# s-esposito/MonoGS

Hardware: AMD Instinct MI355X
Metric: rasteriser fwd+bwd Mpix/s @1080p (higher is better)
Workload: dtype f32; 1 GPU; C5: 2000000 Gaussians, 1920x1080, fwd+bwd, seeded synthetic map (SURVEY.md 8d), one keyframe per GPU; gaussians=2000000, width=1920, height=1080, settle_steps=60, instance_count=device-side (capacity mode, overflow checked), parallelism=keyframe-per-gpu x1

## Files before the change

include/monogs_raster.h:

```cpp
#ifndef MONOGS_RASTER_H
#define MONOGS_RASTER_H

#include <stddef.h>
#include <stdint.h>

#ifdef __cplusplus
extern "C" {
#endif

#define MGS_ABI_VERSION 12
#define MGS_TILE 16

typedef struct mgs_camera {
    int32_t image_height;
    int32_t image_width;
    float tanfovx;
    float tanfovy;
    float scale_modifier;
    int32_t sh_degree;
    int32_t sh_coeffs;
    int32_t scale_dim;
    int32_t flags;
    const float* bg;
    const float* viewmatrix;
    const float* projmatrix;
    const float* projmatrix_raw;
    const float* campos;
} mgs_camera;

#define MGS_FLAG_EXCLUSIVE_DEVICE 1

typedef struct mgs_timing {
    float preprocess_ms;
    float depth_sort_ms;
    float scan_ms;
    float duplicate_ms;
    float sort_ms;
    float ranges_ms;
    float blend_fwd_ms;
    float blend_bwd_ms;
    float geom_bwd_ms;
} mgs_timing;

int mgs_abi_version(void);
const char* mgs_last_error(void);

#define MGS_MAX_GAUSSIANS ((1 << 26) - 1)

size_t mgs_geometry_bytes(int32_t P);
size_t mgs_image_bytes(int32_t width, int32_t height);
size_t mgs_binning_bytes(uint64_t num_rendered, int32_t width, int32_t height);
size_t mgs_backward_bytes(int32_t P);
float* mgs_backward_tau(void* backward_scratch, int32_t P);

int mgs_forward_preprocess(const mgs_camera* cam, int32_t P,
                           const float* means3D,
                           const float* shs,
                           const float* colors_precomp,
                           const float* opacities,
                           const float* scales,
                           const float* rotations,
                           const float* cov3D_precomp,
                           void* geometry, int32_t* radii ,
                           void* prepare_backward ,
                           uint64_t* num_rendered ,
                           const uint32_t* prev_status ,
                           uint32_t* prev_status_out ,
                           mgs_timing* timing , void* stream);

int mgs_forward_render(const mgs_camera* cam, int32_t P, uint64_t num_rendered,
                       void* geometry, void* binning, void* image,
                       float* out_color, float* out_depth, float* out_opacity, int32_t* n_touched,
                       uint32_t* status ,
                       mgs_timing* timing, void* stream);

#define MGS_STATUS_CAPACITY_OVERFLOW 1u
#define MGS_STATUS_DEPTH_SORT_TIMEOUT 2u
#define MGS_STATUS_TILE_SORT_TIMEOUT 4u

int mgs_debug_set_radix_spin_limit(uint32_t limit);
int mgs_debug_set_option(const char* name, int64_t value);

int mgs_binning_path(int32_t P, int32_t W, int32_t H);

size_t mgs_debug_sort_temp_bytes(uint64_t n, int32_t bits);
int mgs_debug_sort_pairs(uint32_t* keys, uint32_t* vals, uint32_t* keys_alt, uint32_t* vals_alt, uint64_t n, int32_t bits,
                         void* temp, void* stream);

int mgs_forward_render_capacity(const mgs_camera* cam, int32_t P, uint64_t capacity,
                                void* geometry, void* binning, void* image,
                                float* out_color, float* out_depth, float* out_opacity, int32_t* n_touched,
                                uint32_t* overflow, mgs_timing* timing, void* stream);
int mgs_forward_capacity(const mgs_camera* cam, int32_t P, const float* means3D, const float* shs,
                         const float* colors_precomp, const float* opacities, const float* scales, const float* rotations,
                         const float* cov3D_precomp, void* geometry, int32_t* radii, void* prepare_backward,
                         uint64_t capacity, void* binning, void* image, float* out_color, float* out_depth,
                         float* out_opacity, int32_t* n_touched, uint32_t* overflow, mgs_timing* timing, void* stream);

int mgs_backward(const mgs_camera* cam, int32_t P, uint64_t num_rendered,
                 const float* means3D, const float* shs, const float* colors_precomp,
                 const float* opacities, const float* scales, const float* rotations,
                 const float* cov3D_precomp, const int32_t* radii,
                 const void* geometry, const void* binning, const void* image,
                 const float* dL_dcolor, const float* dL_ddepth,
                 const float* out_color, const float* out_depth,
                 float* dL_dmeans2D,
                 float* dL_dcolors,
                 float* dL_dopacity,
                 float* dL_dmeans3D,
                 float* dL_dcov3D,
                 float* dL_dsh,
                 float* dL_dscales,
                 float* dL_drotations,
                 float* dL_dtau,
                 void* backward_scratch, int32_t scratch_prepared, mgs_timing* timing, void* stream);

#define MGS_VALU_CEILING_BLOCKS 2048
int mgs_debug_valu_ceiling(float* out, int32_t iters, void* stream);

int mgs_debug_set_blend_events(void* fwd_start, void* fwd_end, void* bwd_start, void* bwd_end);

int mgs_debug_last_backward_split(void);

#define MGS_BLEND_STATS_WORDS 24
int mgs_debug_blend_stats(const mgs_camera* cam, int32_t P, uint64_t num_rendered, const void* geometry,
                          const void* binning, const void* image, uint64_t* stats_dev, void* stream);

int mgs_mark_visible(int32_t P, const float* means3D, const float* viewmatrix, const float* projmatrix,
                     uint8_t* visible, void* stream);

size_t mgs_knn_scratch_bytes(int32_t P);
int mgs_dist2_knn(int32_t P, const float* points , float* out ,
                  void* scratch, void* stream);

#define MGS_LOSS_TRACKING 1
#define MGS_LOSS_INVERT_DEPTH 2
#define MGS_LOSS_SCRATCH_DAB 10
#define MGS_LOSS_SCRATCH_LOSS 12
size_t mgs_loss_scratch_bytes(void);
int mgs_loss_forward(int32_t width, int32_t height, int32_t mode, int32_t init, float lambda_rgb,
                     const float* render, const float* depth, const float* opacity, const float* gt_rgb,
                     const float* gt_depth, const uint8_t* mask, const uint8_t* grad_mask,
                     const float* exposure_a, const float* exposure_b, float* scratch, float* loss_out,
                     void* stream);
int mgs_loss_backward(int32_t width, int32_t height, int32_t mode, int32_t init, float lambda_rgb,
                      const float* render, const float* depth, const float* opacity, const float* gt_rgb,
                      const float* gt_depth, const uint8_t* mask, const uint8_t* grad_mask,
                      const float* exposure_a, const float* exposure_b, const float* scratch,
                      const float* grad_out, float* d_render, float* d_depth, float* d_exposure, void* stream);
int mgs_loss_grads(int32_t width, int32_t height, int32_t mode, int32_t init, float lambda_rgb,
                   const float* render, const float* depth, const float* opacity, const float* gt_rgb,
                   const float* gt_depth, const uint8_t* mask, const uint8_t* grad_mask,
                   const float* exposure_a, const float* exposure_b, float* scratch, float* d_render, float* d_depth,
                   void* stream);

#define MGS_SSIM_C1 0.0001f
#define MGS_SSIM_C2 0.0009f
#define MGS_SSIM_SCRATCH_LOSS 0
#define MGS_SSIM_SCRATCH_L1 1
#define MGS_SSIM_SCRATCH_SSIM 2
size_t mgs_ssim_scratch_bytes(int32_t planes, int32_t width, int32_t height, int32_t train);
int mgs_ssim_forward(int32_t planes, int32_t width, int32_t height, int32_t valid, int32_t train, float C1, float C2,
                     const float* img1, const float* img2, float* scratch, float* value_out, void* stream);
int mgs_ssim_backward(int32_t planes, int32_t width, int32_t height, int32_t valid, float C1, float C2,
                      const float* img1, const float* img2, const float* scratch, const float* grad_out,
                      float* d_img1, void* stream);
int mgs_refine_loss_forward(int32_t width, int32_t height, float lambda_ssim, const float* render, const float* gt_rgb,
                            float* scratch, float* loss_out, void* stream);
int mgs_refine_loss_backward(int32_t width, int32_t height, float lambda_ssim, const float* render, const float* gt_rgb,
                             const float* scratch, const float* grad_out, float* d_render, void* stream);
int mgs_refine_loss_grads(int32_t width, int32_t height, float lambda_ssim, const float* render, const float* gt_rgb,
                          float* scratch, float* d_render, void* stream);

#define MGS_POSE_STICKY 1
int mgs_pose_step(float* R, float* T, float* rot_delta, float* trans_delta, float* exposure_a, float* exposure_b,
                  const float* grad_rot, const float* grad_trans, const float* grad_a, const float* grad_b,
                  float* adam_m, float* adam_v, int32_t step, float lr_rot, float lr_trans, float lr_exposure,
                  float beta1, float beta2, float eps, float converged_threshold, int32_t* step_counter, float* out,
                  int32_t flags, float* host_flag ,
                  const float* projmatrix_raw, float* viewmatrix, float* projmatrix, float* campos ,
                  void* stream);
int mgs_pose_step_batch(int32_t n, void* const* ptrs, float lr_rot, float lr_trans, float lr_exposure, float beta1,
                        float beta2, float eps, float converged_threshold, int32_t flags, void* stream);

int mgs_backproject(int32_t N, int32_t W, int32_t H, const int64_t* selected, const float* rgb ,
                    const float* depth , const int32_t* segmentation ,
                    const float* exposure_a, const float* exposure_b, float fx, float fy, float cx, float cy,
                    const float* R, const float* T, float* points , float* features ,
                    int32_t* ids , void* stream);

int mgs_camera_setup(const float* R, const float* T, const float* projmatrix_raw, float* viewmatrix ,
                     float* projmatrix , float* campos , void* stream);

int mgs_adam_step(int32_t n_tensors, float* const* params, const float* const* grads, float* const* exp_avg,
                  float* const* exp_avg_sq, const uint64_t* numel, const float* lr, double beta1, double beta2,
                  double eps, int32_t step, int32_t* step_counter,
                  const float* lr_device ,
                  void* stream);
int mgs_densify_stats(int32_t P, const float* viewspace_grad , const int32_t* radii,
                      float* xyz_gradient_accum , float* denom , float* max_radii_2d ,
                      void* stream);
int mgs_window_stats(int32_t P, int32_t n_keyframes, const float* const* grad_means2D, const int32_t* const* radii,
                     const int32_t* const* n_touched, float* grad_norm , float* visible ,
                     float* max_radii , int32_t accumulate, uint64_t* visibility_bits, void* stream);
int mgs_window_apply(int32_t P, const float* grad_norm, const float* visible, const float* max_radii,
                     float* xyz_gradient_accum, float* denom, float* max_radii_2d, void* stream);
int mgs_lr_schedule_step(int32_t* iteration, float* lr_out, double lr_init, double lr_final, int32_t lr_delay_steps,
                         double lr_delay_mult, int32_t max_steps, void* stream);

int mgs_activate_forward(int32_t P, int32_t scale_dim , const float* rot_raw ,
                         const float* scale_raw , const float* opacity_raw ,
                         float* rotations , float* scales3 , float* opacities ,
                         void* stream);
int mgs_activate_backward(int32_t P, int32_t scale_dim, const float* rot_raw, const float* scales3,
                          const float* opacities, const float* grad_rotations, const float* grad_scales3,
                          const float* grad_opacities, float* d_rot_raw, float* d_scale_raw, float* d_opacity_raw,
                          void* stream);

int mgs_sum_buffers(int32_t n_src, const float* const* src, float* dst, uint64_t count, void* stream);

#ifdef __cplusplus
}
#endif
#endif
```

monogs_amd/_lib.py:

```python
from __future__ import annotations

import ctypes as C
import os

_HERE = os.path.dirname(os.path.abspath(__file__))
LIB_PATH = os.environ.get("MGS_LIB_PATH") or os.path.join(_HERE, "lib", "libmonogs_raster.so")
ABI_VERSION = 12

c_float_p = C.c_void_p


class MgsCamera(C.Structure):
    _fields_ = [
        ("image_height", C.c_int32), ("image_width", C.c_int32),
        ("tanfovx", C.c_float), ("tanfovy", C.c_float), ("scale_modifier", C.c_float),
        ("sh_degree", C.c_int32), ("sh_coeffs", C.c_int32), ("scale_dim", C.c_int32), ("flags", C.c_int32),
        ("bg", C.c_void_p), ("viewmatrix", C.c_void_p), ("projmatrix", C.c_void_p),
        ("projmatrix_raw", C.c_void_p), ("campos", C.c_void_p),
    ]


class MgsTiming(C.Structure):
    _fields_ = [(n, C.c_float) for n in (
        "preprocess_ms", "depth_sort_ms", "scan_ms", "duplicate_ms", "sort_ms", "ranges_ms", "blend_fwd_ms",
        "blend_bwd_ms", "geom_bwd_ms")]

    def as_dict(self):
        return {n: float(getattr(self, n)) for n, _ in self._fields_}


SIGNATURES = {
    "mgs_abi_version": (C.c_int, []),
    "mgs_last_error": (C.c_char_p, []),
    "mgs_geometry_bytes": (C.c_size_t, [C.c_int32]),
    "mgs_image_bytes": (C.c_size_t, [C.c_int32, C.c_int32]),
    "mgs_binning_bytes": (C.c_size_t, [C.c_uint64, C.c_int32, C.c_int32]),
    "mgs_backward_bytes": (C.c_size_t, [C.c_int32]),
    "mgs_forward_preprocess": (C.c_int, [C.POINTER(MgsCamera), C.c_int32] + [C.c_void_p] * 7
                               + [C.c_void_p, C.c_void_p, C.c_void_p, C.POINTER(C.c_uint64), C.c_void_p, C.POINTER(C.c_uint32),
                                  C.POINTER(MgsTiming), C.c_void_p]),
    "mgs_forward_capacity": (C.c_int, [C.POINTER(MgsCamera), C.c_int32] + [C.c_void_p] * 7 + [C.c_void_p] * 3 + [C.c_uint64]
                             + [C.c_void_p] * 7 + [C.POINTER(MgsTiming), C.c_void_p]),
    "mgs_forward_render": (C.c_int, [C.POINTER(MgsCamera), C.c_int32, C.c_uint64] + [C.c_void_p] * 8
                           + [C.POINTER(MgsTiming), C.c_void_p]),
    "mgs_debug_set_radix_spin_limit": (C.c_int, [C.c_uint32]),
    "mgs_debug_set_option": (C.c_int, [C.c_char_p, C.c_int64]),
    "mgs_binning_path": (C.c_int, [C.c_int32, C.c_int32, C.c_int32]),
    "mgs_debug_sort_temp_bytes": (C.c_size_t, [C.c_uint64, C.c_int32]),
    "mgs_debug_sort_pairs": (C.c_int, [C.c_void_p] * 4 + [C.c_uint64, C.c_int32, C.c_void_p, C.c_void_p]),
    "mgs_forward_render_capacity": (C.c_int, [C.POINTER(MgsCamera), C.c_int32, C.c_uint64] + [C.c_void_p] * 8
                                    + [C.POINTER(MgsTiming), C.c_void_p]),
    "mgs_backward": (C.c_int, [C.POINTER(MgsCamera), C.c_int32, C.c_uint64] + [C.c_void_p] * 7
                     + [C.c_void_p] * 4 + [C.c_void_p] * 4 + [C.c_void_p] * 9
                     + [C.c_void_p, C.c_int32, C.POINTER(MgsTiming), C.c_void_p]),
    "mgs_backward_tau": (C.c_void_p, [C.c_void_p, C.c_int32]),
    "mgs_debug_blend_stats": (C.c_int, [C.POINTER(MgsCamera), C.c_int32, C.c_uint64] + [C.c_void_p] * 5),
    "mgs_debug_valu_ceiling": (C.c_int, [C.c_void_p, C.c_int32, C.c_void_p]),
    "mgs_debug_set_blend_events": (C.c_int, [C.c_void_p] * 4),
    "mgs_debug_last_backward_split": (C.c_int, []),
    "mgs_mark_visible": (C.c_int, [C.c_int32, C.c_void_p, C.c_void_p, C.c_void_p, C.c_void_p, C.c_void_p]),
    "mgs_loss_scratch_bytes": (C.c_size_t, []),
    "mgs_loss_forward": (C.c_int, [C.c_int32] * 4 + [C.c_float] + [C.c_void_p] * 9 + [C.c_void_p, C.c_void_p, C.c_void_p]),
    "mgs_loss_backward": (C.c_int, [C.c_int32] * 4 + [C.c_float] + [C.c_void_p] * 9
                          + [C.c_void_p, C.c_void_p, C.c_void_p, C.c_void_p, C.c_void_p, C.c_void_p]),
    "mgs_loss_grads": (C.c_int, [C.c_int32] * 4 + [C.c_float] + [C.c_void_p] * 9 + [C.c_void_p] * 4),
    "mgs_ssim_scratch_bytes": (C.c_size_t, [C.c_int32] * 4),
    "mgs_ssim_forward": (C.c_int, [C.c_int32] * 5 + [C.c_float] * 2 + [C.c_void_p] * 5),
    "mgs_ssim_backward": (C.c_int, [C.c_int32] * 4 + [C.c_float] * 2 + [C.c_void_p] * 6),
    "mgs_refine_loss_forward": (C.c_int, [C.c_int32] * 2 + [C.c_float] + [C.c_void_p] * 5),
    "mgs_refine_loss_backward": (C.c_int, [C.c_int32] * 2 + [C.c_float] + [C.c_void_p] * 6),
    "mgs_refine_loss_grads": (C.c_int, [C.c_int32] * 2 + [C.c_float] + [C.c_void_p] * 5),
    "mgs_backproject": (C.c_int, [C.c_int32] * 3 + [C.c_void_p] * 6 + [C.c_float] * 4 + [C.c_void_p] * 6),
    "mgs_camera_setup": (C.c_int, [C.c_void_p] * 7),
    "mgs_pose_step": (C.c_int, [C.c_void_p] * 12 + [C.c_int32] + [C.c_float] * 7
                      + [C.c_void_p, C.c_void_p, C.c_int32, C.c_void_p] + [C.c_void_p] * 4 + [C.c_void_p]),
    "mgs_pose_step_batch": (C.c_int, [C.c_int32, C.POINTER(C.c_void_p)] + [C.c_float] * 7 + [C.c_int32, C.c_void_p]),
    "mgs_adam_step": (C.c_int, [C.c_int32] + [C.c_void_p] * 6 + [C.c_double] * 3 + [C.c_int32, C.c_void_p, C.c_void_p, C.c_void_p]),
    "mgs_window_stats": (C.c_int, [C.c_int32, C.c_int32] + [C.c_void_p] * 6 + [C.c_int32, C.c_void_p, C.c_void_p]),
    "mgs_window_apply": (C.c_int, [C.c_int32] + [C.c_void_p] * 7),
    "mgs_lr_schedule_step": (C.c_int, [C.c_void_p, C.c_void_p, C.c_double, C.c_double, C.c_int32, C.c_double, C.c_int32, C.c_void_p]),
    "mgs_densify_stats": (C.c_int, [C.c_int32] + [C.c_void_p] * 6),
    "mgs_sum_buffers": (C.c_int, [C.c_int32, C.POINTER(C.c_void_p), C.c_void_p, C.c_uint64, C.c_void_p]),
    "mgs_activate_forward": (C.c_int, [C.c_int32, C.c_int32] + [C.c_void_p] * 7),
    "mgs_activate_backward": (C.c_int, [C.c_int32, C.c_int32] + [C.c_void_p] * 10),
    "mgs_knn_scratch_bytes": (C.c_size_t, [C.c_int32]),
    "mgs_dist2_knn": (C.c_int, [C.c_int32, C.c_void_p, C.c_void_p, C.c_void_p, C.c_void_p]),
}

_lib = None


class MonoGSNativeError(RuntimeError):
    pass


def load():
    global _lib
    if _lib is not None:
        return _lib
    if not os.path.exists(LIB_PATH):
        raise MonoGSNativeError(
            f"{LIB_PATH} not found: build it with `python -c 'import __graft_entry__ as g; g.build()'` "
            "or `make -C monogs_amd/csrc`.  There is no CPU fallback.")
    lib = C.CDLL(LIB_PATH)
    for name, (res, args) in SIGNATURES.items():
        fn = getattr(lib, name)
        fn.restype = res
        fn.argtypes = args
    if lib.mgs_abi_version() != ABI_VERSION:
        raise MonoGSNativeError(f"ABI mismatch: library {lib.mgs_abi_version()} vs binding {ABI_VERSION}; rebuild")
    for kv in filter(None, os.environ.get("MGS_DEBUG_OPTIONS", "").split(",")):
        k, _, v = kv.partition("=")
        if lib.mgs_debug_set_option(k.strip().encode(), int(v)) != 0:
            raise MonoGSNativeError(f"MGS_DEBUG_OPTIONS: {lib.mgs_last_error().decode()}")
    _lib = lib
    return lib


def check(rc: int, what: str):
    if rc != 0:
        msg = load().mgs_last_error().decode("utf-8", "replace")
        raise Exception(msg) if rc == 1 else MonoGSNativeError(f"{what}: {msg}")
```

monogs_amd/csrc/api.hip:

```cpp
#include "common.h"

#include <stdarg.h>
#include <stdio.h>
#include <string.h>

namespace mgs {

static thread_local char g_err[512] = "";

void set_error(const char* fmt, ...) {
    va_list ap;
    va_start(ap, fmt);
    vsnprintf(g_err, sizeof(g_err), fmt, ap);
    va_end(ap);
}

static inline char* take(char*& p, size_t bytes) {
    char* r = p;
    p += align_up(bytes, 256);
    return r;
}

GeometryState GeometryState::carve(void* base, int P) {
    char* p = (char*)align_up((size_t)base, 256);
    GeometryState g;
    g.rec = (float*)take(p, (size_t)P * REC_FLOATS * sizeof(float));
    g.depth_key = (uint32_t*)take(p, (size_t)P * sizeof(uint32_t));
    g.depth_alt = (uint32_t*)take(p, (size_t)P * sizeof(uint32_t));
    g.iota = (uint32_t*)take(p, (size_t)P * sizeof(uint32_t));
    g.iota_alt = (uint32_t*)take(p, (size_t)P * sizeof(uint32_t));
    g.perm = (uint32_t*)take(p, (size_t)P * sizeof(uint32_t));
    g.point_offsets = (uint32_t*)take(p, (size_t)P * sizeof(uint32_t));
    g.scan_blocks = (uint32_t*)take(p, ((size_t)scan_nblocks(P) + 64) * sizeof(uint32_t));
    g.clamped = (uint8_t*)take(p, (size_t)P * 4);
    g.rect = (uint2*)take(p, (size_t)P * sizeof(uint2));
    g.rect_sorted = (uint2*)take(p, (size_t)P * sizeof(uint2));
    g.scan_status = (uint64_t*)take(p, (SCAN_SMALL_MAX_BLOCKS + 1) * sizeof(uint64_t));
    g.tile_hist = (uint32_t*)take(p, 4 * 256 * sizeof(uint32_t));
    g.sort_temp_bytes = radix_depth_temp_bytes((uint64_t)P);
    g.sort_temp = take(p, g.sort_temp_bytes);
    g.end = p;
    return g;
}
size_t GeometryState::bytes(int P) {
    const GeometryState g = carve(nullptr, P);
    return (size_t)g.end + 256;
}

size_t ImageState::bytes(int W, int H) {
    const size_t HW = (size_t)W * H, nt = (size_t)tiles_x(W) * tiles_y(H);
    return align_up(HW * 4, 256) * 2 + align_up(nt * sizeof(uint2), 256) + 256;
}
ImageState ImageState::carve(void* base, int W, int H) {
    const size_t HW = (size_t)W * H, nt = (size_t)tiles_x(W) * tiles_y(H);
    char* p = (char*)align_up((size_t)base, 256);
    ImageState s;
    s.final_T = (float*)take(p, HW * 4);
    s.n_contrib = (uint32_t*)take(p, HW * 4);
    s.ranges = (uint2*)take(p, nt * sizeof(uint2));
    return s;
}

size_t BinningState::bytes(uint64_t R, int W, int H) {
    const size_t r = (size_t)(R ? R : 1);
    return align_up(r * 4, 256) * 4 + align_up(mgs::sort_temp_bytes(R, tile_bits(W, H)), 256) + 256 + 256;
}
BinningState BinningState::carve(void* base, uint64_t R, int W, int H) {
    const size_t r = (size_t)(R ? R : 1);
    char* p = (char*)align_up((size_t)base, 256);
    BinningState b;
    b.keys_a = (uint32_t*)take(p, r * 4);
    b.keys_b = (uint32_t*)take(p, r * 4);
    b.vals_a = (uint32_t*)take(p, r * 4);
    b.vals_b = (uint32_t*)take(p, r * 4);
    const bool in_b = radix_result_in_b(tile_bits(W, H));
    b.keys_sorted = in_b ? b.keys_b : b.keys_a;
    b.vals_sorted = in_b ? b.vals_b : b.vals_a;
    b.sort_temp_bytes = mgs::sort_temp_bytes(R, tile_bits(W, H));
    b.sort_temp = take(p, b.sort_temp_bytes);
    b.count = (uint32_t*)take(p, 2 * sizeof(uint32_t));
    return b;
}

struct StageTimer {
    hipStream_t s;
    bool on;
    hipEvent_t ev[10];
    int n = 0;
    StageTimer(hipStream_t s_, bool on_) : s(s_), on(on_) {
        if (on) for (auto& e : ev) (void)hipEventCreate(&e);
    }
    ~StageTimer() {
        if (on) for (auto& e : ev) (void)hipEventDestroy(e);
    }
    void mark() {
        if (on && n < 10) (void)hipEventRecord(ev[n++], s);
    }
    float ms(int i) {
        float t = 0.f;
        if (on && i + 1 < n) (void)hipEventElapsedTime(&t, ev[i], ev[i + 1]);
        return t;
    }
    void sync() {
        if (on && n) (void)hipEventSynchronize(ev[n - 1]);
    }
};

static int check_cam(const mgs_camera* cam) {
    if (!cam) { set_error("camera is NULL"); return 1; }
    if (cam->image_width <= 0 || cam->image_height <= 0) { set_error("image size must be positive"); return 1; }
    if (!cam->bg || !cam->viewmatrix || !cam->projmatrix || !cam->projmatrix_raw || !cam->campos) {
        set_error("camera tensors (bg, viewmatrix, projmatrix, projmatrix_raw, campos) must be non-NULL");
        return 1;
    }
    return 0;
}

static hipEvent_t g_dbg_fwd_events[2] = {nullptr, nullptr}, g_dbg_bwd_events[2] = {nullptr, nullptr};

static int check_map_size(int32_t P) {
    if (P > MGS_MAX_GAUSSIANS) {
        set_error("P exceeds MGS_MAX_GAUSSIANS (2^26 - 1): the gradient-line offset of the blend backward is 32-bit");
        return 1;
    }
    return 0;
}

}

using namespace mgs;

extern "C" {

int mgs_abi_version(void) { return MGS_ABI_VERSION; }
int mgs_binning_path(int32_t P, int32_t W, int32_t H) { return binning_path(P, W, H); }
const char* mgs_last_error(void) { return g_err; }

size_t mgs_geometry_bytes(int32_t P) { return GeometryState::bytes(P < 0 ? 0 : P); }
size_t mgs_image_bytes(int32_t W, int32_t H) { return ImageState::bytes(W, H); }
size_t mgs_binning_bytes(uint64_t R, int32_t W, int32_t H) { return BinningState::bytes(R, W, H); }
size_t mgs_backward_bytes(int32_t P) {
    return (size_t)(P < 0 ? 0 : P) * GRAD_FLOATS * sizeof(float) + (size_t)(TAU_SLOTS + 1) * 16 * sizeof(float) + 256;
}
float* mgs_backward_tau(void* backward_scratch, int32_t P) { return backward_tau_out(backward_scratch, P < 0 ? 0 : P); }

int mgs_forward_preprocess(const mgs_camera* cam, int32_t P, const float* means3D, const float* shs,
                           const float* colors_precomp, const float* opacities, const float* scales,
                           const float* rotations, const float* cov3D_precomp, void* geometry, int32_t* radii,
                           void* prepare_backward, uint64_t* num_rendered, const uint32_t* prev_status,
                           uint32_t* prev_status_out, mgs_timing* timing, void* stream) {
    if (check_cam(cam)) return 1;
    if (P < 0) { set_error("P must be >= 0"); return 1; }
    if (check_map_size(P)) return 1;
    if (num_rendered) *num_rendered = 0;
    if (prev_status_out) *prev_status_out = 0;
    if (P == 0) {
        if (prev_status && prev_status_out) {
            MGS_HIP(hipMemcpyAsync(prev_status_out, prev_status, sizeof(uint32_t), hipMemcpyDeviceToHost, (hipStream_t)stream));
            MGS_HIP(hipStreamSynchronize((hipStream_t)stream));
        }
        return 0;
    }
    if (!means3D || !opacities || !geometry || !radii) { set_error("means3D, opacities, geometry, radii must be non-NULL"); return 1; }
    if ((shs == nullptr) == (colors_precomp == nullptr)) {
        set_error("Please provide excatly one of either SHs or precomputed colors!");
        return 1;
    }
    const bool have_sr = scales != nullptr || rotations != nullptr;
    if ((have_sr && (!scales || !rotations || cov3D_precomp)) || (!have_sr && !cov3D_precomp)) {
        set_error("Please provide exactly one of either scale/rotation pair or precomputed 3D covariance!");
        return 1;
    }
    if (shs && (cam->sh_degree < 0 || cam->sh_degree > 3 || cam->sh_coeffs < (cam->sh_degree + 1) * (cam->sh_degree + 1))) {
        set_error("sh_degree must be 0..3 and shs must hold at least (degree+1)^2 coefficients");
        return 1;
    }
    hipStream_t s = (hipStream_t)stream;
    GeometryState g = GeometryState::carve(geometry, P);
    StageTimer tm(s, timing != nullptr);
    tm.mark();
    if (int rc = launch_preprocess_forward(*cam, P, means3D, shs, colors_precomp, opacities, scales, rotations,
                                           cov3D_precomp, g, radii,
                                           prepare_backward ? backward_grad_acc(prepare_backward) : nullptr, s)) return rc;
    tm.mark();
    const bool exclusive = (cam->flags & MGS_FLAG_EXCLUSIVE_DEVICE) != 0;
    const bool per_tile = binning_path(P, cam->image_width, cam->image_height) != 0;
    if (per_tile) {
        tm.mark();
        if (int rc = launch_scan(g, P, s, exclusive, g.rect)) return rc;
    } else {
        if (int rc = launch_depth_sort(g, P, depth_sort_payload(P, cam->image_width, cam->image_height), s, exclusive)) return rc;
        tm.mark();
        if (int rc = launch_scan(g, P, s, exclusive, g.rect_sorted)) return rc;
    }
    tm.mark();
    if (num_rendered) {
        uint32_t total = 0, sort_errors[RADIX_ERROR_WORDS] = {0, 0, 0, 0};
        MGS_HIP(hipMemcpyAsync(&total, g.scan_blocks + scan_nblocks(P), sizeof(uint32_t), hipMemcpyDeviceToHost, s));
        MGS_HIP(hipMemcpyAsync(sort_errors, radix_depth_error_flag(g.sort_temp, (uint64_t)P), sizeof(sort_errors),
                               hipMemcpyDeviceToHost, s));
        if (prev_status && prev_status_out)
            MGS_HIP(hipMemcpyAsync(prev_status_out, prev_status, sizeof(uint32_t), hipMemcpyDeviceToHost, s));
        MGS_HIP(hipStreamSynchronize(s));
        if (sort_errors[0] | sort_errors[1] | sort_errors[2] | sort_errors[3]) { set_error("depth sort: a look-back spin timed out (results invalid)"); return 3; }
        *num_rendered = total;
    }
    if (timing) {
        if (!num_rendered) MGS_HIP(hipStreamSynchronize(s));
        timing->preprocess_ms = tm.ms(0);
        timing->depth_sort_ms = per_tile ? 0.f : tm.ms(1);
        timing->scan_ms = tm.ms(2);
    }
    return 0;
}

static int g_opt_tile_sort_fused = 1;

static int forward_render_impl(const mgs_camera* cam, int32_t P, uint64_t R, bool capacity, void* geometry,
                               void* binning, void* image, float* out_color, float* out_depth, float* out_opacity,
                               int32_t* n_touched, uint32_t* overflow, mgs_timing* timing, void* stream) {
    if (check_cam(cam)) return 1;
    if (P < 0) { set_error("P must be >= 0"); return 1; }
    if (check_map_size(P)) return 1;
    if (!image || !out_color || !out_depth || !out_opacity) { set_error("image scratch and outputs must be non-NULL"); return 1; }
    if (P > 0 && (!geometry || !n_touched)) { set_error("geometry and n_touched must be non-NULL"); return 1; }
    if (R > 0 && !binning) { set_error("binning scratch is NULL"); return 1; }
    if (R >= (1ull << 32)) { set_error("num_rendered exceeds 2^32-1"); return 1; }
    if (P == 0) R = 0;
    hipStream_t s = (hipStream_t)stream;
    const int W = cam->image_width, H = cam->image_height;
    GeometryState g = GeometryState::carve(geometry, P);
    ImageState img = ImageState::carve(image, W, H);
    BinningState b = BinningState::carve(binning, R, W, H);
    const uint32_t* n_dev = nullptr;
    StageTimer tm(s, timing != nullptr);
    const bool cap = capacity && binning;
    if (cap) n_dev = b.count;
    const bool per_tile = binning_path(P, W, H) != 0;
    tm.mark();
    if (int rc = launch_duplicate(*cam, P, g, b, capacity ? R : (R > 0 ? 0xFFFFFFFFull : 0ull), n_touched, img, R,
                                  tile_bits(W, H), cap ? b.count : nullptr, overflow, s, per_tile)) return rc;
    tm.mark();
    if (int rc = launch_sort(g, b, R, tile_bits(W, H), s, n_dev, (cam->flags & MGS_FLAG_EXCLUSIVE_DEVICE) != 0, img.ranges,
                             per_tile)) return rc;
    const uint32_t* sort_err = R > 0 ? radix_error_flag(b.sort_temp, R, tile_bits(W, H)) : nullptr;
    const bool sort_tiles = per_tile && R > 0;
    const TileSortArgs ts = sort_tiles ? tile_sort_args(*cam, g, b, R, n_dev) : TileSortArgs{};
    const bool fused = sort_tiles && g_opt_tile_sort_fused != 0;
    if (sort_tiles && !fused)
        if (int rc = launch_tile_depth_sort(*cam, ts, img, sort_err, s)) return rc;
    tm.mark();
    if (g_dbg_fwd_events[0]) MGS_HIP(hipEventRecord(g_dbg_fwd_events[0], s));
    if (int rc = launch_blend_forward(*cam, g, b, img, out_color, out_depth, out_opacity, n_touched, sort_err, overflow,
                                      fused ? &ts : nullptr, s)) return rc;
    if (g_dbg_fwd_events[1]) MGS_HIP(hipEventRecord(g_dbg_fwd_events[1], s));
    tm.mark();
    if (timing) {
        tm.sync();
        timing->duplicate_ms = tm.ms(0);
        timing->sort_ms = tm.ms(1);
        timing->ranges_ms = 0.f;
        timing->blend_fwd_ms = tm.ms(2);
    }
    return 0;
}

int mgs_forward_render(const mgs_camera* cam, int32_t P, uint64_t R, void* geometry, void* binning, void* image,
                       float* out_color, float* out_depth, float* out_opacity, int32_t* n_touched,
                       uint32_t* status, mgs_timing* timing, void* stream) {
    return forward_render_impl(cam, P, R, false, geometry, binning, image, out_color, out_depth, out_opacity, n_touched,
                               status, timing, stream);
}

int mgs_forward_render_capacity(const mgs_camera* cam, int32_t P, uint64_t capacity, void* geometry, void* binning,
                                void* image, float* out_color, float* out_depth, float* out_opacity,
                                int32_t* n_touched, uint32_t* overflow, mgs_timing* timing, void* stream) {
    if (capacity == 0) { set_error("capacity must be > 0"); return 1; }
    return forward_render_impl(cam, P, capacity, true, geometry, binning, image, out_color, out_depth, out_opacity,
                               n_touched, overflow, timing, stream);
}

int mgs_forward_capacity(const mgs_camera* cam, int32_t P, const float* means3D, const float* shs,
                         const float* colors_precomp, const float* opacities, const float* scales, const float* rotations,
                         const float* cov3D_precomp, void* geometry, int32_t* radii, void* prepare_backward,
                         uint64_t capacity, void* binning, void* image, float* out_color, float* out_depth,
                         float* out_opacity, int32_t* n_touched, uint32_t* overflow, mgs_timing* timing, void* stream) {
    if (int rc = mgs_forward_preprocess(cam, P, means3D, shs, colors_precomp, opacities, scales, rotations, cov3D_precomp,
                                        geometry, radii, prepare_backward, nullptr, nullptr, nullptr, timing, stream)) return rc;
    return mgs_forward_render_capacity(cam, P, capacity, geometry, binning, image, out_color, out_depth, out_opacity,
                                       n_touched, overflow, timing, stream);
}

int mgs_backward(const mgs_camera* cam, int32_t P, uint64_t R, const float* means3D, const float* shs,
                 const float* colors_precomp, const float* opacities, const float* scales, const float* rotations,
                 const float* cov3D_precomp, const int32_t* radii, const void* geometry, const void* binning,
                 const void* image, const float* dL_dcolor, const float* dL_ddepth, const float* out_color,
                 const float* out_depth, float* dL_dmeans2D, float* dL_dcolors, float* dL_dopacity, float* dL_dmeans3D, float* dL_dcov3D, float* dL_dsh,
                 float* dL_dscales, float* dL_drotations, float* dL_dtau, void* backward_scratch,
                 int32_t scratch_prepared, mgs_timing* timing, void* stream) {
    if (check_cam(cam)) return 1;
    if (P < 0) { set_error("P must be >= 0"); return 1; }
    if (check_map_size(P)) return 1;
    hipStream_t s = (hipStream_t)stream;
    if (P == 0) {
        if (dL_dtau) MGS_HIP(zero_fill(dL_dtau, 6 * sizeof(float), s));
        return 0;
    }
    if (!means3D || !opacities || !radii || !geometry || !image || !dL_dcolor || !dL_ddepth || !backward_scratch) {
        set_error("means3D, opacities, radii, geometry, image, dL_dcolor, dL_ddepth, backward_scratch must be non-NULL");
        return 1;
    }
    if (R > 0 && !binning) { set_error("binning scratch is NULL"); return 1; }
    const int W = cam->image_width, H = cam->image_height;
    GeometryState g = GeometryState::carve(const_cast<void*>(geometry), P);
    ImageState img = ImageState::carve(const_cast<void*>(image), W, H);
    BinningState b = BinningState::carve(const_cast<void*>(binning), R, W, H);
    float* grad_acc = backward_grad_acc(backward_scratch);
    StageTimer tm(s, timing != nullptr);
    float* tau_part = (dL_dtau && (P + 255) / 256 > TAU_DIRECT_MAX_BLOCKS) ? backward_tau_part(backward_scratch, P) : nullptr;
    if (scratch_prepared) {
        if (dL_dtau && dL_dtau != backward_tau_out(backward_scratch, P)) {
            set_error("scratch_prepared: dL_dtau must be mgs_backward_tau(backward_scratch, P)");
            return 1;
        }
    } else {
        MGS_HIP(zero_fill2(grad_acc, (size_t)P * GRAD_FLOATS * sizeof(float) + (tau_part ? (size_t)TAU_SLOTS * 16 * sizeof(float) : 0),
                           dL_dtau, 6 * sizeof(float), s));
    }
    tm.mark();
    if (R > 0) {
        const bool pose_only = !dL_dcolors && !dL_dopacity && !dL_dsh && !shs;
        if (g_dbg_bwd_events[0]) MGS_HIP(hipEventRecord(g_dbg_bwd_events[0], s));
        if (int rc = launch_blend_backward(*cam, g, b, img, dL_dcolor, dL_ddepth, out_color, out_depth, grad_acc, pose_only, R, s)) return rc;
        if (g_dbg_bwd_events[1]) MGS_HIP(hipEventRecord(g_dbg_bwd_events[1], s));
    }
    tm.mark();
    GeomBackwardArgs a;
    a.means3D = means3D; a.shs = shs; a.colors_precomp = colors_precomp; a.opacities = opacities;
    a.scales = scales; a.rotations = rotations; a.cov3D_precomp = cov3D_precomp; a.radii = radii;
    a.grad_acc = grad_acc;
    a.dL_dmeans2D = dL_dmeans2D; a.dL_dcolors = dL_dcolors; a.dL_dopacity = dL_dopacity;
    a.dL_dmeans3D = dL_dmeans3D; a.dL_dcov3D = dL_dcov3D; a.dL_dsh = dL_dsh; a.dL_dscales = dL_dscales;
    a.dL_drotations = dL_drotations; a.dL_dtau = dL_dtau; a.tau_part = tau_part;
    if (int rc = launch_geom_backward(*cam, P, g, a, s)) return rc;
    tm.mark();
    if (timing) {
        tm.sync();
        timing->blend_bwd_ms = tm.ms(0);
        timing->geom_bwd_ms = tm.ms(1);
    }
    return 0;
}

int mgs_debug_blend_stats(const mgs_camera* cam, int32_t P, uint64_t R, const void* geometry, const void* binning,
                           const void* image, uint64_t* stats_dev, void* stream) {
    if (check_cam(cam)) return 1;
    if (!geometry || !image || !stats_dev || (R > 0 && !binning)) { set_error("bad arguments"); return 1; }
    hipStream_t s = (hipStream_t)stream;
    MGS_HIP(zero_fill(stats_dev, MGS_BLEND_STATS_WORDS * sizeof(uint64_t), s));
    if (P == 0 || R == 0) return 0;
    const int W = cam->image_width, H = cam->image_height;
    GeometryState g = GeometryState::carve(const_cast<void*>(geometry), P);
    ImageState img = ImageState::carve(const_cast<void*>(image), W, H);
    BinningState b = BinningState::carve(const_cast<void*>(binning), R, W, H);
    return launch_blend_backward_stats(*cam, g, b, img, (unsigned long long*)stats_dev, s);
}

int mgs_debug_valu_ceiling(float* out, int32_t iters, void* stream) {
    if (!out || iters < 1) { set_error("mgs_debug_valu_ceiling: bad arguments"); return 1; }
    return launch_valu_ceiling(out, iters, (hipStream_t)stream);
}

int mgs_debug_last_backward_split(void) { return g_dbg_last_bwd_split; }

int mgs_debug_set_radix_spin_limit(uint32_t limit) { return set_radix_spin_limit(limit); }

int mgs_debug_set_blend_events(void* fwd_start, void* fwd_end, void* bwd_start, void* bwd_end) {
    if ((fwd_start == nullptr) != (fwd_end == nullptr) || (bwd_start == nullptr) != (bwd_end == nullptr)) {
        set_error("mgs_debug_set_blend_events: a pair is both events or neither");
        return 1;
    }
    g_dbg_fwd_events[0] = (hipEvent_t)fwd_start; g_dbg_fwd_events[1] = (hipEvent_t)fwd_end;
    g_dbg_bwd_events[0] = (hipEvent_t)bwd_start; g_dbg_bwd_events[1] = (hipEvent_t)bwd_end;
    return 0;
}

static int g_opt_debug_sort_exclusive = 0;
size_t mgs_debug_sort_temp_bytes(uint64_t n, int32_t bits) { return radix_temp_bytes(n, bits); }
int mgs_debug_sort_pairs(uint32_t* keys, uint32_t* vals, uint32_t* keys_alt, uint32_t* vals_alt, uint64_t n, int32_t bits,
                         void* temp, void* stream) {
    if (bits < 1 || bits > 32 || (n && (!keys || !vals || !keys_alt || !vals_alt || !temp))) {
        set_error("mgs_debug_sort_pairs: bad arguments");
        return 1;
    }
    if (n == 0) return 0;
    hipStream_t s = (hipStream_t)stream;
    if (int rc = radix_sort_pairs(keys, vals, keys_alt, vals_alt, n, bits, temp, s, nullptr, false, nullptr, nullptr, nullptr, false,
                                  g_opt_debug_sort_exclusive != 0))
        return rc;
    if (radix_result_in_b(bits)) {
        MGS_HIP(hipMemcpyAsync(keys, keys_alt, n * 4, hipMemcpyDeviceToDevice, s));
        MGS_HIP(hipMemcpyAsync(vals, vals_alt, n * 4, hipMemcpyDeviceToDevice, s));
    }
    uint32_t err[RADIX_ERROR_WORDS];
    MGS_HIP(hipMemcpyAsync(err, radix_error_flag(temp, n, bits), sizeof(err), hipMemcpyDeviceToHost, s));
    MGS_HIP(hipStreamSynchronize(s));
    if (err[0] | err[1] | err[2] | err[3]) { set_error("mgs_debug_sort_pairs: a look-back spin timed out"); return 2; }
    return 0;
}

int mgs_debug_set_option(const char* name, int64_t value) {
    if (name && !strcmp(name, "radix_scanned")) { g_opt_radix_scanned = (int)value; return 0; }
    if (name && !strcmp(name, "radix_ballot_rank")) { g_opt_radix_ballot_rank = (int)value; return 0; }
    if (name && !strcmp(name, "radix_xcd_band")) { g_opt_radix_xcd_band = (int)value; return 0; }
    if (name && !strcmp(name, "debug_sort_exclusive")) { g_opt_debug_sort_exclusive = (int)value; return 0; }
    if (name && !strcmp(name, "dup_slot_major")) { g_opt_dup_slot_major = (int)value; return 0; }
    if (name && !strcmp(name, "blend_bwd_transposed")) {
        g_opt_blend_bwd_transposed = value < 0 ? 2 : (int)value;
        g_opt_blend_bwd_transposed_set = value >= 0;
        return 0;
    }
    if (name && !strcmp(name, "blend_bwd_split")) { g_opt_blend_bwd_split = value < 0 ? -1 : (int)value; return 0; }
    if (name && !strcmp(name, "blend_bwd_split_min")) { g_opt_blend_bwd_split_min = value < 0 ? 4 : (int)value; return 0; }
    if (name && !strcmp(name, "blend_bwd_split_frac")) { g_opt_blend_bwd_split_frac = value < 0 ? 32 : (int)value; return 0; }
    if (name && !strcmp(name, "scan_small")) { g_opt_scan_small = (int)value; return 0; }
    if (name && !strcmp(name, "tile_sort_fused")) { g_opt_tile_sort_fused = value < 0 ? 1 : (int)value; return 0; }
    if (name && !strcmp(name, "knn_grid_min")) { g_opt_knn_grid_min = value > 0x7FFFFFFF ? 0x7FFFFFFF : (int)value; return 0; }
    set_error("mgs_debug_set_option: unknown option");
    return 1;
}

int mgs_mark_visible(int32_t P, const float* means3D, const float* viewmatrix, const float* projmatrix,
                     uint8_t* visible, void* stream) {
    (void)projmatrix;
    if (P < 0 || (P > 0 && (!means3D || !viewmatrix || !visible))) { set_error("bad arguments"); return 1; }
    return launch_mark_visible(P, means3D, viewmatrix, visible, (hipStream_t)stream);
}

size_t mgs_knn_scratch_bytes(int32_t P) { return knn_scratch_bytes(P); }

int mgs_dist2_knn(int32_t P, const float* points, float* out, void* scratch, void* stream) {
    if (P < 0 || (P > 0 && (!points || !out))) { set_error("bad arguments"); return 1; }
    return launch_knn(P, points, out, scratch, (hipStream_t)stream);
}

}
```

monogs_amd/csrc/binning.hip:

```cpp
#include "common.h"
#include "tile_sort.h"


namespace mgs {

constexpr int SCAN_THREADS = 256;
__device__ __forceinline__ int scan_nblocks_dev(int P) { return (P + SCAN_ITEMS - 1) / SCAN_ITEMS; }
constexpr int SCAN_PER_THREAD = SCAN_ITEMS / SCAN_THREADS;

__device__ __forceinline__ uint32_t wave_incl_scan(uint32_t v, int) { return wave_incl_scan_dpp(v); }

__device__ __forceinline__ uint32_t block_excl_scan(uint32_t v, uint32_t& total, uint32_t* smem ) {
    const int lane = threadIdx.x & 63, wv = threadIdx.x >> 6;
    const uint32_t incl = wave_incl_scan(v, lane);
    if (lane == 63) smem[wv] = incl;
    __syncthreads();
    uint32_t base = 0;
    for (int w = 0; w < wv; ++w) base += smem[w];
    total = smem[0] + smem[1] + smem[2] + smem[3];
    __syncthreads();
    return base + incl - v;
}

__device__ __forceinline__ uint32_t scan_block_rows(const uint2* __restrict__ rects, int n, int cbase, int lane, int wv,
                                                    uint32_t (&incl)[SCAN_PER_THREAD], uint32_t* smem ) {
    uint32_t v[SCAN_PER_THREAD];
#pragma unroll
    for (int i = 0; i < SCAN_PER_THREAD; ++i) {
        const int idx = cbase + i * WAVE + lane;
        const uint32_t wh = idx < n ? rects[idx].y : 0u;
        v[i] = (wh & 0xFFFFu) * (wh >> 16);
    }
    uint32_t run = 0;
#pragma unroll
    for (int i = 0; i < SCAN_PER_THREAD; ++i) {
        const uint32_t sc = wave_incl_scan_dpp(v[i]);
        incl[i] = run + sc;
        run += (uint32_t)__builtin_amdgcn_readlane((int)sc, 63);
    }
    if (lane == 0) smem[wv] = run;
    __syncthreads();
    uint32_t wbase = 0;
    for (int w = 0; w < wv; ++w) wbase += smem[w];
    const uint32_t total = (smem[0] + smem[1]) + (smem[2] + smem[3]);
#pragma unroll
    for (int i = 0; i < SCAN_PER_THREAD; ++i) incl[i] += wbase;
    return total;
}

__global__ void __launch_bounds__(SCAN_THREADS) scan_local_kernel(const uint2* __restrict__ rects, uint32_t* out,
                                                                  uint32_t* block_sums, int n) {
    __shared__ uint32_t smem[8];
    const int lane = threadIdx.x & 63, wv = threadIdx.x >> 6;
    const int cbase = blockIdx.x * SCAN_ITEMS + wv * (SCAN_PER_THREAD * WAVE);
    uint32_t incl[SCAN_PER_THREAD];
    const uint32_t total = scan_block_rows(rects, n, cbase, lane, wv, incl, smem);
#pragma unroll
    for (int i = 0; i < SCAN_PER_THREAD; ++i) {
        const int idx = cbase + i * WAVE + lane;
        if (idx < n) out[idx] = incl[i];
    }
    if (threadIdx.x == 0) block_sums[blockIdx.x] = total;
}

__global__ void __launch_bounds__(SCAN_THREADS) scan_blocks_kernel(uint32_t* block_sums, int nblocks) {
    __shared__ uint32_t smem[8];
    uint32_t carry = 0;
    for (int start = 0; start < nblocks; start += SCAN_THREADS) {
        const int i = start + threadIdx.x;
        const uint32_t v = i < nblocks ? block_sums[i] : 0u;
        uint32_t total;
        const uint32_t ex = block_excl_scan(v, total, smem);
        if (i < nblocks) block_sums[i] = carry + ex;
        carry += total;
    }
    if (threadIdx.x == 0) block_sums[nblocks] = carry;
}

constexpr uint32_t SCAN_SPIN_LIMIT = 1u << 22;
__global__ void __launch_bounds__(SCAN_THREADS) scan_small_kernel(const uint2* __restrict__ rects, uint32_t* out,
                                                                  uint32_t* block_sums, uint64_t* status, int n, int nb,
                                                                  uint32_t* err, int ticketed) {
    __shared__ uint32_t smem[8];
    __shared__ uint32_t s_prefix, s_bid;
    const int lane = threadIdx.x & 63, wv = threadIdx.x >> 6;
    int bid = (int)blockIdx.x;
    if (ticketed) {
        if (threadIdx.x == 0) s_bid = atomicAdd((uint32_t*)(status + SCAN_SMALL_MAX_BLOCKS), 1u);
        __syncthreads();
        bid = (int)s_bid;
    }
    const int cbase = bid * SCAN_ITEMS + wv * (SCAN_PER_THREAD * WAVE);
    uint32_t incl[SCAN_PER_THREAD];
    const uint32_t total = scan_block_rows(rects, n, cbase, lane, wv, incl, smem);
    if (threadIdx.x == 0)
        __hip_atomic_store(status + bid, (1ull << 63) | (uint64_t)total, __ATOMIC_RELAXED, __HIP_MEMORY_SCOPE_AGENT);
    if (threadIdx.x < WAVE) {
        uint32_t before = 0;
        if ((int)threadIdx.x < bid) {
            uint64_t w = 0;
            uint32_t spins = 0;
            while (true) {
                w = __hip_atomic_load(status + threadIdx.x, __ATOMIC_RELAXED, __HIP_MEMORY_SCOPE_AGENT);
                if (w >> 63) break;
                if (++spins > SCAN_SPIN_LIMIT) { atomicExch(err, 1u); break; }
                __builtin_amdgcn_s_sleep(1);
            }
            before = (uint32_t)w;
        }
#pragma unroll
        for (int o = 32; o > 0; o >>= 1) before += __shfl_xor(before, o, 64);
        if (threadIdx.x == 0) s_prefix = before;
    }
    __syncthreads();
#pragma unroll
    for (int i = 0; i < SCAN_PER_THREAD; ++i) {
        const int idx = cbase + i * WAVE + lane;
        if (idx < n) out[idx] = incl[i] + s_prefix;
    }
    if (threadIdx.x == 0 && bid == nb - 1) block_sums[nb] = s_prefix + total;
}
int g_opt_scan_small = -1;
bool scan_is_small(int P) { return g_opt_scan_small != 0 && scan_nblocks(P) <= SCAN_SMALL_MAX_BLOCKS; }


int launch_scan(const GeometryState& g, int P, hipStream_t s, bool exclusive, const uint2* rects) {
    if (P == 0) return 0;
    const int nb = scan_nblocks(P);
    if (scan_is_small(P)) {
        hipLaunchKernelGGL(scan_small_kernel, dim3(nb), dim3(SCAN_THREADS), 0, s, rects, g.point_offsets, g.scan_blocks,
                           g.scan_status, P, nb, const_cast<uint32_t*>(radix_depth_error_flag(g.sort_temp, (uint64_t)P)),
                           exclusive ? 0 : 1);
        MGS_HIP(hipGetLastError());
        return 0;
    }
    hipLaunchKernelGGL(scan_local_kernel, dim3(nb), dim3(SCAN_THREADS), 0, s, rects, g.point_offsets,
                       g.scan_blocks, P);
    hipLaunchKernelGGL(scan_blocks_kernel, dim3(1), dim3(SCAN_THREADS), 0, s, g.scan_blocks, nb);
    MGS_HIP(hipGetLastError());
    return 0;
}

__device__ __forceinline__ void dup_pair(uint32_t gidx, const uint32_t* __restrict__ depth_key, int lo, uint32_t& val,
                                         uint32_t& kfield) {
    val = gidx; kfield = 0u;
    if (depth_key) {
        const uint32_t k = depth_key[gidx];
        const uint32_t d = k == 0xFFFFFFFFu ? DEPTH_KEY_NARROW : min(k - DEPTH_KEY_SUB, DEPTH_KEY_NARROW);
        kfield = d >> lo;
        if (lo) val |= (d & ((1u << lo) - 1u)) << (32 - lo);
    }
}
__global__ void __launch_bounds__(256) duplicate_kernel(int P, const uint2* __restrict__ rects,
                                                        const uint32_t* __restrict__ perm,
                                                        const uint32_t* __restrict__ depth_key, int tshift, int lo,
                                                        const uint32_t* __restrict__ offsets ,
                                                        const uint32_t* __restrict__ block_sums ,
                                                        uint32_t* keys,
                                                        uint32_t* vals, int gx, int gy, uint32_t r_cap,
                                                        int32_t* __restrict__ n_touched, uint2* __restrict__ ranges,
                                                        int ntiles, uint32_t* __restrict__ zero_ptr, size_t zero_words,
                                                        uint32_t* __restrict__ count, uint32_t* __restrict__ overflow,
                                                        const uint32_t* __restrict__ depth_err, int offsets_global,
                                                        uint32_t* __restrict__ hist , int hist_passes,
                                                        int n_threads , int slot_major) {
    const int i = blockIdx.x * 256 + threadIdx.x;
    const int lane = threadIdx.x & 63;
    grid_zero(zero_ptr, zero_words, (size_t)n_threads, 256);
    const bool depth_bad = depth_err && radix_failed(depth_err) != 0u;
    if (i == 0 && count) {
        const uint32_t R = (P > 0 && !depth_bad) ? block_sums[scan_nblocks_dev(P)] : 0u;
        count[0] = min(R, r_cap);
        count[1] = R > r_cap ? 1u : 0u;
    }
    if (i == 0 && overflow)
        overflow[0] = (count ? count[1] : 0u) | (depth_bad ? (uint32_t)MGS_STATUS_DEPTH_SORT_TIMEOUT : 0u);
    if (i < ntiles) ranges[i] = make_uint2(0xFFFFFFFFu, 0u);
    if (i < P) n_touched[i] = 0;
    uint32_t idx = 0, nt = 0, off = 0, kf = 0;
    int x0 = 0, y0 = 0, x1 = 0;
    if (i < P) {
        dup_pair(perm ? perm[i] : (uint32_t)i, depth_key, lo, idx, kf);
        const uint2 r = rects[i];
        const int w = (int)(r.y & 0xFFFFu), h = (int)(r.y >> 16);
        nt = (uint32_t)(w * h);
        x0 = (int)(r.x & 0xFFFFu); y0 = (int)(r.x >> 16); x1 = x0 + w;
    }
    if (depth_bad) nt = 0;
    if (nt) off = i == 0 ? 0u : offsets[i - 1] + (offsets_global ? 0u : block_sums[(i - 1) / SCAN_ITEMS]);
    __shared__ uint32_t s_own[4][WAVE];
    __shared__ uint32_t s_idx[4][WAVE], s_off[4][WAVE], s_kf[4][WAVE];
    __shared__ int s_x0[4][WAVE], s_y0[4][WAVE], s_w[4][WAVE];
    __shared__ uint32_t s_hist[2][256];
    if (hist) {
        s_hist[0][threadIdx.x] = 0u; s_hist[1][threadIdx.x] = 0u;
        __syncthreads();
    }
    const int wv = threadIdx.x >> 6;
    if (slot_major) {
        const uint32_t R_all = (P > 0 && !depth_bad) ? block_sums[scan_nblocks_dev(P)] : 0u;
        const uint32_t R_emit = min(R_all, r_cap);
        const uint32_t n_waves = (uint32_t)n_threads / WAVE;
        const uint32_t CH = (((R_emit + n_waves - 1u) / n_waves) + 63u) & ~63u;
        const uint32_t wave_id = (uint32_t)blockIdx.x * 4u + (uint32_t)wv;
        const uint64_t s0w = (uint64_t)wave_id * CH;
        const uint32_t s0 = s0w < (uint64_t)R_emit ? (uint32_t)s0w : R_emit, s1 = (uint64_t)s0 + CH < (uint64_t)R_emit ? s0 + CH : R_emit;
        auto incl = [&](uint32_t k) { return offsets[k] + (offsets_global ? 0u : block_sums[k / SCAN_ITEMS]); };
        uint32_t g = 0;
        if (s0 < s1) {
            uint32_t lo = 0, hi = (uint32_t)P;
            while (hi - lo > 1u) {
                const uint32_t span = hi - lo, step = (span + 63u) / 64u;
                const uint32_t probe = lo + min(((uint32_t)lane + 1u) * step, span) - 1u;
                const unsigned long long above = __builtin_amdgcn_ballot_w64(incl(probe) > s0);
                const int k = __builtin_ctzll(above);
                const uint32_t pk = lo + min(((uint32_t)k + 1u) * step, span) - 1u;
                const uint32_t pk1 = k == 0 ? lo : lo + min((uint32_t)k * step, span);
                lo = pk1; hi = pk + 1u;
            }
            g = lo;
        }
        uint32_t sl = s0;
        while (sl < s1 && g < (uint32_t)P) {
            const uint32_t gi = g + (uint32_t)lane;
            const bool valid = gi < (uint32_t)P;
            uint32_t inc = 0, ntg = 0, idg = 0, kfg = 0;
            int gx0 = 0, gy0 = 0, gw = 1;
            if (valid) {
                inc = incl(gi);
                const uint2 r = rects[gi];
                gw = (int)(r.y & 0xFFFFu);
                ntg = (uint32_t)(gw * (int)(r.y >> 16));
                gx0 = (int)(r.x & 0xFFFFu); gy0 = (int)(r.x >> 16);
                dup_pair(perm ? perm[gi] : gi, depth_key, lo, idg, kfg);
            }
            const uint32_t exc = inc - ntg;
            uint32_t Eg = valid ? inc : 0u;
#pragma unroll
            for (int o2 = 32; o2 > 0; o2 >>= 1) Eg = max(Eg, (uint32_t)__shfl_xor((int)Eg, o2, 64));
            __builtin_amdgcn_wave_barrier();
            s_idx[wv][lane] = idg; s_kf[wv][lane] = kfg; s_off[wv][lane] = exc; s_x0[wv][lane] = gx0; s_y0[wv][lane] = gy0; s_w[wv][lane] = max(gw, 1);
            const uint32_t e = min(s1, Eg);
            const uint32_t cb0 = sl & ~63u;
            const unsigned long long before = __builtin_amdgcn_ballot_w64(ntg != 0u && exc < cb0);
            uint32_t carry = before ? 64u - (uint32_t)__builtin_clzll(before) : 0u;
            for (uint32_t cb = cb0; cb < e; cb += WAVE) {
                __builtin_amdgcn_wave_barrier();
                s_own[wv][lane] = 0u;
                __builtin_amdgcn_wave_barrier();
                if (ntg != 0u && exc >= cb && exc < cb + WAVE) s_own[wv][exc - cb] = (uint32_t)lane + 1u;
                __builtin_amdgcn_wave_barrier();
                uint32_t m = s_own[wv][lane];
#define MGS_DPP_MAX(ctrl, row_mask) m = max(m, (uint32_t)__builtin_amdgcn_update_dpp(0, (int)m, ctrl, row_mask, 0xf, false))
                MGS_DPP_MAX(0x111, 0xf); MGS_DPP_MAX(0x112, 0xf); MGS_DPP_MAX(0x114, 0xf); MGS_DPP_MAX(0x118, 0xf);
                MGS_DPP_MAX(0x142, 0xa); MGS_DPP_MAX(0x143, 0xc);
#undef MGS_DPP_MAX
                const uint32_t owner = max(m, carry);
                carry = (uint32_t)__builtin_amdgcn_readlane((int)owner, 63);
                const uint32_t o = cb + lane;
                if (owner != 0u && o >= sl && o < e) {
                    const uint32_t L = owner - 1u;
                    const uint32_t t = o - s_off[wv][L];
                    const uint32_t w = (uint32_t)s_w[wv][L];
                    const uint32_t yy = t / w, xx = t - yy * w;
                    const uint32_t tid = (uint32_t)((s_y0[wv][L] + (int)yy) * gx + s_x0[wv][L] + (int)xx);
                    const uint32_t key = (tid << tshift) | s_kf[wv][L];
                    keys[o] = key;
                    vals[o] = s_idx[wv][L];
                    if (hist) {
                        atomicAdd(&s_hist[0][(key >> tshift) & 0xFFu], 1u);
                        if (hist_passes > 1) {
                            const uint32_t d1 = (key >> (tshift + 8)) & 0xFFu;
                            const uint32_t lead = (uint32_t)__builtin_amdgcn_readfirstlane((int)d1);
                            const unsigned long long same = __builtin_amdgcn_ballot_w64(d1 == lead);
                            if (d1 != lead) atomicAdd(&s_hist[1][d1], 1u);
                            else if (lane == (int)__builtin_ctzll(same)) atomicAdd(&s_hist[1][lead], (uint32_t)__popcll(same));
                        }
                    }
                }
            }
            sl = max(sl, e);
            if (Eg <= sl) g += WAVE;
        }
        if (hist) {
            __syncthreads();
            const uint32_t c0 = s_hist[0][threadIdx.x], c1 = s_hist[1][threadIdx.x];
            if (c0) atomicAdd(hist + threadIdx.x, c0);
            if (c1) atomicAdd(hist + 256 + threadIdx.x, c1);
        }
        return;
    }
    s_idx[wv][lane] = idx; s_kf[wv][lane] = kf; s_off[wv][lane] = off; s_x0[wv][lane] = x0; s_y0[wv][lane] = y0; s_w[wv][lane] = max(x1 - x0, 1);
    const unsigned long long live = __builtin_amdgcn_ballot_w64(nt != 0);
    if (live == 0ull && !hist) return;
    const int first = live ? __builtin_ctzll(live) : 0, lastl = live ? 63 - __builtin_clzll(live) : 0;
    const uint32_t S = live ? (uint32_t)__builtin_amdgcn_readlane((int)off, first) : 0u;
    const uint32_t E = live ? (uint32_t)__builtin_amdgcn_readlane((int)(off + nt), lastl) : 0u;
    uint32_t carry = 0;
    for (uint32_t cb = S & ~63u; cb < E; cb += WAVE) {
        __builtin_amdgcn_wave_barrier();
        s_own[wv][lane] = 0u;
        __builtin_amdgcn_wave_barrier();
        if (nt != 0 && off >= cb && off < cb + WAVE) s_own[wv][off - cb] = (uint32_t)lane + 1u;
        __builtin_amdgcn_wave_barrier();
        uint32_t m = s_own[wv][lane];
#define MGS_DPP_MAX(ctrl, row_mask) m = max(m, (uint32_t)__builtin_amdgcn_update_dpp(0, (int)m, ctrl, row_mask, 0xf, false))
        MGS_DPP_MAX(0x111, 0xf); MGS_DPP_MAX(0x112, 0xf); MGS_DPP_MAX(0x114, 0xf); MGS_DPP_MAX(0x118, 0xf);
        MGS_DPP_MAX(0x142, 0xa); MGS_DPP_MAX(0x143, 0xc);
#undef MGS_DPP_MAX
        const uint32_t owner = max(m, carry);
        carry = (uint32_t)__builtin_amdgcn_readlane((int)owner, 63);
        const uint32_t o = cb + lane;
        if (owner != 0u && o < E && o < r_cap) {
            const uint32_t L = owner - 1u;
            const uint32_t t = o - s_off[wv][L];
            const uint32_t w = (uint32_t)s_w[wv][L];
            const uint32_t yy = t / w, xx = t - yy * w;
            const uint32_t tid = (uint32_t)((s_y0[wv][L] + (int)yy) * gx + s_x0[wv][L] + (int)xx);
            const uint32_t key = (tid << tshift) | s_kf[wv][L];
            keys[o] = key;
            vals[o] = s_idx[wv][L];
            if (hist) {
                atomicAdd(&s_hist[0][(key >> tshift) & 0xFFu], 1u);
                if (hist_passes > 1) {
                    const uint32_t d1 = (key >> (tshift + 8)) & 0xFFu;
                    const uint32_t lead = (uint32_t)__builtin_amdgcn_readfirstlane((int)d1);
                    const unsigned long long same = __builtin_amdgcn_ballot_w64(d1 == lead);
                    if (d1 != lead) atomicAdd(&s_hist[1][d1], 1u);
                    else if (lane == (int)__builtin_ctzll(same)) atomicAdd(&s_hist[1][lead], (uint32_t)__popcll(same));
                }
            }
        }
    }
    if (hist) {
        __syncthreads();
        const uint32_t c0 = s_hist[0][threadIdx.x], c1 = s_hist[1][threadIdx.x];
        if (c0) atomicAdd(hist + threadIdx.x, c0);
        if (c1) atomicAdd(hist + 256 + threadIdx.x, c1);
    }
}

constexpr uint64_t DUP_SLOT_MAJOR_MIN = 768ull * 1024;
int g_opt_dup_slot_major = -1;

int launch_duplicate(const mgs_camera& cam, int P, const GeometryState& g, const BinningState& b, uint64_t r_cap,
                     int32_t* n_touched, const ImageState& img, uint64_t sort_n, int sort_bits, uint32_t* count,
                     uint32_t* overflow, hipStream_t s, bool per_tile) {
    const uint32_t* depth_err = P > 0 ? radix_depth_error_flag(g.sort_temp, (uint64_t)P) : nullptr;
    const int ntiles = tiles_x(cam.image_width) * tiles_y(cam.image_height);
    int n = P > ntiles ? P : ntiles;
    if (n == 0) return 0;
    const bool slot_major = P > 0 && g_opt_dup_slot_major != 0 &&
                            (g_opt_dup_slot_major > 0 || (sort_n >= DUP_SLOT_MAJOR_MIN && sort_n >= 6ull * (uint64_t)P));
    if (slot_major) {
        const uint64_t want = sort_n / 8;
        if (want > (uint64_t)n) n = (int)(want > 0x3FFFFFFFull ? 0x3FFFFFFFull : want);
    }
    const int n_threads = (n + 255) / 256 * 256;
    uint32_t* zero_ptr = nullptr;
    size_t zero_words = 0;
    if (sort_n > 0) radix_zero_region(b.sort_temp, sort_n, sort_bits, &zero_ptr, &zero_words);
    const bool count_digits = P > 0 && sort_bits <= 16 && radix_wants_hist(sort_n);
    const int tb = tile_bits(cam.image_width, cam.image_height);
    hipLaunchKernelGGL(duplicate_kernel, dim3(n_threads / 256), dim3(256), 0, s, P, per_tile ? g.rect : g.rect_sorted,
                       per_tile ? nullptr : g.perm, per_tile ? g.depth_key : nullptr, per_tile ? 32 - tb : 0,
                       per_tile ? tile_depth_lo_bits(tb) : 0, g.point_offsets,
                       g.scan_blocks, b.keys_a, b.vals_a, tiles_x(cam.image_width), tiles_y(cam.image_height),
                       (uint32_t)(r_cap > 0xFFFFFFFFull ? 0xFFFFFFFFull : r_cap), n_touched, img.ranges, ntiles, zero_ptr,
                       zero_words, count, overflow, depth_err,
                       (P > 0 && scan_is_small(P)) ? 1 : 0,
                       count_digits ? g.tile_hist : nullptr, (sort_bits + 7) / 8, n_threads, slot_major ? 1 : 0);
    MGS_HIP(hipGetLastError());
    return 0;
}

size_t sort_temp_bytes(uint64_t n, int bits) { return radix_temp_bytes(n, bits); }

int launch_depth_sort(const GeometryState& g, int P, bool payload, hipStream_t s, bool exclusive) {
    return radix_sort_depth(g.depth_key, g.depth_alt, g.iota, g.iota_alt, g.rect, payload, g.perm, g.rect_sorted, (uint64_t)P,
                            g.sort_temp, s, true, exclusive);
}

int launch_sort(const GeometryState& g, const BinningState& b, uint64_t R, int bits, hipStream_t s, const uint32_t* n_dev,
                bool exclusive, uint2* ranges, bool per_tile) {
    if (R == 0) return 0;
    const bool counted = bits <= 16 && radix_wants_hist(R) && g.tile_hist != nullptr;
    return radix_sort_pairs(b.keys_a, b.vals_a, b.keys_b, b.vals_b, R, bits, b.sort_temp, s, n_dev, true, nullptr, nullptr,
                            counted ? g.tile_hist : nullptr, false, exclusive, ranges, per_tile ? 32 - bits : 0);
}

TileSortArgs tile_sort_args(const mgs_camera& cam, const GeometryState& g, const BinningState& b, uint64_t R,
                            const uint32_t* n_dev) {
    TileSortArgs ts;
    ts.keys = b.keys_sorted;
    ts.vals = b.vals_sorted;
    ts.keys_alt = b.keys_sorted == b.keys_a ? b.keys_b : b.keys_a;
    ts.vals_alt = b.vals_sorted == b.vals_a ? b.vals_b : b.vals_a;
    ts.depth_key = g.depth_key;
    ts.n_dev = n_dev;
    ts.n_cap = (uint32_t)R;
    ts.tb = tile_bits(cam.image_width, cam.image_height);
    return ts;
}

__global__ void __launch_bounds__(TDS_THREADS) tile_depth_sort_kernel(TileSortArgs ts, const uint2* __restrict__ ranges,
                                                                       int ntiles, const uint32_t* __restrict__ sort_err) {
    __shared__ uint32_t s_k[TDS_CAP], s_v[TDS_CAP];
    __shared__ uint32_t s_cnt[TDS_WAVES][TDS_RADIX];
    __shared__ uint32_t s_wsum[TDS_WAVES], s_red[2 * TDS_WAVES];
    const int tile = blockIdx.x;
    if (tile >= ntiles) return;
    tile_depth_sort(ts, ranges[tile], sort_err && radix_failed(sort_err) != 0u, TdsLds{s_k, s_v, s_cnt, s_wsum, s_red});
}

int launch_tile_depth_sort(const mgs_camera& cam, const TileSortArgs& ts, const ImageState& img, const uint32_t* sort_err,
                           hipStream_t s) {
    const int ntiles = tiles_x(cam.image_width) * tiles_y(cam.image_height);
    hipLaunchKernelGGL(tile_depth_sort_kernel, dim3(ntiles), dim3(TDS_THREADS), 0, s, ts, img.ranges, ntiles, sort_err);
    MGS_HIP(hipGetLastError());
    return 0;
}


}
```

monogs_amd/csrc/blend.hip:

```cpp
#include "common.h"
#include "tile_sort.h"

#include <type_traits>


namespace mgs {

#ifdef BS_TRACE
static unsigned long long* g_trace_fwd = nullptr;
static unsigned long long* g_trace_bwd = nullptr;
static unsigned long long g_trace_bwd_records = 0;
#define BS_STAMP(v) asm volatile("s_memrealtime %0\n\ts_waitcnt lgkmcnt(0)" : "=s"(v) :: "memory")
#endif

__device__ __forceinline__ uint32_t bcast(uint32_t v, int lane) {
    return (uint32_t)__builtin_amdgcn_readlane((int)v, lane);
}

constexpr int MGS_WG_WAVES = 4;
#define MGS_TILE_WAVE(ntiles_, tile_, wave_, ws_)                                                   \
    const int tile_ = (int)blockIdx.x, wave_ = __builtin_amdgcn_readfirstlane((int)(threadIdx.x >> 6)), ws_ = wave_; \
    if (tile_ >= (ntiles_)) return;
struct BlendArgs {
#ifdef BS_TRACE
    unsigned long long* trace;
#endif
    const float4* __restrict__ rec;
    const uint32_t* __restrict__ point_list;
    const uint2* __restrict__ ranges;
    const float* __restrict__ bg;
    int W, H, gx;
};

__device__ __forceinline__ bool quadrant_hit(const float4 c , const float4 n ,
                                             float qx0, float qy0, unsigned long long alive) {
    const float x0 = qx0 - 0.05f - c.x, x1 = qx0 + (float)(SUB - 1) + 0.05f - c.x;
    const float y0 = qy0 - 0.05f - c.y, y1 = qy0 + (float)(SUB - 1) + 0.05f - c.y;
    if (c.z < 0.f) return false;
    if (!((c.z >= x0) && (-c.z <= x1) && (c.w >= y0) && (-c.w <= y1))) return false;
    {
        const int ix0 = (int)fminf(8.f, fmaxf(0.f, ceilf(-x0 - c.z - 0.06f))), ix1 = (int)fminf(7.f, fmaxf(-1.f, floorf(-x0 + c.z + 0.06f)));
        const int iy0 = (int)fminf(8.f, fmaxf(0.f, ceilf(-y0 - c.w - 0.06f))), iy1 = (int)fminf(7.f, fmaxf(-1.f, floorf(-y0 + c.w + 0.06f)));
        if (ix0 > ix1 || iy0 > iy1) return false;
        const unsigned long long cols = (unsigned long long)((0xFFu >> (7 - ix1)) & (0xFFu << ix0) & 0xFFu) * 0x0101010101010101ull;
        const unsigned long long rows = (~0ull >> (8 * (7 - iy1))) & (~0ull << (8 * iy0));
        if ((cols & rows & alive) == 0ull) return false;
    }
    if (x0 <= 0.f && x1 >= 0.f && y0 <= 0.f && y1 >= 0.f) return true;
    if (!(n.x > 0.f) || !(n.z > 0.f)) return true;
    const float rby = -n.y * __builtin_amdgcn_rcpf(n.z), rbx = -n.y * __builtin_amdgcn_rcpf(n.x);
    auto edge_x = [&](float xe) {
        const float t = fminf(y1, fmaxf(y0, rby * xe));
        return n.x * xe * xe + 2.f * n.y * xe * t + n.z * t * t;
    };
    auto edge_y = [&](float ye) {
        const float t = fminf(x1, fmaxf(x0, rbx * ye));
        return n.x * t * t + 2.f * n.y * t * ye + n.z * ye * ye;
    };
    const float qmin = fminf(fminf(edge_x(x0), edge_x(x1)), fminf(edge_y(y0), edge_y(y1)));
    return qmin <= 1.02f;
}

struct Rec {
    float px, py, ca, cb, cc, op, r, g, b, z;
};
__device__ __forceinline__ Rec fetch(const BlendArgs& a, uint32_t gid_uniform) {
    const const_float_p p = MGS_CONST(reinterpret_cast<const float*>(a.rec)) + (size_t)gid_uniform * REC_FLOATS;
    return Rec{p[R_X], p[R_Y], p[R_CA], p[R_CB], p[R_CC], p[R_OPAC], p[R_R], p[R_G], p[R_B], p[R_DEPTH]};
}

template <bool TOUCH>
__device__ __forceinline__ void blend_one(unsigned long long& live, unsigned long long& mask, float& T, uint32_t& last, float& C0, float& C1, float& C2,
                                      float& D, const Rec& g, float power, float alpha, uint32_t pos, int j,
                                      int& touched_cnt) {
    const float test_T = T * (1.f - alpha);
    float w;
    int cnt;
    if (TOUCH) {
        asm volatile(
            "s_mov_b64 exec, %[live]\n\t"
            "v_cmpx_nlt_f32_e32 vcc, 0, %[power]\n\t"
            "v_cmpx_ngt_f32_e32 vcc, %[amin], %[alpha]\n\t"
            "v_cmp_gt_f32_e32 vcc, %[tmin], %[tt]\n\t"
            "s_andn2_b64 exec, exec, vcc\n\t"
            "s_andn2_b64 %[live], %[live], vcc\n\t"
            "s_cselect_b64 %[mask], %[mask], 0\n\t"
            "v_mul_f32_e32 %[w], %[alpha], %[T]\n\t"
            "v_mov_b32_e32 %[T], %[tt]\n\t"
            "v_mov_b32_e32 %[last], %[pos]\n\t"
            "v_cmp_lt_f32_e32 vcc, 0.5, %[tt]\n\t"
            "v_fmac_f32_e32 %[C0], %[cr], %[w]\n\t"
            "v_fmac_f32_e32 %[C1], %[cg], %[w]\n\t"
            "s_bcnt1_i32_b64 %[cnt], vcc\n\t"
            "s_mov_b32 m0, %[j]\n\t"
            "v_fmac_f32_e32 %[C2], %[cb], %[w]\n\t"
            "v_fmac_f32_e32 %[D], %[cz], %[w]\n\t"
            "s_mov_b64 exec, -1\n\t"
            "v_writelane_b32 %[tc], %[cnt], m0\n\t"
            : [live] "+s"(live), [mask] "+s"(mask), [T] "+v"(T), [last] "+v"(last), [C0] "+v"(C0), [C1] "+v"(C1), [C2] "+v"(C2), [D] "+v"(D),
              [w] "=&v"(w), [cnt] "=&s"(cnt), [tc] "+v"(touched_cnt)
            : [power] "v"(power), [alpha] "v"(alpha), [tt] "v"(test_T), [amin] "s"(1.0f / 255.0f), [tmin] "s"(0.0001f),
              [pos] "s"(pos), [cr] "v"(g.r), [cg] "v"(g.g), [cb] "v"(g.b), [cz] "v"(g.z), [j] "s"(j)
            : "vcc", "scc", "m0");
    } else {
        asm volatile(
            "s_mov_b64 exec, %[live]\n\t"
            "v_cmpx_nlt_f32_e32 vcc, 0, %[power]\n\t"
            "v_cmpx_ngt_f32_e32 vcc, %[amin], %[alpha]\n\t"
            "v_cmp_gt_f32_e32 vcc, %[tmin], %[tt]\n\t"
            "s_andn2_b64 exec, exec, vcc\n\t"
            "s_andn2_b64 %[live], %[live], vcc\n\t"
            "s_cselect_b64 %[mask], %[mask], 0\n\t"
            "v_mul_f32_e32 %[w], %[alpha], %[T]\n\t"
            "v_mov_b32_e32 %[T], %[tt]\n\t"
            "v_mov_b32_e32 %[last], %[pos]\n\t"
            "v_fmac_f32_e32 %[C0], %[cr], %[w]\n\t"
            "v_fmac_f32_e32 %[C1], %[cg], %[w]\n\t"
            "v_fmac_f32_e32 %[C2], %[cb], %[w]\n\t"
            "v_fmac_f32_e32 %[D], %[cz], %[w]\n\t"
            "s_mov_b64 exec, -1\n\t"
            : [live] "+s"(live), [mask] "+s"(mask), [T] "+v"(T), [last] "+v"(last), [C0] "+v"(C0), [C1] "+v"(C1), [C2] "+v"(C2), [D] "+v"(D),
              [w] "=&v"(w)
            : [power] "v"(power), [alpha] "v"(alpha), [tt] "v"(test_T), [amin] "s"(1.0f / 255.0f), [tmin] "s"(0.0001f),
              [pos] "s"(pos), [cr] "v"(g.r), [cg] "v"(g.g), [cb] "v"(g.b), [cz] "v"(g.z)
            : "vcc", "scc");
    }
}

template <bool SORT>
__global__ void __launch_bounds__(256) blend_forward_kernel(BlendArgs a, float* __restrict__ out_color,
                                                            float* __restrict__ out_depth,
                                                            float* __restrict__ out_opacity,
                                                            float* __restrict__ final_T,
                                                            uint32_t* __restrict__ n_contrib,
                                                            int32_t* __restrict__ n_touched,
                                                            uint2* ranges_rw ,
                                                            const uint32_t* __restrict__ sort_err,
                                                            uint32_t* __restrict__ status, TileSortArgs ts) {
    MGS_TILE_WAVE(a.gx * ((a.H + TILE - 1) / TILE), tile, wave, ws)
    const int tx = tile % a.gx, ty = tile / a.gx;
    const int lane = threadIdx.x & 63;
    const bool first_of_tile = wave == 0 && lane == 0;
    const int qx0i = tx * TILE + (wave & 1) * SUB, qy0i = ty * TILE + (wave >> 1) * SUB;
    const int pxi = qx0i + (lane & 7), pyi = qy0i + (lane >> 3);
    const bool inside = pxi < a.W && pyi < a.H;
    const float pxf = (float)pxi, pyf = (float)pyi;
    const float qx0 = (float)qx0i, qy0 = (float)qy0i;
    uint2 range = ranges_rw[tile];
    const uint2 range_raw = range;
    const bool sort_bad = sort_err != nullptr && radix_failed(sort_err) != 0u;
    {
        if (sort_bad && tile == 0 && first_of_tile && status) atomicOr(status, (uint32_t)MGS_STATUS_TILE_SORT_TIMEOUT);
        if (sort_bad || range.x >= range.y) {
            range = make_uint2(0u, 0u);
            if (first_of_tile) ranges_rw[tile] = range;
        }
    }

    float T = 1.f, C0 = 0.f, C1 = 0.f, C2 = 0.f, D = 0.f;
    uint32_t last = 0;
    unsigned long long live = __builtin_amdgcn_ballot_w64(inside);
#ifdef BS_TRACE
    unsigned long long tr0;
    BS_STAMP(tr0);
#endif

    uint32_t gid_n = 0;
    float4 box_n = make_float4(0.f, 0.f, -1.f, -1.f), ell_n = make_float4(0.f, 0.f, 0.f, 0.f);
    __shared__ __attribute__((aligned(16))) float4 s_queue[MGS_WG_WAVES][WAVE][3];
    __shared__ uint32_t s_list[TDS_CAP], s_wsum[TDS_WAVES], s_red[2 * TDS_WAVES];
    static_assert(sizeof(s_queue) == sizeof(uint32_t) * (TDS_CAP + TDS_WAVES * TDS_RADIX), "sort scratch = record queue");
    bool list_in_lds = false;
    if constexpr (SORT) {
        uint32_t* const s_k = reinterpret_cast<uint32_t*>(&s_queue[0][0][0]);
        const uint32_t n_lds = tile_depth_sort(ts, range_raw, sort_bad,
                                               TdsLds{s_k, s_list, reinterpret_cast<uint32_t (*)[TDS_RADIX]>(s_k + TDS_CAP),
                                                      s_wsum, s_red});
        list_in_lds = n_lds != 0u && n_lds == range.y - range.x;
        if (!list_in_lds) __syncthreads();
    }
    float4 c1_n = make_float4(0.f, 0.f, 0.f, 0.f), c2_n = c1_n;
    float4* const my_entry = &s_queue[ws][lane][0];
    const uint32_t q_base = (uint32_t)__builtin_amdgcn_readfirstlane((int)(uint32_t)(uintptr_t)&s_queue[ws][0][0]);
    auto prefetch = [&](uint32_t i) {
        gid_n = 0;
        box_n = make_float4(0.f, 0.f, -1.f, -1.f);
        if (i < range.y) {
            if constexpr (SORT) gid_n = list_in_lds ? s_list[i - range.x] : ts.vals[i];
            else gid_n = a.point_list[i];
            box_n = a.rec[(size_t)gid_n * 4];
            ell_n = a.rec[(size_t)gid_n * 4 + 3];
            c1_n = a.rec[(size_t)gid_n * 4 + 1];
            c2_n = a.rec[(size_t)gid_n * 4 + 2];
        }
    };
    auto walk_step = [&](auto touch_tag, uint32_t base, uint32_t gid_l, unsigned long long mask) {
        int touched_cnt = 0;
        while (mask) {
            const int j = __builtin_ctzll(mask);
            mask &= ~(1ull << j);
            typedef float qv2 __attribute__((ext_vector_type(2)));
            typedef float qv4 __attribute__((ext_vector_type(4)));
            qv2 e0;
            qv4 e1, e2;
            {
                const uint32_t ad = q_base + (uint32_t)j * 48u;
                asm volatile("ds_read_b64 %0, %3\n\tds_read_b128 %1, %3 offset:16\n\tds_read_b128 %2, %3 offset:32"
                             : "=&v"(e0), "=&v"(e1), "=&v"(e2) : "v"(ad) : "memory");
            }
            asm volatile("s_waitcnt lgkmcnt(2)" : "+v"(e0));
            float dx = e0[0] - pxf, dy = e0[1] - pyf;
            asm volatile("s_waitcnt lgkmcnt(1)" : "+v"(e1), "+v"(dx), "+v"(dy));
            const float power = dx * (e1[0] * dx + e1[1] * dy) + (e1[2] * dy) * dy;
            float alpha = fminf(0.99f, e1[3] * __builtin_amdgcn_exp2f(power));
            asm volatile("s_waitcnt lgkmcnt(0)" : "+v"(e2), "+v"(alpha));
            const Rec g{e0[0], e0[1], e1[0], e1[1], e1[2], e1[3], e2[0], e2[1], e2[2], e2[3]};
            blend_one<decltype(touch_tag)::value>(live, mask, T, last, C0, C1, C2, D, g, power, alpha,
                                                  (base - range.x) + (uint32_t)j + 1u, j, touched_cnt);
        }
        if (decltype(touch_tag)::value && touched_cnt != 0) atomicAdd(n_touched + gid_l, touched_cnt);
    };
    if (range.x < range.y) prefetch(range.x + lane);
    for (uint32_t base = range.x; base < range.y && live != 0ull; base += WAVE) {
        const uint32_t gid_l = gid_n;
        const float4 c = box_n, el = ell_n;
        my_entry[0] = c; my_entry[1] = c1_n; my_entry[2] = c2_n;
        prefetch(base + WAVE + lane);
        const unsigned long long mask = __builtin_amdgcn_ballot_w64(quadrant_hit(c, el, qx0, qy0, live));
        if ((live & __builtin_amdgcn_ballot_w64(T > 0.5f)) != 0ull) walk_step(std::true_type{}, base, gid_l, mask);
        else walk_step(std::false_type{}, base, gid_l, mask);
    }
#ifdef BS_TRACE
    if (a.trace) {
        unsigned long long tr1;
        BS_STAMP(tr1);
        const unsigned hw = __builtin_amdgcn_s_getreg((31 << 11) | 4), xcc = __builtin_amdgcn_s_getreg((31 << 11) | 20);
        if (lane == 0) {
            unsigned long long* o = a.trace + ((size_t)tile * 4 + wave) * 4;
            o[0] = tr0; o[1] = tr1; o[2] = (unsigned long long)hw | ((unsigned long long)xcc << 32); o[3] = range.y - range.x;
        }
    }
#endif
    if (inside) {
        const size_t pix = (size_t)pyi * a.W + pxi, HW = (size_t)a.H * a.W;
        final_T[pix] = T;
        n_contrib[pix] = last;
        out_color[pix] = C0 + T * a.bg[0];
        out_color[HW + pix] = C1 + T * a.bg[1];
        out_color[2 * HW + pix] = C2 + T * a.bg[2];
        out_depth[pix] = D;
        out_opacity[pix] = 1.f - T;
    }
}

static BlendArgs make_args(const mgs_camera& cam, const GeometryState& g, const BinningState& b,
                           const ImageState& img) {
    BlendArgs a;
#ifdef BS_TRACE
    a.trace = nullptr;
#endif
    a.rec = reinterpret_cast<const float4*>(g.rec);
    a.point_list = b.vals_sorted;
    a.ranges = img.ranges;
    a.bg = cam.bg;
    a.W = cam.image_width;
    a.H = cam.image_height;
    a.gx = tiles_x(a.W);
    return a;
}

int launch_blend_forward(const mgs_camera& cam, const GeometryState& g, const BinningState& b,
                         const ImageState& img, float* out_color, float* out_depth, float* out_opacity,
                         int32_t* n_touched, const uint32_t* sort_err, uint32_t* status, const TileSortArgs* tile_sort,
                         hipStream_t s) {
    BlendArgs a = make_args(cam, g, b, img);
#ifdef BS_TRACE
    a.trace = g_trace_fwd;
#endif
    const int ntiles = a.gx * tiles_y(a.H);
    if (ntiles == 0) return 0;
    const dim3 grid(ntiles), block(256);
    const TileSortArgs ts = tile_sort ? *tile_sort : TileSortArgs{};
    if (tile_sort)
        hipLaunchKernelGGL(blend_forward_kernel<true>, grid, block, 0, s, a, out_color, out_depth,
                           out_opacity, img.final_T, img.n_contrib, n_touched, img.ranges, sort_err, status, ts);
    else
        hipLaunchKernelGGL(blend_forward_kernel<false>, grid, block, 0, s, a, out_color, out_depth,
                           out_opacity, img.final_T, img.n_contrib, n_touched, img.ranges, sort_err, status, ts);
    MGS_HIP(hipGetLastError());
    return 0;
}


__device__ __forceinline__ float swap32_add(float x, float y) {
    auto r = __builtin_amdgcn_permlane32_swap(__float_as_uint(x), __float_as_uint(y), false, false);
    return __uint_as_float(r[0]) + __uint_as_float(r[1]);
}
__device__ __forceinline__ float swap16_add(float x, float y) {
    auto r = __builtin_amdgcn_permlane16_swap(__float_as_uint(x), __float_as_uint(y), false, false);
    return __uint_as_float(r[0]) + __uint_as_float(r[1]);
}
template <int XOR>
__device__ __forceinline__ float swz_add(float v) {
    return v + __int_as_float(__builtin_amdgcn_ds_swizzle(__float_as_int(v), 0x001F | (XOR << 10)));
}
__device__ __forceinline__ float row_sum_all(float v) {
    v = swz_add<1>(v);
    v = swz_add<2>(v);
    v = swz_add<4>(v);
    v = swz_add<8>(v);
    return v;
}
__device__ __forceinline__ int reduce10_slot(int lane) {
    const int row = lane >> 4, pos = lane & 15;
    if (pos == 15) return row == 0 ? 0 : row == 1 ? 2 : row == 2 ? 1 : 3;
    if (pos == 0) return row == 0 ? 4 : row == 1 ? 6 : row == 2 ? 5 : 7;
    if (pos == 1) return row == 0 ? 8 : row == 2 ? 9 : -1;
    return -1;
}
__device__ __forceinline__ float reduce10(float a0, float a1, float a2, float a3, float a4, float a5, float a6,
                                          float a7, float a8, float a9, int lane) {
    const float b0 = swap32_add(a0, a1), b1 = swap32_add(a2, a3), b2 = swap32_add(a4, a5);
    const float b3 = swap32_add(a6, a7), b4 = swap32_add(a8, a9);
    float c0 = swap16_add(b0, b1);
    float c1 = swap16_add(b2, b3);
    float c2 = swz_add<16>(b4);
    c0 = row_sum_all(c0);
    c1 = row_sum_all(c1);
    c2 = row_sum_all(c2);
    const int pos = lane & 15;
    return pos == 15 ? c0 : (pos == 0 ? c1 : c2);
}

__device__ __forceinline__ int reduce6_slot(int lane) {
    const int row = lane >> 4, pos = lane & 15;
    if (pos == 15) return row == 0 ? G_SX : row == 1 ? G_SXX : row == 2 ? G_SY : G_SXY;
    if (pos == 0) return row == 0 ? G_SYY : row == 2 ? G_DDEPTH : -1;
    return -1;
}
__device__ __forceinline__ float reduce6(float a0, float a1, float a2, float a3, float a4, float a5, int lane) {
    const float b0 = swap32_add(a0, a1), b1 = swap32_add(a2, a3), b2 = swap32_add(a4, a5);
    float c0 = swap16_add(b0, b1);
    float c1 = swz_add<16>(b2);
    c0 = row_sum_all(c0);
    c1 = row_sum_all(c1);
    return (lane & 15) == 15 ? c0 : c1;
}

__device__ __forceinline__ uint32_t wave_max_u32(uint32_t v) {
#pragma unroll
    for (int o = 32; o > 0; o >>= 1) v = max(v, (uint32_t)__shfl_xor((int)v, o, 64));
    return v;
}

template <bool POSE_ONLY>
__global__ void __launch_bounds__(256) blend_backward_kernel(BlendArgs a, int ntiles,
                                                             const float* __restrict__ final_T,
                                                             const uint32_t* __restrict__ n_contrib,
                                                             const float* __restrict__ dL_dcolor,
                                                             const float* __restrict__ dL_ddepth,
                                                             float* __restrict__ grad_acc) {
    const int wave = threadIdx.x >> 6, lane = threadIdx.x & 63;
    const int tile = (int)blockIdx.x;
    if (tile >= ntiles) return;
    const int tx = tile % a.gx, ty = tile / a.gx;
    const uint2 range = a.ranges[tile];
    if (range.y <= range.x) return;
    const size_t HW = (size_t)a.H * a.W;
    const float bg0 = a.bg[0], bg1 = a.bg[1], bg2 = a.bg[2];

    const int qx0i = tx * TILE + (wave & 1) * SUB, qy0i = ty * TILE + (wave >> 1) * SUB;
    const int pxi = qx0i + (lane & 7), pyi = qy0i + (lane >> 3);
    const bool inside = pxi < a.W && pyi < a.H;
    const size_t pix = (size_t)pyi * a.W + pxi;
    const float pxf = (float)pxi, pyf = (float)pyi, qx0 = (float)qx0i, qy0 = (float)qy0i;
    const float T_final = inside ? final_T[pix] : 0.f;
    const uint32_t last = inside ? n_contrib[pix] : 0u;
    const float g0 = inside ? dL_dcolor[pix] : 0.f;
    const float g1 = inside ? dL_dcolor[HW + pix] : 0.f;
    const float g2 = inside ? dL_dcolor[2 * HW + pix] : 0.f;
    const float gd = inside ? dL_ddepth[pix] : 0.f;
    const float bgT = -T_final * (bg0 * g0 + bg1 * g1 + bg2 * g2);
    float T = T_final, Bk = 0.f;
    const uint32_t maxc = wave_max_u32(last);
    if (maxc == 0) return;
    const uint32_t end = range.x + maxc;

    const int slot = POSE_ONLY ? reduce6_slot(lane) : reduce10_slot(lane);
    const uint32_t slot_bytes = slot < 0 ? 0u : (uint32_t)slot * 4u;

    uint32_t gid_n = 0;
    float4 box_n = make_float4(0.f, 0.f, -1.f, -1.f), ell_n = make_float4(0.f, 0.f, 0.f, 0.f);
    auto prefetch = [&](int b) {
        gid_n = 0;
        box_n = make_float4(0.f, 0.f, -1.f, -1.f);
        const uint32_t i = range.x + (uint32_t)b * WAVE + lane;
        if (b >= 0 && i < end) {
            gid_n = a.point_list[i];
            box_n = a.rec[(size_t)gid_n * 4];
            ell_n = a.rec[(size_t)gid_n * 4 + 3];
        }
    };
    prefetch((int)((maxc - 1) / WAVE));
    for (int b = (int)((maxc - 1) / WAVE); b >= 0; --b) {
        const uint32_t gid_l = gid_n;
        const float4 c = box_n, el = ell_n;
        prefetch(b - 1);
        const unsigned long long alive = __builtin_amdgcn_ballot_w64(last >= (uint32_t)b * WAVE + 1u);
        unsigned long long mask = __builtin_amdgcn_ballot_w64(quadrant_hit(c, el, qx0, qy0, alive));
        const int rel_last = (int)last - (int)((uint32_t)b * WAVE + 1u);
        while (mask) {
            const int j = 63 - __builtin_clzll(mask);
            mask &= ~(1ull << j);
            const uint32_t gid = bcast(gid_l, j);
            const Rec g = fetch(a, gid);
            const float dx = g.px - pxf, dy = g.py - pyf;
            const float power = dx * (g.ca * dx + g.cb * dy) + (g.cc * dy) * dy;
            const float G = __builtin_amdgcn_exp2f(power);
            const float alpha = fminf(0.99f, g.op * G);
            const bool act = (j <= rel_last) && !(power > 0.f) && !(alpha < 1.0f / 255.0f);
            if (__builtin_amdgcn_ballot_w64(act) == 0ull) continue;
            const float a_eff = act ? alpha : 0.f;
            const float inv = __builtin_amdgcn_rcpf(1.f - a_eff);
            const float Tn = T * inv;
            const float qq = __builtin_fmaf(g.z, gd, __builtin_fmaf(g.b, g2, __builtin_fmaf(g.g, g1, g.r * g0)));
            const float diff = qq - Bk;
            const float dL_dalpha = diff * Tn + bgT * inv;
            Bk = Bk + a_eff * diff;
            T = Tn;
            const float w = a_eff * Tn;
            const float h = act ? G * dL_dalpha : 0.f;
            const float hx = h * dx, hy = h * dy;
            const float s_x = hx, s_y = hy, s_xx = hx * dx, s_xy = hx * dy, s_yy = hy * dy, s_h = h;
            const float s_r = w * g0, s_g = w * g1, s_b = w * g2, s_z = w * gd;
            const float m = POSE_ONLY ? reduce6(s_x, s_y, s_xx, s_xy, s_yy, s_z, lane)
                                      : reduce10(s_x, s_y, s_xx, s_xy, s_yy, s_h, s_r, s_g, s_b, s_z, lane);
            float* const line = grad_acc + (size_t)gid * GRAD_FLOATS;
            if (slot >= 0) asm volatile("global_atomic_add_f32 %0, %1, %2" ::"v"(slot_bytes), "v"(m), "s"(line) : "memory");
        }
    }
}
// ... 152 lines not shown
    const size_t pix = (size_t)pyi * a.W + pxi;
    const float pxf = (float)pxi, pyf = (float)pyi, qx0 = (float)qx0i, qy0 = (float)qy0i;
    const float T_final = inside ? final_T[pix] : 0.f;
    const uint32_t last = inside ? n_contrib[pix] : 0u;
    const float g0 = inside ? dL_dcolor[pix] : 0.f;
    const float g1 = inside ? dL_dcolor[HW + pix] : 0.f;
    const float g2 = inside ? dL_dcolor[2 * HW + pix] : 0.f;
    const float gd = inside ? dL_ddepth[pix] : 0.f;
    const float bgT = -T_final * (bg0 * g0 + bg1 * g1 + bg2 * g2);
    float T = T_final, Bk = 0.f;
    const uint32_t maxc = (uint32_t)__builtin_amdgcn_readfirstlane((int)wave_max_u32(last));
    if (maxc == 0) return;
    const uint32_t end = range.x + maxc;

    const int q = lane & 15;
    const int fxi = qx0i + 4 * (q & 1), fyi = qy0i + (q >> 1);
    if (lane < 16) {
#pragma unroll
        for (int i = 0; i < 4; ++i) {
            const bool in_i = (fxi + i) < a.W && fyi < a.H;
            const size_t px_i = (size_t)fyi * a.W + fxi + i;
            if (!POSE_ONLY) {
                s_pix[wave][0][q][i] = in_i ? dL_dcolor[px_i] : 0.f;
                s_pix[wave][1][q][i] = in_i ? dL_dcolor[HW + px_i] : 0.f;
                s_pix[wave][2][q][i] = in_i ? dL_dcolor[2 * HW + px_i] : 0.f;
            }
            s_pix[wave][POSE_ONLY ? 0 : 3][q][i] = in_i ? dL_ddepth[px_i] : 0.f;
        }
    }
    const int slot = POSE_ONLY ? bt_slot6(q) : bt_slot10(q);
    const uint32_t slot_bytes = slot < 0 ? 0u : (uint32_t)slot * 4u;
    const unsigned long long m_out = __builtin_amdgcn_ballot_w64(slot >= 0);
    const unsigned long long m_q0 = __builtin_amdgcn_ballot_w64((q & 3) == 0), m_q1 = __builtin_amdgcn_ballot_w64((q & 3) == 1);
    float* const fhl = &s_fac[wave][0][0][lane];
    BtMetaRec* const fmeta = &s_meta[wave][0];
    const BtLane bl{&s_fac[wave][0][0][0], &s_pix[wave][0][0][0], fmeta, lane, qx0, qy0, slot_bytes, m_out, m_q0, m_q1, grad_acc};
    int k = 0;

    uint32_t gid_n = 0;
    float4 box_n = make_float4(0.f, 0.f, -1.f, -1.f), ell_n = make_float4(0.f, 0.f, 0.f, 0.f);
    auto prefetch = [&](int b) {
        gid_n = 0;
        box_n = make_float4(0.f, 0.f, -1.f, -1.f);
        const uint32_t i = range.x + (uint32_t)b * WAVE + lane;
        if (b >= 0 && i < end) {
            gid_n = a.point_list[i];
            box_n = a.rec[(size_t)gid_n * 4];
            ell_n = a.rec[(size_t)gid_n * 4 + 3];
        }
    };
    prefetch((int)((maxc - 1) / WAVE));
    for (int b = (int)((maxc - 1) / WAVE); b >= 0; --b) {
        const uint32_t gid_l = gid_n;
        const float4 c = box_n, el = ell_n;
        prefetch(b - 1);
        const unsigned long long alive = __builtin_amdgcn_ballot_w64(last >= (uint32_t)b * WAVE + 1u);
        unsigned long long mask = __builtin_amdgcn_ballot_w64(quadrant_hit(c, el, qx0, qy0, alive));
        const uint32_t k_first = (uint32_t)b * WAVE + 1u;
        auto apply = [&](const Rec& g, int j, float power, float G, float alpha) {
            const bool act = (k_first + (uint32_t)j <= last) && !(power > 0.f) && !(alpha < 1.0f / 255.0f);
            if (__builtin_amdgcn_ballot_w64(act) == 0ull) return;
            const float a_eff = act ? alpha : 0.f;
            const float inv = __builtin_amdgcn_rcpf(1.f - a_eff);
            const float Tn = T * inv;
            const float qq = __builtin_fmaf(g.z, gd, __builtin_fmaf(g.b, g2, __builtin_fmaf(g.g, g1, g.r * g0)));
            const float diff = qq - Bk;
            const float dL_dalpha = diff * Tn + bgT * inv;
            Bk = Bk + a_eff * diff;
            T = Tn;
            const float w = a_eff * Tn;
            const float h = act ? G * dL_dalpha : 0.f;
            fhl[k * WAVE] = h;
            fhl[(BT_SLOTS + k) * WAVE] = w;
            if (__builtin_amdgcn_inverse_ballot_w64(1ull << j)) fmeta[k] = BtMetaRec{c.x, c.y, gid_l};
            if (++k == BT_SLOTS) {
                bt_flush<POSE_ONLY>(bl, BT_SLOTS);
                k = 0;
            }
        };
        while (mask) {
            const int j = 63 - __builtin_clzll(mask);
            mask &= ~(1ull << j);
            const Rec g = fetch(a, bcast(gid_l, j));
            const float dx = g.px - pxf, dy = g.py - pyf;
            const float power = dx * (g.ca * dx + g.cb * dy) + (g.cc * dy) * dy;
            const float G = __builtin_amdgcn_exp2f(power);
            apply(g, j, power, G, fminf(0.99f, g.op * G));
        }
    }
    if (k) bt_flush<POSE_ONLY>(bl, k);
}

typedef float v2f __attribute__((ext_vector_type(2)));
typedef float v3f __attribute__((ext_vector_type(3)));
typedef float v8f __attribute__((ext_vector_type(8)));
constexpr int BS_SPLIT_MIN = 4, BS_SPLIT_FRAC = 32;
struct BsSplit { int min_steps, frac256; };
__device__ __forceinline__ uint32_t bs_split_point(uint32_t maxc, BsSplit sp) {
    const uint32_t steps = (maxc + WAVE - 1) / WAVE;
    if (steps < 2u || steps < (uint32_t)sp.min_steps) return 0u;
    const uint32_t f = (maxc * (uint32_t)sp.frac256 / 256u + WAVE / 2) / WAVE;
    return min(max(f, 1u), steps - 1u) * WAVE;
}
struct BsWaveLds { float h[BT_SLOTS][BS_STRIDE / 4]; float pad[(BS_W_OFF - BT_SLOTS * BS_STRIDE) / 4]; float w[BT_SLOTS][BS_STRIDE / 4];
                   BtMetaRec meta[BT_SLOTS][BS_STRIDE / 16]; };
static_assert(sizeof(BsWaveLds) == BS_META_OFF + BT_SLOTS * BS_STRIDE, "layout");
template <bool POSE_ONLY, int DIR>
__device__ __forceinline__ void bs_walk(const BlendArgs& a, const int tile, const int job, const int wave, BsWaveLds* const s_w_ws, float* const s_pix_ws,
                                        const float* __restrict__ final_T, const uint32_t* __restrict__ n_contrib,
                                        const float* __restrict__ dL_dcolor, const float* __restrict__ dL_ddepth,
                                        const float* __restrict__ out_color, const float* __restrict__ out_depth,
                                        float* __restrict__ grad_acc, const BsSplit sp) {
    constexpr bool FRONT = DIR == 2;
    const int lane = threadIdx.x & 63;
    const int tx = tile % a.gx, ty = tile / a.gx;
    const uint2 range = a.ranges[tile];
    if (range.y <= range.x) return;
    const size_t HW = (size_t)a.H * a.W;

    const int qx0i = tx * TILE + (wave & 1) * SUB, qy0i = ty * TILE + (wave >> 1) * SUB;
    const int pxi = qx0i + (lane & 7), pyi = qy0i + (lane >> 3);
    const bool inside = pxi < a.W && pyi < a.H;
    const size_t pix = (size_t)pyi * a.W + pxi;
    const float pxf = (float)pxi, pyf = (float)pyi;
    const uint32_t last = inside ? n_contrib[pix] : 0u;
    const uint32_t maxc = (uint32_t)__builtin_amdgcn_readfirstlane((int)wave_max_u32(last));
    if (maxc == 0) return;
    const uint32_t m = DIR == 0 ? 0u : bs_split_point(maxc, sp);
    if (FRONT && m == 0) return;
    const float g0 = inside ? dL_dcolor[pix] : 0.f;
    const float g1 = inside ? dL_dcolor[HW + pix] : 0.f;
    const float g2 = inside ? dL_dcolor[2 * HW + pix] : 0.f;
    const float gd = inside ? dL_ddepth[pix] : 0.f;
    float T, Bk, bgT = 0.f;
    if (FRONT) {
        const float C0 = inside ? out_color[pix] : 0.f, C1 = inside ? out_color[HW + pix] : 0.f;
        const float C2 = inside ? out_color[2 * HW + pix] : 0.f, Dz = inside ? out_depth[pix] : 0.f;
        T = 1.f;
        Bk = -(C0 * g0 + C1 * g1 + C2 * g2 + Dz * gd);
    } else {
        const float T_final = inside ? final_T[pix] : 0.f;
        bgT = -T_final * (a.bg[0] * g0 + a.bg[1] * g1 + a.bg[2] * g2);
        T = T_final, Bk = 0.f;
    }
    const uint32_t end = range.x + (FRONT ? m : maxc);
    const int b_lo = (int)(m / WAVE);
#ifdef BS_TRACE
    unsigned long long tr0;
    uint32_t tr_n = 0;
    BS_STAMP(tr0);
#endif

    const int q = lane & 15;
    const int fxi = qx0i + 4 * (q & 1), fyi = qy0i + (q >> 1);
    if (lane < 16) {
#pragma unroll
        for (int i = 0; i < 4; ++i) {
            const bool in_i = (fxi + i) < a.W && fyi < a.H;
            const size_t px_i = (size_t)fyi * a.W + fxi + i;
            if (!POSE_ONLY) {
                s_pix_ws[(0 * 16 + q) * 4 + i] = in_i ? dL_dcolor[px_i] : 0.f;
                s_pix_ws[(1 * 16 + q) * 4 + i] = in_i ? dL_dcolor[HW + px_i] : 0.f;
                s_pix_ws[(2 * 16 + q) * 4 + i] = in_i ? dL_dcolor[2 * HW + px_i] : 0.f;
            }
            s_pix_ws[((POSE_ONLY ? 0 : 3) * 16 + q) * 4 + i] = in_i ? dL_ddepth[px_i] : 0.f;
        }
    }
    const int slot = POSE_ONLY ? bt_slot6(q) : bt_slot10(q);
    const uint32_t slot_bytes = slot < 0 ? 0u : (uint32_t)slot * 4u;
    const unsigned long long m_out = __builtin_amdgcn_ballot_w64(slot >= 0);
    const unsigned long long m_q0 = __builtin_amdgcn_ballot_w64((q & 3) == 0), m_q1 = __builtin_amdgcn_ballot_w64((q & 3) == 1);
    const BtLane bl{&s_w_ws->h[0][0], s_pix_ws, &s_w_ws->meta[0][0], lane, 0.f, 0.f, slot_bytes, m_out, m_q0, m_q1, grad_acc, qx0i, qy0i};
    const uint32_t wbase = (uint32_t)__builtin_amdgcn_readfirstlane((int)(uint32_t)(uintptr_t)s_w_ws);
    const const_float_p recs = MGS_CONST(reinterpret_cast<const float*>(a.rec));
    uint32_t koff = 0;
    float zero = 0.f;
    asm volatile("" : "+v"(zero));

    uint32_t gid_n = 0;
    float4 box_n = make_float4(0.f, 0.f, -1.f, -1.f), ell_n = make_float4(0.f, 0.f, 0.f, 0.f);
    auto prefetch = [&](int b) {
        gid_n = 0;
        box_n = make_float4(0.f, 0.f, -1.f, -1.f);
        const uint32_t i = range.x + (uint32_t)b * WAVE + (uint32_t)(FRONT ? lane : 63 - lane);
        if (b >= (FRONT ? 0 : b_lo) && i < end) {
            gid_n = a.point_list[i];
            box_n = a.rec[(size_t)gid_n * 4];
            ell_n = a.rec[(size_t)gid_n * 4 + 3];
        }
    };
    const int b_first = FRONT ? 0 : (int)((maxc - 1) / WAVE), b_step = FRONT ? 1 : -1;
    prefetch(b_first);
    for (int b = b_first; FRONT ? b < b_lo : b >= b_lo; b += b_step) {
        const float4 c = box_n, el = ell_n;
        v3f meta = {c.x, c.y, __uint_as_float(gid_n << 6)};
        prefetch(b + b_step);
        const unsigned long long alive = __builtin_amdgcn_ballot_w64(last >= (uint32_t)b * WAVE + 1u);
        int qxs = qx0i, qys = qy0i;
        asm volatile("" : "+s"(qxs), "+s"(qys));
        unsigned long long mask = __builtin_amdgcn_ballot_w64(quadrant_hit(c, el, (float)qxs, (float)qys, alive));
        const int thr = FRONT ? (int)last - (int)((uint32_t)b * WAVE + 1u) : 63 + (int)((uint32_t)b * WAVE + 1u) - (int)last;
#define BS_POP(J, R0, R1)                                                                                                    \
        asm volatile("s_ff1_i32_b64 %0, %1\n\ts_bitset0_b64 %1, %0" : "=&s"(J), "+s"(mask));                                 \
        {                                                                                                                    \
            const uint32_t goff = (uint32_t)__builtin_amdgcn_readlane((int)__float_as_uint(meta[2]), J);                     \
            asm volatile("s_load_dwordx2 %0, %2, %3\n\ts_load_dwordx8 %1, %2, %3 offset:0x10"                                \
                         : "=&s"(R0), "=&s"(R1) : "s"(recs), "s"(goff) : "memory");                                          \
        }
        auto evaluate = [&](const v2f r0, const v8f r1, const int j) {
                float dx, dy, t1, t2, G, al, inv, qq;
                uint32_t adv, sa, tmp;
                if (FRONT)
                asm volatile(
                    "v_sub_f32_e32 %[dx], %[px], %[pxf]\n\t"
                    "v_sub_f32_e32 %[dy], %[py], %[pyf]\n\t"
                    "v_mul_f32_e32 %[t1], %[cb], %[dy]\n\t"
                    "v_mul_f32_e32 %[t2], %[cc], %[dy]\n\t"
                    "v_fmac_f32_e32 %[t1], %[ca], %[dx]\n\t"
                    "v_mul_f32_e32 %[t2], %[dy], %[t2]\n\t"
                    "v_fmac_f32_e32 %[t2], %[dx], %[t1]\n\t"
                    "v_exp_f32_e32 %[G], %[t2]\n\t"
                    "s_add_u32 %[tmp], %[wbase], %[koff]\n\t"
                    "v_lshl_add_u32 %[sa], %[lane], 2, %[tmp]\n\t"
                    "ds_write2st64_b32 %[sa], %[zero], %[zero] offset1:5\n\t"
                    "v_cmpx_le_i32_e32 vcc, %[j], %[thr]\n\t"
                    "v_cmpx_nlt_f32_e32 vcc, 0, %[t2]\n\t"
                    "v_mul_f32_e32 %[al], %[op], %[G]\n\t"
                    "v_min_f32_e32 %[al], 0x3f7d70a4, %[al]\n\t"
                    "v_cmpx_ngt_f32_e32 vcc, %[amin], %[al]\n\t"
                    "v_sub_f32_e32 %[t1], 1.0, %[al]\n\t"
                    "v_rcp_f32_e32 %[inv], %[t1]\n\t"
                    "v_mul_f32_e32 %[qq], %[cr], %[g0]\n\t"
                    "v_fmac_f32_e32 %[qq], %[cg], %[g1]\n\t"
                    "v_fmac_f32_e32 %[qq], %[cb2], %[g2]\n\t"
                    "v_fmac_f32_e32 %[qq], %[cz], %[gd]\n\t"
                    "v_mul_f32_e32 %[dy], %[al], %[T]\n\t"
                    "v_mul_f32_e32 %[dx], %[T], %[qq]\n\t"
                    "v_fmac_f32_e32 %[Bk], %[dy], %[qq]\n\t"
                    "v_fmac_f32_e32 %[dx], %[Bk], %[inv]\n\t"
                    "v_mul_f32_e32 %[dx], %[G], %[dx]\n\t"
                    "v_mul_f32_e32 %[T], %[T], %[t1]\n\t"
                    "ds_write2st64_b32 %[sa], %[dx], %[dy] offset1:5\n\t"
                    "s_cmp_lg_u64 exec, 0\n\t"
                    "s_cselect_b32 %[adv], 272, 0\n\t"
                    "s_lshl_b64 exec, 1, %[j]\n\t"
                    "v_mov_b32_e32 %[sa], %[tmp]\n\t"
                    "ds_write_b96 %[sa], %[meta] offset:2368\n\t"
                    "s_mov_b64 exec, -1\n\t"
                    : [dx] "=&v"(dx), [dy] "=&v"(dy), [t1] "=&v"(t1), [t2] "=&v"(t2), [G] "=&v"(G), [al] "=&v"(al), [inv] "=&v"(inv),
                      [qq] "=&v"(qq), [sa] "=&v"(sa), [T] "+v"(T), [Bk] "+v"(Bk), [adv] "=&s"(adv), [tmp] "=&s"(tmp)
                    : [px] "s"(r0[0]), [py] "s"(r0[1]), [ca] "s"(r1[0]), [cb] "s"(r1[1]), [cc] "s"(r1[2]), [op] "s"(r1[3]),
                      [cr] "s"(r1[4]), [cg] "s"(r1[5]), [cb2] "s"(r1[6]), [cz] "s"(r1[7]), [pxf] "v"(pxf), [pyf] "v"(pyf), [thr] "v"(thr),
                      [j] "s"(j), [g0] "v"(g0), [g1] "v"(g1), [g2] "v"(g2), [gd] "v"(gd), [lane] "v"(lane), [zero] "v"(zero),
                      [koff] "s"(koff), [wbase] "s"(wbase), [meta] "v"(meta), [amin] "s"(1.0f / 255.0f)
                    : "vcc", "scc", "memory");
                else
                asm volatile(
                    "v_sub_f32_e32 %[dx], %[px], %[pxf]\n\t"
                    "v_sub_f32_e32 %[dy], %[py], %[pyf]\n\t"
                    "v_mul_f32_e32 %[t1], %[cb], %[dy]\n\t"
                    "v_mul_f32_e32 %[t2], %[cc], %[dy]\n\t"
                    "v_fmac_f32_e32 %[t1], %[ca], %[dx]\n\t"
                    "v_mul_f32_e32 %[t2], %[dy], %[t2]\n\t"
                    "v_fmac_f32_e32 %[t2], %[dx], %[t1]\n\t"
                    "v_exp_f32_e32 %[G], %[t2]\n\t"
                    "s_add_u32 %[tmp], %[wbase], %[koff]\n\t"
                    "v_lshl_add_u32 %[sa], %[lane], 2, %[tmp]\n\t"
                    "ds_write2st64_b32 %[sa], %[zero], %[zero] offset1:5\n\t"
                    "v_cmpx_ge_i32_e32 vcc, %[j], %[thr]\n\t"
                    "v_cmpx_nlt_f32_e32 vcc, 0, %[t2]\n\t"
                    "v_mul_f32_e32 %[al], %[op], %[G]\n\t"
                    "v_min_f32_e32 %[al], 0x3f7d70a4, %[al]\n\t"
                    "v_cmpx_ngt_f32_e32 vcc, %[amin], %[al]\n\t"
                    "v_sub_f32_e32 %[inv], 1.0, %[al]\n\t"
                    "v_rcp_f32_e32 %[inv], %[inv]\n\t"
                    "v_mul_f32_e32 %[qq], %[cr], %[g0]\n\t"
                    "v_fmac_f32_e32 %[qq], %[cg], %[g1]\n\t"
                    "v_fmac_f32_e32 %[qq], %[cb2], %[g2]\n\t"
                    "v_fmac_f32_e32 %[qq], %[cz], %[gd]\n\t"
                    "v_mul_f32_e32 %[T], %[T], %[inv]\n\t"
                    "v_sub_f32_e32 %[qq], %[qq], %[Bk]\n\t"
                    "v_mul_f32_e32 %[dx], %[T], %[qq]\n\t"
                    "v_fmac_f32_e32 %[dx], %[bgT], %[inv]\n\t"
                    "v_mul_f32_e32 %[dx], %[G], %[dx]\n\t"
                    "v_mul_f32_e32 %[dy], %[al], %[T]\n\t"
                    "v_fmac_f32_e32 %[Bk], %[al], %[qq]\n\t"
                    "ds_write2st64_b32 %[sa], %[dx], %[dy] offset1:5\n\t"
                    "s_cmp_lg_u64 exec, 0\n\t"
                    "s_cselect_b32 %[adv], 272, 0\n\t"
                    "s_lshl_b64 exec, 1, %[j]\n\t"
                    "v_mov_b32_e32 %[sa], %[tmp]\n\t"
                    "ds_write_b96 %[sa], %[meta] offset:2368\n\t"
                    "s_mov_b64 exec, -1\n\t"
                    : [dx] "=&v"(dx), [dy] "=&v"(dy), [t1] "=&v"(t1), [t2] "=&v"(t2), [G] "=&v"(G), [al] "=&v"(al), [inv] "=&v"(inv),
                      [qq] "=&v"(qq), [sa] "=&v"(sa), [T] "+v"(T), [Bk] "+v"(Bk), [adv] "=&s"(adv), [tmp] "=&s"(tmp)
                    : [px] "s"(r0[0]), [py] "s"(r0[1]), [ca] "s"(r1[0]), [cb] "s"(r1[1]), [cc] "s"(r1[2]), [op] "s"(r1[3]),
                      [cr] "s"(r1[4]), [cg] "s"(r1[5]), [cb2] "s"(r1[6]), [cz] "s"(r1[7]), [pxf] "v"(pxf), [pyf] "v"(pyf), [thr] "v"(thr),
                      [j] "s"(j), [g0] "v"(g0), [g1] "v"(g1), [g2] "v"(g2), [gd] "v"(gd), [bgT] "v"(bgT), [lane] "v"(lane), [zero] "v"(zero),
                      [koff] "s"(koff), [wbase] "s"(wbase), [meta] "v"(meta), [amin] "s"(1.0f / 255.0f)
                    : "vcc", "scc", "memory");
                koff += adv;
            if (koff == BT_SLOTS * BS_STRIDE) {
                bt_flush<POSE_ONLY, true>(bl, BT_SLOTS);
                koff = 0;
            }
        };
#ifdef BS_TRACE
        tr_n += (uint32_t)__popcll(mask);
#endif
        if (mask) {
            int jA, jB = 0;
            v2f a0, b0;
            v8f a1, b1;
            BS_POP(jA, a0, a1)
            for (;;) {
                asm volatile("s_waitcnt lgkmcnt(0)" : "+s"(a0), "+s"(a1) : : "memory");
                const bool moreB = mask != 0ull;
                if (moreB) { BS_POP(jB, b0, b1) }
                evaluate(a0, a1, jA);
                if (!moreB) break;
                asm volatile("s_waitcnt lgkmcnt(0)" : "+s"(b0), "+s"(b1) : : "memory");
                const bool moreA = mask != 0ull;
                if (moreA) { BS_POP(jA, a0, a1) }
                evaluate(b0, b1, jB);
                if (!moreA) break;
            }
        }
#undef BS_POP
    }
    if (koff) bt_flush<POSE_ONLY, true>(bl, (int)(koff >> 8));
#ifdef BS_TRACE
    if (a.trace) {
        unsigned long long tr1;
        BS_STAMP(tr1);
        const unsigned hw = __builtin_amdgcn_s_getreg((31 << 11) | 4), xcc = __builtin_amdgcn_s_getreg((31 << 11) | 20);
        if (lane == 0) {
            unsigned long long* o = a.trace + ((size_t)job * 4 + wave) * 4;
            o[0] = tr0; o[1] = tr1; o[2] = (unsigned long long)hw | ((unsigned long long)xcc << 32); o[3] = tr_n;
        }
    }
#endif
}

template <bool POSE_ONLY, bool SPLIT>
__global__ void __launch_bounds__(256) blend_backward_s_kernel(BlendArgs a, int ntiles,
                                                               const float* __restrict__ final_T,
                                                               const uint32_t* __restrict__ n_contrib,
                                                               const float* __restrict__ dL_dcolor,
                                                               const float* __restrict__ dL_ddepth,
                                                               const float* __restrict__ out_color,
                                                               const float* __restrict__ out_depth,
                                                               float* __restrict__ grad_acc, BsSplit sp, int adjacent) {
    __shared__ __attribute__((aligned(16))) BsWaveLds s_w[MGS_WG_WAVES];
// ... 25 lines not shown
    const int tile = (int)blockIdx.x;
    if (tile >= ntiles) return;
    const int tx = tile % a.gx, ty = tile / a.gx;
    const uint2 range = a.ranges[tile];
    if (range.y <= range.x) return;
    const int qx0i = tx * TILE + (wave & 1) * SUB, qy0i = ty * TILE + (wave >> 1) * SUB;
    const int pxi = qx0i + (lane & 7), pyi = qy0i + (lane >> 3);
    const bool inside = pxi < a.W && pyi < a.H;
    const float pxf = (float)pxi, pyf = (float)pyi, qx0 = (float)qx0i, qy0 = (float)qy0i;
    const uint32_t last = inside ? n_contrib[(size_t)pyi * a.W + pxi] : 0u;
    const uint32_t maxc = wave_max_u32(last);
    if (maxc == 0) return;
    const uint32_t end = range.x + maxc;
    unsigned long long c[8] = {0, 0, 0, 0, 0, 0, 0, 0};
    for (int b = (int)((maxc - 1) / WAVE); b >= 0; --b) {
        const uint32_t i = range.x + (uint32_t)b * WAVE + lane;
        uint32_t gid_l = 0;
        float4 box = make_float4(0.f, 0.f, -1.f, -1.f), el = make_float4(0.f, 0.f, 0.f, 0.f);
        if (i < end) {
            gid_l = a.point_list[i];
            box = a.rec[(size_t)gid_l * 4];
            el = a.rec[(size_t)gid_l * 4 + 3];
        }
        const unsigned long long alive = __builtin_amdgcn_ballot_w64(last >= (uint32_t)b * WAVE + 1u);
        unsigned long long mask = __builtin_amdgcn_ballot_w64(quadrant_hit(box, el, qx0, qy0, alive));
        c[0] += 1;
        c[1] += __popcll(mask);
        while (mask) {
            const int j = 63 - __builtin_clzll(mask);
            mask &= ~(1ull << j);
            const uint32_t k = (uint32_t)b * WAVE + (uint32_t)j + 1u;
            const Rec g = fetch(a, bcast(gid_l, j));
            const float dx = g.px - pxf, dy = g.py - pyf;
            const float power = dx * (g.ca * dx + g.cb * dy) + (g.cc * dy) * dy;
            const float alpha = fminf(0.99f, g.op * __builtin_amdgcn_exp2f(power));
            const bool geo = !(power > 0.f) && !(alpha < 1.0f / 255.0f);
            const unsigned long long act = __builtin_amdgcn_ballot_w64(geo && k <= last);
            const int n = __popcll(act);
            if (n == 0) {
                if (__builtin_amdgcn_ballot_w64(geo) != 0ull) c[4] += 1;
                continue;
            }
            c[2] += 1;
            c[3] += n;
            c[5] += n <= 2;
            c[6] += n <= 4;
            c[7] += n <= 8;
        }
    }
    if (lane < 8) {
        unsigned long long v = c[0];
#pragma unroll
        for (int q = 1; q < 8; ++q) v = lane == q ? c[q] : v;
        atomicAdd(stats + lane, v);
    }
}

__device__ __forceinline__ bool rect_hit(const float4 c, const float4 n, float qx0, float qy0, int ox, int oy, int w, int h,
                                         unsigned long long alive) {
    if (c.z < 0.f) return false;
    const float x0q = qx0 - 0.05f - c.x, y0q = qy0 - 0.05f - c.y;
    const float x0 = x0q + (float)ox, x1 = qx0 + (float)(ox + w - 1) + 0.05f - c.x;
    const float y0 = y0q + (float)oy, y1 = qy0 + (float)(oy + h - 1) + 0.05f - c.y;
    if (!((c.z >= x0) && (-c.z <= x1) && (c.w >= y0) && (-c.w <= y1))) return false;
    {
        const int ix0 = (int)fminf(8.f, fmaxf(0.f, ceilf(-x0q - c.z - 0.06f))), ix1 = (int)fminf(7.f, fmaxf(-1.f, floorf(-x0q + c.z + 0.06f)));
        const int iy0 = (int)fminf(8.f, fmaxf(0.f, ceilf(-y0q - c.w - 0.06f))), iy1 = (int)fminf(7.f, fmaxf(-1.f, floorf(-y0q + c.w + 0.06f)));
        if (ix0 > ix1 || iy0 > iy1) return false;
        const unsigned long long cols = (unsigned long long)((0xFFu >> (7 - ix1)) & (0xFFu << ix0) & 0xFFu) * 0x0101010101010101ull;
        const unsigned long long rows = (~0ull >> (8 * (7 - iy1))) & (~0ull << (8 * iy0));
        const unsigned long long gcols = (unsigned long long)(((1u << w) - 1u) << ox) * 0x0101010101010101ull;
        const unsigned long long grows = ((h >= 8 ? ~0ull : ((1ull << (8 * h)) - 1ull)) << (8 * oy));
        if ((cols & rows & gcols & grows & alive) == 0ull) return false;
    }
    if (x0 <= 0.f && x1 >= 0.f && y0 <= 0.f && y1 >= 0.f) return true;
    if (!(n.x > 0.f) || !(n.z > 0.f)) return true;
    const float rby = -n.y * __builtin_amdgcn_rcpf(n.z), rbx = -n.y * __builtin_amdgcn_rcpf(n.x);
    auto edge_x = [&](float xe) { const float t = fminf(y1, fmaxf(y0, rby * xe)); return n.x * xe * xe + 2.f * n.y * xe * t + n.z * t * t; };
    auto edge_y = [&](float ye) { const float t = fminf(x1, fmaxf(x0, rbx * ye)); return n.x * t * t + 2.f * n.y * t * ye + n.z * ye * ye; };
    return fminf(fminf(edge_x(x0), edge_x(x1)), fminf(edge_y(y0), edge_y(y1))) <= 1.02f;
}
__global__ void __launch_bounds__(256) blend_group_stats_kernel(BlendArgs a, int ntiles, const uint32_t* __restrict__ n_contrib,
                                                                unsigned long long* __restrict__ stats) {
    const int wave = threadIdx.x >> 6, lane = threadIdx.x & 63;
    const int tile = (int)blockIdx.x;
    if (tile >= ntiles) return;
    const int tx = tile % a.gx, ty = tile / a.gx;
    const uint2 range = a.ranges[tile];
    if (range.y <= range.x) return;
    const int qx0i = tx * TILE + (wave & 1) * SUB, qy0i = ty * TILE + (wave >> 1) * SUB;
    const int pxi = qx0i + (lane & 7), pyi = qy0i + (lane >> 3);
    const bool inside = pxi < a.W && pyi < a.H;
    const float qx0 = (float)qx0i, qy0 = (float)qy0i;
    const uint32_t last = inside ? n_contrib[(size_t)pyi * a.W + pxi] : 0u;
    const uint32_t maxc = wave_max_u32(last);
    if (maxc == 0) return;
    const uint32_t end = range.x + maxc;
    constexpr int ND = 5;
    constexpr int NG[ND] = {2, 2, 4, 4, 8}, GW[ND] = {8, 4, 4, 8, 4}, GH[ND] = {4, 8, 4, 2, 2}, GX[ND] = {1, 2, 2, 1, 2};
    unsigned long long trips_step[ND] = {0, 0, 0, 0, 0}, rows[ND] = {0, 0, 0, 0, 0};
    uint32_t walk[ND][8];
#pragma unroll
    for (int d = 0; d < ND; ++d)
#pragma unroll
        for (int g = 0; g < 8; ++g) walk[d][g] = 0;
    for (int b = (int)((maxc - 1) / WAVE); b >= 0; --b) {
        const uint32_t i = range.x + (uint32_t)b * WAVE + lane;
        float4 box = make_float4(0.f, 0.f, -1.f, -1.f), el = make_float4(0.f, 0.f, 0.f, 0.f);
        if (i < end) {
            const uint32_t gid_l = a.point_list[i];
            box = a.rec[(size_t)gid_l * 4];
            el = a.rec[(size_t)gid_l * 4 + 3];
        }
        const unsigned long long alive = __builtin_amdgcn_ballot_w64(last >= (uint32_t)b * WAVE + 1u);
#pragma unroll
        for (int d = 0; d < ND; ++d) {
            int mx = 0, sum = 0;
#pragma unroll
            for (int g = 0; g < NG[d]; ++g) {
                const int ox = (g % GX[d]) * GW[d], oy = (g / GX[d]) * GH[d];
                const int n = __popcll(__builtin_amdgcn_ballot_w64(rect_hit(box, el, qx0, qy0, ox, oy, GW[d], GH[d], alive)));
                mx = max(mx, n);
                sum += n;
                walk[d][g] += (uint32_t)n;
            }
            trips_step[d] += mx;
            rows[d] += sum;
        }
    }
    if (lane == 0) {
#pragma unroll
        for (int d = 0; d < ND; ++d) {
            uint32_t mx = 0;
#pragma unroll
            for (int g = 0; g < NG[d]; ++g) mx = max(mx, walk[d][g]);
            atomicAdd(stats + 8 + 3 * d + 0, trips_step[d]);
            atomicAdd(stats + 8 + 3 * d + 1, rows[d]);
            atomicAdd(stats + 8 + 3 * d + 2, (unsigned long long)mx);
        }
    }
}

int launch_blend_backward_stats(const mgs_camera& cam, const GeometryState& g, const BinningState& b,
                                const ImageState& img, unsigned long long* stats, hipStream_t s) {
    const BlendArgs a = make_args(cam, g, b, img);
    const int ntiles = a.gx * tiles_y(a.H);
    if (ntiles == 0) return 0;
    hipLaunchKernelGGL(blend_backward_stats_kernel, dim3(ntiles), dim3(256), 0, s, a, ntiles, img.n_contrib, stats);
    hipLaunchKernelGGL(blend_group_stats_kernel, dim3(ntiles), dim3(256), 0, s, a, ntiles, img.n_contrib, stats);
    MGS_HIP(hipGetLastError());
    return 0;
}

int g_opt_blend_bwd_split = -1;
int g_opt_blend_bwd_split_min = BS_SPLIT_MIN, g_opt_blend_bwd_split_frac = BS_SPLIT_FRAC;
int g_opt_blend_bwd_transposed = 2;
int g_dbg_last_bwd_split = -1;
static int bs_split_default(int ntiles, uint64_t num_rendered) {
    return num_rendered >= (uint64_t)ntiles * 128u ? 1 : 0;
}
bool g_opt_blend_bwd_transposed_set = false;
int launch_blend_backward(const mgs_camera& cam, const GeometryState& g, const BinningState& b,
                          const ImageState& img, const float* dL_dcolor, const float* dL_ddepth, const float* out_color,
                          const float* out_depth, float* grad_acc, bool pose_only, uint64_t num_rendered, hipStream_t s) {
    BlendArgs a = make_args(cam, g, b, img);
#ifdef BS_TRACE
    a.trace = g_trace_bwd;
#endif
    const int ntiles = a.gx * tiles_y(a.H);
    if (ntiles == 0) return 0;
    if (g_opt_blend_bwd_transposed == 2) {
        const int opt = g_opt_blend_bwd_split >= 0 ? g_opt_blend_bwd_split : g_opt_blend_bwd_transposed_set ? 0 : bs_split_default(ntiles, num_rendered);
        bool split = opt != 0 && out_color && out_depth;
#ifdef BS_TRACE
        if (a.trace && g_trace_bwd_records < 8ull * (unsigned long long)ntiles) split = false;
#endif
        g_dbg_last_bwd_split = split ? 1 : 0;
        const BsSplit sp{max(g_opt_blend_bwd_split_min, 2), min(max(g_opt_blend_bwd_split_frac, 1), 255)};
        const dim3 grid(split ? 2 * ntiles : ntiles), block(256);
#define BS_LAUNCH(P_, S_) hipLaunchKernelGGL((blend_backward_s_kernel<P_, S_>), grid, block, 0, s, a, ntiles, img.final_T, img.n_contrib, \
                                             dL_dcolor, dL_ddepth, out_color, out_depth, grad_acc, sp, (int)(opt == 2))
        if (pose_only) { if (split) BS_LAUNCH(true, true); else BS_LAUNCH(true, false); }
        else { if (split) BS_LAUNCH(false, true); else BS_LAUNCH(false, false); }
#undef BS_LAUNCH
    } else if (g_opt_blend_bwd_transposed != 0) {
        if (pose_only)
            hipLaunchKernelGGL((blend_backward_t_kernel<true>), dim3(ntiles), dim3(256), 0, s, a, ntiles, img.final_T,
                               img.n_contrib, dL_dcolor, dL_ddepth, grad_acc);
        else
            hipLaunchKernelGGL((blend_backward_t_kernel<false>), dim3(ntiles), dim3(256), 0, s, a, ntiles, img.final_T,
                               img.n_contrib, dL_dcolor, dL_ddepth, grad_acc);
    } else if (pose_only)
        hipLaunchKernelGGL((blend_backward_kernel<true>), dim3(ntiles), dim3(256), 0, s, a, ntiles, img.final_T,
                           img.n_contrib, dL_dcolor, dL_ddepth, grad_acc);
    else
        hipLaunchKernelGGL((blend_backward_kernel<false>), dim3(ntiles), dim3(256), 0, s, a, ntiles, img.final_T,
                           img.n_contrib, dL_dcolor, dL_ddepth, grad_acc);
    MGS_HIP(hipGetLastError());
    return 0;
}

__global__ void __launch_bounds__(256) valu_ceiling_kernel(float* out, int iters, float seed) {
    float a0 = seed + threadIdx.x, a1 = a0 + 1, a2 = a0 + 2, a3 = a0 + 3, a4 = a0 + 4, a5 = a0 + 5, a6 = a0 + 6, a7 = a0 + 7;
    const float c = 1.0001f, d = 0.0001f;
    for (int i = 0; i < iters; ++i) {
        a0 = __builtin_fmaf(a0, c, d); a1 = __builtin_fmaf(a1, c, d); a2 = __builtin_fmaf(a2, c, d); a3 = __builtin_fmaf(a3, c, d);
        a4 = __builtin_fmaf(a4, c, d); a5 = __builtin_fmaf(a5, c, d); a6 = __builtin_fmaf(a6, c, d); a7 = __builtin_fmaf(a7, c, d);
    }
    out[blockIdx.x * 256 + threadIdx.x] = ((a0 + a1) + (a2 + a3)) + ((a4 + a5) + (a6 + a7));
}
int launch_valu_ceiling(float* out, int iters, hipStream_t s) {
    hipLaunchKernelGGL(valu_ceiling_kernel, dim3(MGS_VALU_CEILING_BLOCKS), dim3(256), 0, s, out, iters, 1.0f);
    MGS_HIP(hipGetLastError());
    return 0;
}

}

#ifdef BS_TRACE
extern "C" int mgs_trace_set_blend_buffers(void* fwd, void* bwd, unsigned long long bwd_records) {
    mgs::g_trace_fwd = (unsigned long long*)fwd;
    mgs::g_trace_bwd = (unsigned long long*)bwd;
    mgs::g_trace_bwd_records = bwd ? bwd_records : 0;
    return 0;
}
#endif
```

monogs_amd/csrc/common.h:

```cpp
#pragma once

#include <hip/hip_runtime.h>
#include <stdint.h>
#include <stddef.h>

#include "../../include/monogs_raster.h"

namespace mgs {

constexpr int TILE = MGS_TILE;
constexpr int WAVE = 64;
constexpr int SUB = 8;
constexpr int REC_FLOATS = 16;
constexpr int GRAD_FLOATS = 16;

enum : int {
    R_X = 0, R_Y = 1, R_EX = 2, R_EY = 3,
    R_CA = 4, R_CB = 5, R_CC = 6, R_OPAC = 7,
    R_R = 8, R_G = 9, R_B = 10, R_DEPTH = 11,
    R_NA = 12, R_NB = 13, R_NC = 14, R_RADIUS = 15
};
enum : int {
    G_SX = 0, G_SY = 1, G_SXX = 2, G_SXY = 3, G_SYY = 4, G_SH = 5,
    G_DR = 6, G_DG = 7, G_DB = 8, G_DDEPTH = 9
};

inline size_t align_up(size_t v, size_t a) { return (v + a - 1) / a * a; }

#if defined(__HIP_DEVICE_COMPILE__)
typedef const float __attribute__((address_space(4))) * const_float_p;
#define MGS_CONST(p) ((mgs::const_float_p)(p))
#else
typedef const float* const_float_p;
#define MGS_CONST(p) (p)
#endif

__device__ __forceinline__ uint32_t wave_incl_scan_dpp(uint32_t v) {
#define MGS_DPP_ADD(ctrl, row_mask) v += (uint32_t)__builtin_amdgcn_update_dpp(0, (int)v, ctrl, row_mask, 0xf, false)
    MGS_DPP_ADD(0x111, 0xf);
    MGS_DPP_ADD(0x112, 0xf);
    MGS_DPP_ADD(0x114, 0xf);
    MGS_DPP_ADD(0x118, 0xf);
    MGS_DPP_ADD(0x142, 0xa);
    MGS_DPP_ADD(0x143, 0xc);
#undef MGS_DPP_ADD
    return v;
}

__global__ static void zero_fill_kernel(uint32_t* __restrict__ p, size_t n_words, int vec) {
    const size_t i0 = (size_t)blockIdx.x * blockDim.x + threadIdx.x, stride = (size_t)gridDim.x * blockDim.x;
    if (vec) {
        uint4* q = reinterpret_cast<uint4*>(p);
        const size_t nv = n_words / 4;
        for (size_t i = i0; i < nv; i += stride) q[i] = make_uint4(0u, 0u, 0u, 0u);
        for (size_t i = nv * 4 + i0; i < n_words; i += stride) p[i] = 0u;
    } else {
        for (size_t i = i0; i < n_words; i += stride) p[i] = 0u;
    }
}
__device__ __forceinline__ void grid_zero(uint32_t* __restrict__ p, size_t n_words, size_t threads, int block) {
    const size_t i0 = (size_t)blockIdx.x * block + threadIdx.x, stride = threads;
    uint4* q = reinterpret_cast<uint4*>(p);
    const size_t nv = n_words / 4;
    for (size_t i = i0; i < nv; i += stride) q[i] = make_uint4(0u, 0u, 0u, 0u);
    for (size_t i = nv * 4 + i0; i < n_words; i += stride) p[i] = 0u;
}
__global__ static void zero_fill2_kernel(uint32_t* __restrict__ p, size_t n_words, uint32_t* __restrict__ p2, int n2) {
    grid_zero(p, n_words, (size_t)gridDim.x * 256, 256);
    if (blockIdx.x == 0 && (int)threadIdx.x < n2) p2[threadIdx.x] = 0u;
}
static inline hipError_t zero_fill2(void* ptr, size_t bytes, void* ptr2, size_t bytes2, hipStream_t s) {
    const size_t n_words = bytes / 4;
    size_t blocks = (n_words / 4 + 255) / 256;
    blocks = blocks < 1 ? 1 : (blocks > 4096 ? 4096 : blocks);
    hipLaunchKernelGGL(zero_fill2_kernel, dim3((unsigned)blocks), dim3(256), 0, s, (uint32_t*)ptr, n_words,
                       (uint32_t*)ptr2, ptr2 ? (int)(bytes2 / 4) : 0);
    return hipGetLastError();
}
static inline hipError_t zero_fill(void* ptr, size_t bytes, hipStream_t s) {
    if (bytes == 0) return hipSuccess;
    const size_t n_words = bytes / 4;
    const int vec = ((size_t)ptr % 16 == 0) ? 1 : 0;
    const size_t items = vec ? (n_words + 3) / 4 : n_words;
    size_t blocks = (items + 255) / 256;
    if (blocks > 4096) blocks = 4096;
    hipLaunchKernelGGL(zero_fill_kernel, dim3((unsigned)blocks), dim3(256), 0, s, (uint32_t*)ptr, n_words, vec);
    return hipGetLastError();
}

struct GeometryState {
    float* rec;
    uint32_t* depth_key;
    uint32_t* depth_alt;
    uint32_t* iota;
    uint32_t* iota_alt;
    uint32_t* perm;
    uint32_t* point_offsets;
    uint32_t* scan_blocks;
    uint8_t* clamped;
    uint2* rect;
    uint2* rect_sorted;
    uint64_t* scan_status;
    uint32_t* tile_hist;
    void* sort_temp;
    size_t sort_temp_bytes;
    char* end;
    static size_t bytes(int P);
    static GeometryState carve(void* base, int P);
};
constexpr int SCAN_SMALL_MAX_BLOCKS = 64;

struct ImageState {
    float* final_T;
    uint32_t* n_contrib;
    uint2* ranges;
    static size_t bytes(int W, int H);
    static ImageState carve(void* base, int W, int H);
};

struct BinningState {
    uint32_t* keys_a;
    uint32_t* vals_a;
    uint32_t* keys_b;
    uint32_t* vals_b;
    uint32_t* keys_sorted;
    uint32_t* vals_sorted;
    void* sort_temp;
    size_t sort_temp_bytes;
    uint32_t* count;
    static size_t bytes(uint64_t R, int W, int H);
    static BinningState carve(void* base, uint64_t R, int W, int H);
};

constexpr int SCAN_ITEMS = 2048;
inline int scan_nblocks(int P) { return (P + SCAN_ITEMS - 1) / SCAN_ITEMS; }

inline int tiles_x(int W) { return (W + TILE - 1) / TILE; }
inline int tiles_y(int H) { return (H + TILE - 1) / TILE; }
inline int tile_bits(int W, int H) {
    uint32_t n = (uint32_t)(tiles_x(W) * tiles_y(H));
    int b = 0;
    while ((1u << b) < n && b < 31) ++b;
    return b == 0 ? 1 : b;
}

constexpr uint32_t DEPTH_KEY_SUB = 0x3E4CCCCDu;
constexpr uint32_t DEPTH_KEY_NARROW = (1u << 27) - 1u;
__host__ __device__ inline int tile_depth_lo_bits(int tb) { return tb > 5 ? tb - 5 : 0; }
int binning_path(int P, int W, int H);

void set_error(const char* fmt, ...);
#define MGS_HIP(expr)                                                                     \
    do {                                                                                  \
        hipError_t _e = (expr);                                                           \
        if (_e != hipSuccess) {                                                           \
            mgs::set_error("%s failed: %s (%s:%d)", #expr, hipGetErrorString(_e), __FILE__, __LINE__); \
            return 2;                                                                     \
        }                                                                                 \
    } while (0)

struct StageTimer;

int launch_preprocess_forward(const mgs_camera& cam, int P, const float* means3D, const float* shs,
                              const float* colors_precomp, const float* opacities, const float* scales,
                              const float* rotations, const float* cov3D_precomp,
                              const GeometryState& g, int32_t* radii, float* prepare_grad_acc, hipStream_t s);
constexpr int TAU_SLOTS = 256;
inline float* backward_grad_acc(void* scratch) { return (float*)align_up((size_t)scratch, 256); }
inline float* backward_tau_part(void* scratch, int P) { return backward_grad_acc(scratch) + (size_t)P * GRAD_FLOATS; }
inline float* backward_tau_out(void* scratch, int P) { return backward_tau_part(scratch, P) + (size_t)TAU_SLOTS * 16; }
int launch_scan(const GeometryState& g, int P, hipStream_t s, bool exclusive, const uint2* rects);
int launch_duplicate(const mgs_camera& cam, int P, const GeometryState& g, const BinningState& b, uint64_t r_cap,
                     int32_t* n_touched, const ImageState& img, uint64_t sort_n, int sort_bits, uint32_t* count,
                     uint32_t* overflow, hipStream_t s, bool per_tile);
size_t sort_temp_bytes(uint64_t n, int bits);
size_t radix_temp_bytes(uint64_t n, int bits);
size_t radix_depth_temp_bytes(uint64_t n);
bool radix_result_in_b(int bits);
constexpr int RADIX_ERROR_WORDS = 4;
const uint32_t* radix_error_flag(void* temp, uint64_t n, int bits);
const uint32_t* radix_depth_error_flag(void* temp, uint64_t n);
__device__ __forceinline__ uint32_t radix_failed(const uint32_t* __restrict__ e) { return (e[0] | e[1]) | (e[2] | e[3]); }
void radix_zero_region(void* temp, uint64_t n, int bits, uint32_t** ptr, size_t* words);
void radix_depth_zero_region(void* temp, uint64_t n, uint32_t** ptr, size_t* words, bool header_only = false);
int radix_sort_pairs(uint32_t* ka, uint32_t* va, uint32_t* kb, uint32_t* vb, uint64_t n, int bits, void* temp,
                     hipStream_t s, const uint32_t* n_dev = nullptr, bool temp_zeroed = false,
                     const uint2* aux_in = nullptr, uint2* aux_out = nullptr,
                     const uint32_t* ext_hist = nullptr,
                     bool aux_empty_for_ones = false,
                     bool exclusive = false,
                     uint2* ranges = nullptr,
                     int key_shift = 0);
bool radix_wants_hist(uint64_t n);
bool radix_depth_payload(uint64_t n);
int radix_sort_depth(uint32_t* keys, uint32_t* key_b, uint32_t* val_a, uint32_t* val_b, void* rect, bool payload,
                     uint32_t* perm, uint2* rect_sorted, uint64_t n, void* temp, hipStream_t s, bool temp_zeroed,
                     bool exclusive = false);
inline bool depth_sort_payload(int P, int W, int H) { return radix_depth_payload((uint64_t)P) && tiles_x(W) <= 255 && tiles_y(H) <= 255; }
int launch_depth_sort(const GeometryState& g, int P, bool payload, hipStream_t s, bool exclusive = false);
int launch_sort(const GeometryState& g, const BinningState& b, uint64_t R, int bits, hipStream_t s,
                const uint32_t* n_dev = nullptr, bool exclusive = false, uint2* ranges = nullptr, bool per_tile = false);
struct TileSortArgs {
    uint32_t* keys;
    uint32_t* vals;
    uint32_t* keys_alt;
    uint32_t* vals_alt;
    const uint32_t* depth_key;
    const uint32_t* n_dev;
    uint32_t n_cap;
    int tb;
};
TileSortArgs tile_sort_args(const mgs_camera& cam, const GeometryState& g, const BinningState& b, uint64_t R,
                            const uint32_t* n_dev);
int launch_tile_depth_sort(const mgs_camera& cam, const TileSortArgs& ts, const ImageState& img, const uint32_t* sort_err,
                           hipStream_t s);
int set_radix_spin_limit(uint32_t limit);
extern bool g_opt_blend_bwd_transposed_set;
extern int g_dbg_last_bwd_split;
extern int g_opt_radix_ballot_rank, g_opt_radix_scanned, g_opt_radix_xcd_band, g_opt_knn_grid_min, g_opt_scan_small, g_opt_dup_slot_major, g_opt_blend_bwd_transposed, g_opt_blend_bwd_split, g_opt_blend_bwd_split_min, g_opt_blend_bwd_split_frac;
int launch_blend_forward(const mgs_camera& cam, const GeometryState& g, const BinningState& b,
                         const ImageState& img, float* out_color, float* out_depth, float* out_opacity,
                         int32_t* n_touched, const uint32_t* sort_err, uint32_t* status, const TileSortArgs* tile_sort,
                         hipStream_t s);
int launch_blend_backward(const mgs_camera& cam, const GeometryState& g, const BinningState& b,
                          const ImageState& img, const float* dL_dcolor, const float* dL_ddepth, const float* out_color,
                          const float* out_depth, float* grad_acc, bool pose_only, uint64_t num_rendered, hipStream_t s);
int launch_blend_backward_stats(const mgs_camera& cam, const GeometryState& g, const BinningState& b,
                                const ImageState& img, unsigned long long* stats, hipStream_t s);
int launch_valu_ceiling(float* out, int iters, hipStream_t s);
struct GeomBackwardArgs {
    const float *means3D, *shs, *colors_precomp, *opacities, *scales, *rotations, *cov3D_precomp;
    const int32_t* radii;
    const float* grad_acc;
    float *dL_dmeans2D, *dL_dcolors, *dL_dopacity, *dL_dmeans3D, *dL_dcov3D, *dL_dsh, *dL_dscales,
        *dL_drotations, *dL_dtau;
    float* tau_part;
};
constexpr int TAU_DIRECT_MAX_BLOCKS = 256;
int launch_geom_backward(const mgs_camera& cam, int P, const GeometryState& g, const GeomBackwardArgs& a,
                         hipStream_t s);
int launch_mark_visible(int P, const float* means3D, const float* viewmatrix, uint8_t* visible, hipStream_t s);
size_t knn_scratch_bytes(int P);
int launch_knn(int P, const float* points, float* out, void* scratch, hipStream_t s);

}
```

monogs_amd/csrc/preprocess.hip:

```cpp
#include "common.h"

#pragma clang fp contract(off)

namespace mgs {

__device__ __forceinline__ float dot3p(float m0, float m1, float m2, float m3, float x, float y, float z) {
    return ((m0 * x + m1 * y) + m2 * z) + m3;
}

__device__ constexpr float SH_C0 = 0.28209479177387814f;
__device__ constexpr float SH_C1 = 0.4886025119029199f;
__device__ constexpr float SH_C2[5] = {1.0925484305920792f, -1.0925484305920792f, 0.31539156525252005f,
                                       -1.0925484305920792f, 0.5462742152960396f};
__device__ constexpr float SH_C3[7] = {-0.5900435899266435f, 2.890611442640554f, -0.4570457994644658f,
                                       0.3731763325901154f, -0.4570457994644658f, 1.445305721320277f,
                                       -0.5900435899266435f};

struct Cam {
    float V[16], PM[16], PR[16];
    float campos[3];
    float tanfovx, tanfovy, focal_x, focal_y, mod;
    int W, H, gx, gy, deg, M;
};

__device__ __forceinline__ void load_cam(Cam& c, const float* V_, const float* PM_, const float* PR_,
                                         const float* campos_) {
    const const_float_p V = MGS_CONST(V_), PM = MGS_CONST(PM_), PR = MGS_CONST(PR_), campos = MGS_CONST(campos_);
#pragma unroll
    for (int i = 0; i < 16; ++i) { c.V[i] = V[i]; c.PM[i] = PM[i]; }
    if (PR_) {
#pragma unroll
        for (int i = 0; i < 16; ++i) c.PR[i] = PR[i];
    } else {
#pragma unroll
        for (int i = 0; i < 16; ++i) c.PR[i] = 0.f;
    }
    c.campos[0] = campos[0]; c.campos[1] = campos[1]; c.campos[2] = campos[2];
}

__device__ __forceinline__ void pin_cam(const Cam& c, bool with_pr) {
    asm volatile("" ::"s"(c.V[0]), "s"(c.V[1]), "s"(c.V[2]), "s"(c.V[3]), "s"(c.V[4]), "s"(c.V[5]), "s"(c.V[6]), "s"(c.V[7]),
                 "s"(c.V[8]), "s"(c.V[9]), "s"(c.V[10]), "s"(c.V[11]), "s"(c.V[12]), "s"(c.V[13]), "s"(c.V[14]), "s"(c.V[15]));
    asm volatile("" ::"s"(c.PM[0]), "s"(c.PM[1]), "s"(c.PM[2]), "s"(c.PM[3]), "s"(c.PM[4]), "s"(c.PM[5]), "s"(c.PM[6]),
                 "s"(c.PM[7]), "s"(c.PM[8]), "s"(c.PM[9]), "s"(c.PM[10]), "s"(c.PM[11]), "s"(c.PM[12]), "s"(c.PM[13]),
                 "s"(c.PM[14]), "s"(c.PM[15]), "s"(c.campos[0]), "s"(c.campos[1]), "s"(c.campos[2]));
    if (with_pr)
        asm volatile("" ::"s"(c.PR[0]), "s"(c.PR[1]), "s"(c.PR[2]), "s"(c.PR[3]), "s"(c.PR[4]), "s"(c.PR[5]), "s"(c.PR[6]),
                     "s"(c.PR[7]), "s"(c.PR[8]), "s"(c.PR[9]), "s"(c.PR[10]), "s"(c.PR[11]), "s"(c.PR[12]), "s"(c.PR[13]),
                     "s"(c.PR[14]), "s"(c.PR[15]));
}

__device__ __forceinline__ void cov3d_from_scale_rot(const float s[3], const float q[4], float mod, float cov[6],
                                                     float Mm[9]) {
    const float r = q[0], x = q[1], y = q[2], z = q[3];
    float Rm[9] = {1.f - 2.f * (y * y + z * z), 2.f * (x * y - r * z), 2.f * (x * z + r * y),
                   2.f * (x * y + r * z), 1.f - 2.f * (x * x + z * z), 2.f * (y * z - r * x),
                   2.f * (x * z - r * y), 2.f * (y * z + r * x), 1.f - 2.f * (x * x + y * y)};
    const float sx = s[0] * mod, sy = s[1] * mod, sz = s[2] * mod;
#pragma unroll
    for (int i = 0; i < 3; ++i) {
        Mm[3 * i + 0] = Rm[3 * i + 0] * sx;
        Mm[3 * i + 1] = Rm[3 * i + 1] * sy;
        Mm[3 * i + 2] = Rm[3 * i + 2] * sz;
    }
    auto e = [&](int i, int j) {
        return (Mm[3 * i] * Mm[3 * j] + Mm[3 * i + 1] * Mm[3 * j + 1]) + Mm[3 * i + 2] * Mm[3 * j + 2];
    };
    cov[0] = e(0, 0); cov[1] = e(0, 1); cov[2] = e(0, 2);
    cov[3] = e(1, 1); cov[4] = e(1, 2); cov[5] = e(2, 2);
}

struct Proj {
    float tx, ty, tz;
    bool clamp_x, clamp_y;
    float J00, J02, J11, J12;
    float T0[3], T1[3];
    float cxx, cxy, cyy;
};

__device__ __forceinline__ void project_cov(const Cam& c, const float pv[3], const float cov[6], Proj& p) {
    const float limx = 1.3f * c.tanfovx, limy = 1.3f * c.tanfovy;
    const float tz = pv[2];
    const float txtz = pv[0] / tz, tytz = pv[1] / tz;
    p.clamp_x = (txtz < -limx) || (txtz > limx);
    p.clamp_y = (tytz < -limy) || (tytz > limy);
    p.tx = fminf(limx, fmaxf(-limx, txtz)) * tz;
    p.ty = fminf(limy, fmaxf(-limy, tytz)) * tz;
    p.tz = tz;
    const float tz2 = tz * tz;
    p.J00 = c.focal_x / tz;
    p.J02 = -(c.focal_x * p.tx) / tz2;
    p.J11 = c.focal_y / tz;
    p.J12 = -(c.focal_y * p.ty) / tz2;
#pragma unroll
    for (int j = 0; j < 3; ++j) {
        p.T0[j] = p.J00 * c.V[4 * j + 0] + p.J02 * c.V[4 * j + 2];
        p.T1[j] = p.J11 * c.V[4 * j + 1] + p.J12 * c.V[4 * j + 2];
    }
    const float S[3][3] = {{cov[0], cov[1], cov[2]}, {cov[1], cov[3], cov[4]}, {cov[2], cov[4], cov[5]}};
    float U0[3], U1[3];
#pragma unroll
    for (int j = 0; j < 3; ++j) {
        U0[j] = (p.T0[0] * S[0][j] + p.T0[1] * S[1][j]) + p.T0[2] * S[2][j];
        U1[j] = (p.T1[0] * S[0][j] + p.T1[1] * S[1][j]) + p.T1[2] * S[2][j];
    }
    p.cxx = ((U0[0] * p.T0[0] + U0[1] * p.T0[1]) + U0[2] * p.T0[2]) + 0.3f;
    p.cxy = (U0[0] * p.T1[0] + U0[1] * p.T1[1]) + U0[2] * p.T1[2];
    p.cyy = ((U1[0] * p.T1[0] + U1[1] * p.T1[1]) + U1[2] * p.T1[2]) + 0.3f;
}

__device__ __forceinline__ void tile_rect(float px, float py, float radius, int gx, int gy, int& x0, int& y0,
                                          int& x1, int& y1) {
    x0 = min(gx, max(0, (int)((px - radius) / (float)TILE)));
    y0 = min(gy, max(0, (int)((py - radius) / (float)TILE)));
    x1 = min(gx, max(0, (int)(((px + radius) + (float)(TILE - 1)) / (float)TILE)));
    y1 = min(gy, max(0, (int)(((py + radius) + (float)(TILE - 1)) / (float)TILE)));
}

__device__ __forceinline__ void eval_sh(int deg, const float* sh, const float d[3], float out[3]) {
    const float x = d[0], y = d[1], z = d[2];
#pragma unroll
    for (int ch = 0; ch < 3; ++ch) {
        float res = SH_C0 * sh[ch];
        if (deg > 0) {
            res = res - SH_C1 * y * sh[3 + ch] + SH_C1 * z * sh[6 + ch] - SH_C1 * x * sh[9 + ch];
            if (deg > 1) {
                const float xx = x * x, yy = y * y, zz = z * z, xy = x * y, yz = y * z, xz = x * z;
                res = res + SH_C2[0] * xy * sh[12 + ch] + SH_C2[1] * yz * sh[15 + ch] +
                      SH_C2[2] * (2.f * zz - xx - yy) * sh[18 + ch] + SH_C2[3] * xz * sh[21 + ch] +
                      SH_C2[4] * (xx - yy) * sh[24 + ch];
                if (deg > 2) {
                    res = res + SH_C3[0] * y * (3.f * xx - yy) * sh[27 + ch] + SH_C3[1] * xy * z * sh[30 + ch] +
                          SH_C3[2] * y * (4.f * zz - xx - yy) * sh[33 + ch] +
                          SH_C3[3] * z * (2.f * zz - 3.f * xx - 3.f * yy) * sh[36 + ch] +
                          SH_C3[4] * x * (4.f * zz - xx - yy) * sh[39 + ch] + SH_C3[5] * z * (xx - yy) * sh[42 + ch] +
                          SH_C3[6] * x * (xx - 3.f * yy) * sh[45 + ch];
                }
            }
        }
        out[ch] = res + 0.5f;
    }
}

struct PreArgs {
    const float *means3D, *shs, *colors, *opacities, *scales, *rotations, *cov3D;
    const float *V, *PM, *campos;
    float* rec;
    uint32_t* depth_key;
    int rect_packed;
    uint8_t* clamped;
    uint2* rect;
    int32_t* radii;
    float tanfovx, tanfovy, focal_x, focal_y, mod;
    int P, W, H, gx, gy, deg, M;
    int iso;
    int rot_aligned16;
    uint32_t* zero_ptr;
    size_t zero_words;
    float* grad_acc;
};

__device__ __forceinline__ void load4(const float* __restrict__ p, bool aligned16, float o[4]) {
    if (aligned16) {
        const float4 v = *reinterpret_cast<const float4*>(p);
        o[0] = v.x; o[1] = v.y; o[2] = v.z; o[3] = v.w;
    } else {
        o[0] = p[0]; o[1] = p[1]; o[2] = p[2]; o[3] = p[3];
    }
}

struct PreOut {
    float4 r0, r1, r2, r3;
    int radius;
    uint2 rect;
    uint32_t key;
};

template <bool COV, bool PRECOMP>
__device__ __forceinline__ bool preprocess_one(const PreArgs& a, const Cam& c, int idx, float x, float y, float z,
                                               const float cov_in[6], const float s[3], const float q[4],
                                               const float col_in[3], float opac, PreOut& o) {
    float pv[3];
#pragma unroll
    for (int k = 0; k < 3; ++k) pv[k] = dot3p(c.V[k], c.V[4 + k], c.V[8 + k], c.V[12 + k], x, y, z);
    if (!(pv[2] > 0.2f)) return false;
    float ph[4];
#pragma unroll
    for (int k = 0; k < 4; ++k) ph[k] = dot3p(c.PM[k], c.PM[4 + k], c.PM[8 + k], c.PM[12 + k], x, y, z);
    const float p_w = 1.0f / (ph[3] + 0.0000001f);
    const float projx = ph[0] * p_w, projy = ph[1] * p_w;

    float cov[6];
    if (COV) {
#pragma unroll
        for (int k = 0; k < 6; ++k) cov[k] = cov_in[k];
    } else {
        float Mm[9];
        cov3d_from_scale_rot(s, q, a.mod, cov, Mm);
    }
    Proj p;
    project_cov(c, pv, cov, p);
    const float det = p.cxx * p.cyy - p.cxy * p.cxy;
    if (det == 0.0f) return false;
    const float det_inv = 1.f / det;
    const float ca = p.cyy * det_inv, cb = -p.cxy * det_inv, cc = p.cxx * det_inv;
    const float mid = 0.5f * (p.cxx + p.cyy);
    const float disc = sqrtf(fmaxf(0.1f, mid * mid - det));
    const float lam = fmaxf(mid + disc, mid - disc);
    const float radius = ceilf(3.f * sqrtf(lam));
    const float px = ((projx + 1.0f) * (float)a.W - 1.0f) * 0.5f;
    const float py = ((projy + 1.0f) * (float)a.H - 1.0f) * 0.5f;
    if (!(isfinite(px) && isfinite(py) && isfinite(radius))) return false;
    int x0, y0, x1, y1;
    tile_rect(px, py, radius, a.gx, a.gy, x0, y0, x1, y1);
    const int ntile = (x1 - x0) * (y1 - y0);
    if (ntile == 0) return false;

    float rgb[3];
    if (PRECOMP) {
        rgb[0] = col_in[0]; rgb[1] = col_in[1]; rgb[2] = col_in[2];
    } else {
        float d[3] = {x - c.campos[0], y - c.campos[1], z - c.campos[2]};
        const float len = sqrtf((d[0] * d[0] + d[1] * d[1]) + d[2] * d[2]);
        d[0] = d[0] / len; d[1] = d[1] / len; d[2] = d[2] / len;
        eval_sh(a.deg, a.shs + (size_t)idx * a.M * 3, d, rgb);
#pragma unroll
        for (int ch = 0; ch < 3; ++ch) {
            a.clamped[4 * idx + ch] = rgb[ch] < 0.f;
            rgb[ch] = fmaxf(rgb[ch], 0.f);
        }
    }

    float ex = -1.f, ey = -1.f;
    float na = 0.f, nb = 0.f, nc = 0.f;
    const float tau = logf(255.0f * opac);
    if (tau > 0.f) {
        ex = sqrtf(2.f * tau * p.cxx) * 1.001f + 0.05f;
        ey = sqrtf(2.f * tau * p.cyy) * 1.001f + 0.05f;
        const float it = 1.f / (2.f * tau);
        na = ca * it; nb = cb * it; nc = cc * it;
    } else if (!(tau <= 0.f)) {
        ex = ey = 3.0e38f;
    }

    o.r0 = make_float4(px, py, ex, ey);
    constexpr float LOG2E = 1.4426950408889634f;
    o.r1 = make_float4(-0.5f * LOG2E * ca, -LOG2E * cb, -0.5f * LOG2E * cc, opac);
    o.r2 = make_float4(rgb[0], rgb[1], rgb[2], pv[2]);
    o.r3 = make_float4(na, nb, nc, radius);
    o.radius = (int)radius;
    o.rect = make_uint2((uint32_t)x0 | ((uint32_t)y0 << 16), (uint32_t)(x1 - x0) | ((uint32_t)(y1 - y0) << 16));
    o.key = __float_as_uint(pv[2]);
    return true;
}

template <bool COV, bool PRECOMP>
__global__ void __launch_bounds__(256) preprocess_forward_kernel(PreArgs a) {
    const int idx = blockIdx.x * 256 + threadIdx.x;
    grid_zero(a.zero_ptr, a.zero_words, (size_t)((a.P + 255) / 256) * 256, 256);
    if (a.grad_acc && blockIdx.x == 0) {
        float4* t4 = reinterpret_cast<float4*>(a.grad_acc + (size_t)a.P * GRAD_FLOATS);
        for (int i = threadIdx.x; i < (TAU_SLOTS + 1) * 4; i += 256) t4[i] = make_float4(0.f, 0.f, 0.f, 0.f);
    }
    if (idx >= a.P) return;
    Cam c;
    load_cam(c, a.V, a.PM, nullptr, a.campos);
    c.tanfovx = a.tanfovx; c.tanfovy = a.tanfovy; c.focal_x = a.focal_x; c.focal_y = a.focal_y;
    const float x = a.means3D[3 * idx], y = a.means3D[3 * idx + 1], z = a.means3D[3 * idx + 2];
    const float opac = a.opacities[idx];
    float cov_in[6] = {0.f, 0.f, 0.f, 0.f, 0.f, 0.f}, s[3] = {0.f, 0.f, 0.f}, q[4] = {1.f, 0.f, 0.f, 0.f};
    float col_in[3] = {0.f, 0.f, 0.f};
    if (COV) {
#pragma unroll
        for (int k = 0; k < 6; ++k) cov_in[k] = a.cov3D[6 * idx + k];
    } else {
        const float* sp = a.scales + (a.iso ? (size_t)idx : 3 * (size_t)idx);
        const int o1 = a.iso ? 0 : 1, o2 = a.iso ? 0 : 2;
        s[0] = sp[0]; s[1] = sp[o1]; s[2] = sp[o2];
        load4(a.rotations + 4 * (size_t)idx, a.rot_aligned16 != 0, q);
    }
    if (PRECOMP) { col_in[0] = a.colors[3 * idx]; col_in[1] = a.colors[3 * idx + 1]; col_in[2] = a.colors[3 * idx + 2]; }
    asm volatile("" ::"v"(x), "v"(y), "v"(z), "v"(opac), "v"(s[0]), "v"(s[1]), "v"(s[2]), "v"(q[0]), "v"(q[1]), "v"(q[2]),
                 "v"(q[3]), "v"(col_in[0]), "v"(col_in[1]), "v"(col_in[2]));
    if (COV) asm volatile("" ::"v"(cov_in[0]), "v"(cov_in[1]), "v"(cov_in[2]), "v"(cov_in[3]), "v"(cov_in[4]), "v"(cov_in[5]));
    pin_cam(c, false);

    PreOut o;
    const bool vis = preprocess_one<COV, PRECOMP>(a, c, idx, x, y, z, cov_in, s, q, col_in, opac, o);
    a.radii[idx] = vis ? o.radius : 0;
    if (a.rect_packed) {
        const uint32_t r4 = (o.rect.x & 0xFFu) | ((o.rect.x >> 16) << 8) | ((o.rect.y & 0xFFu) << 16) | ((o.rect.y >> 16) << 24);
        reinterpret_cast<uint32_t*>(a.rect)[idx] = vis ? r4 : 0u;
    } else {
        a.rect[idx] = vis ? o.rect : make_uint2(0u, 0u);
    }
    a.depth_key[idx] = vis ? o.key : 0xFFFFFFFFu;
    {
        __shared__ float4 s_rec[4][WAVE * 5];
        const int lane = threadIdx.x & 63, wv = threadIdx.x >> 6, wave_first = idx - lane;
        if (wave_first + WAVE <= a.P) {
            const unsigned long long vm = __builtin_amdgcn_ballot_w64(vis);
            float4* mine = s_rec[wv] + lane * 5;
            mine[0] = o.r0; mine[1] = o.r1; mine[2] = o.r2; mine[3] = o.r3;
            float4* base = reinterpret_cast<float4*>(a.rec + (size_t)wave_first * REC_FLOATS);
#pragma unroll
            for (int k = 0; k < 4; ++k) {
                const int src = (lane >> 2) + 16 * k;
                const float4 v = s_rec[wv][src * 5 + (lane & 3)];
                if ((vm >> src) & 1ull) base[k * WAVE + lane] = v;
            }
        } else if (vis) {
            float4* rec = reinterpret_cast<float4*>(a.rec + (size_t)idx * REC_FLOATS);
            rec[0] = o.r0; rec[1] = o.r1; rec[2] = o.r2; rec[3] = o.r3;
        }
    }
    if (a.grad_acc) {
        const float4 z4 = make_float4(0.f, 0.f, 0.f, 0.f);
        const int lane = threadIdx.x & 63, wave_first = idx - lane;
        if (wave_first + WAVE <= a.P) {
            const unsigned long long vm = __builtin_amdgcn_ballot_w64(vis);
            float4* base = reinterpret_cast<float4*>(a.grad_acc + (size_t)wave_first * GRAD_FLOATS);
#pragma unroll
            for (int k = 0; k < 4; ++k)
                if ((vm >> ((lane >> 2) + 16 * k)) & 1ull) base[k * WAVE + lane] = z4;
        } else if (vis) {
            float4* ga = reinterpret_cast<float4*>(a.grad_acc + (size_t)idx * GRAD_FLOATS);
            ga[0] = z4; ga[1] = z4; ga[2] = z4; ga[3] = z4;
        }
    }
}

int launch_preprocess_forward(const mgs_camera& cam, int P, const float* means3D, const float* shs,
                              const float* colors_precomp, const float* opacities, const float* scales,
                              const float* rotations, const float* cov3D_precomp, const GeometryState& g,
                              int32_t* radii, float* prepare_grad_acc, hipStream_t s) {
    PreArgs a;
    a.means3D = means3D; a.shs = shs; a.colors = colors_precomp; a.opacities = opacities;
    a.scales = scales; a.rotations = rotations; a.cov3D = cov3D_precomp;
    a.V = cam.viewmatrix; a.PM = cam.projmatrix; a.campos = cam.campos;
    a.rec = g.rec; a.depth_key = g.depth_key;
    a.grad_acc = prepare_grad_acc;
    a.rot_aligned16 = rotations && ((size_t)rotations % 16 == 0);
    a.clamped = g.clamped; a.rect = g.rect; a.radii = radii;
    a.tanfovx = cam.tanfovx; a.tanfovy = cam.tanfovy;
    a.focal_x = (float)cam.image_width / (2.0f * cam.tanfovx);
    a.focal_y = (float)cam.image_height / (2.0f * cam.tanfovy);
    a.mod = cam.scale_modifier;
    a.iso = cam.scale_dim == 1;
    a.P = P; a.W = cam.image_width; a.H = cam.image_height;
    a.gx = tiles_x(a.W); a.gy = tiles_y(a.H); a.deg = cam.sh_degree; a.M = cam.sh_coeffs;
    if (P == 0) return 0;
    const bool per_tile = binning_path(P, cam.image_width, cam.image_height) != 0;
    a.rect_packed = (!per_tile && depth_sort_payload(P, cam.image_width, cam.image_height)) ? 1 : 0;
    radix_depth_zero_region(g.sort_temp, (uint64_t)P, &a.zero_ptr, &a.zero_words, per_tile);
    a.zero_words += (size_t)((char*)a.zero_ptr - (char*)g.scan_status) / 4;
    a.zero_ptr = (uint32_t*)g.scan_status;
    const dim3 grid((P + 255) / 256), block(256);
    if (cov3D_precomp && colors_precomp) hipLaunchKernelGGL((preprocess_forward_kernel<true, true>), grid, block, 0, s, a);
    else if (cov3D_precomp) hipLaunchKernelGGL((preprocess_forward_kernel<true, false>), grid, block, 0, s, a);
    else if (colors_precomp) hipLaunchKernelGGL((preprocess_forward_kernel<false, true>), grid, block, 0, s, a);
    else hipLaunchKernelGGL((preprocess_forward_kernel<false, false>), grid, block, 0, s, a);
    MGS_HIP(hipGetLastError());
    return 0;
}

struct BwdArgs {
    GeomBackwardArgs g;
    const float *V, *PM, *PR, *campos;
    const float* rec;
    const uint8_t* clamped;
    float tanfovx, tanfovy, focal_x, focal_y, mod;
    int P, W, H, deg, M;
    int iso;
    int rot_aligned16, drot_aligned16;
};

__device__ __forceinline__ float wave_sum(float v) {
#pragma unroll
    for (int o = 32; o > 0; o >>= 1) v += __shfl_xor(v, o, 64);
    return v;
}

template <bool SH, bool COV>
__global__ void __launch_bounds__(256) geom_backward_kernel(BwdArgs a) {
    const int idx = blockIdx.x * 256 + threadIdx.x;
    float tau[6] = {0.f, 0.f, 0.f, 0.f, 0.f, 0.f};
    const bool in = idx < a.P;
    const size_t ci = in ? (size_t)idx : 0;
    Cam c;
    load_cam(c, a.V, a.PM, a.PR, a.campos);
    c.tanfovx = a.tanfovx; c.tanfovy = a.tanfovy; c.focal_x = a.focal_x; c.focal_y = a.focal_y;
    const int rad = a.g.radii[ci];
    const float x = a.g.means3D[3 * ci], y = a.g.means3D[3 * ci + 1], z = a.g.means3D[3 * ci + 2];
    const float opq = a.g.opacities[ci];
    __shared__ float4 s_ga[4][WAVE * 5];
    const int lane_ = threadIdx.x & 63, wv_ = threadIdx.x >> 6, wave_first = idx - lane_;
    const bool full_wave = wave_first + WAVE <= a.P;
    const float4* gsrc = full_wave ? reinterpret_cast<const float4*>(a.g.grad_acc + (size_t)wave_first * GRAD_FLOATS) + lane_
                                   : reinterpret_cast<const float4*>(a.g.grad_acc + ci * GRAD_FLOATS);
    const int gstep = full_wave ? WAVE : 1;
    const float4 t0 = gsrc[0], t1 = gsrc[gstep], t2 = gsrc[2 * gstep], t3 = gsrc[3 * gstep];
    float cov[6] = {0.f, 0.f, 0.f, 0.f, 0.f, 0.f}, Mm[9];
    float s[3] = {0.f, 0.f, 0.f}, q[4] = {1.f, 0.f, 0.f, 0.f};
    if (COV) {
#pragma unroll
        for (int k = 0; k < 6; ++k) cov[k] = a.g.cov3D_precomp[6 * ci + k];
        asm volatile("" ::"v"(cov[0]), "v"(cov[1]), "v"(cov[2]), "v"(cov[3]), "v"(cov[4]), "v"(cov[5]));
    } else {
        const float* sp = a.g.scales + (a.iso ? ci : 3 * ci);
        const int o1 = a.iso ? 0 : 1, o2 = a.iso ? 0 : 2;
        s[0] = sp[0]; s[1] = sp[o1]; s[2] = sp[o2];
        load4(a.g.rotations + 4 * ci, a.rot_aligned16 != 0, q);
        asm volatile("" ::"v"(s[0]), "v"(s[1]), "v"(s[2]), "v"(q[0]), "v"(q[1]), "v"(q[2]), "v"(q[3]));
    }
    asm volatile("" ::"v"(rad), "v"(x), "v"(y), "v"(z), "v"(opq));
    float4 ga0 = t0, ga1 = t1, ga2 = t2;
    if (full_wave) {
        float4* row = s_ga[wv_] + (lane_ >> 2) * 5 + (lane_ & 3);
        row[0] = t0; row[16 * 5] = t1; row[32 * 5] = t2; row[48 * 5] = t3;
        ga0 = s_ga[wv_][lane_ * 5 + 0]; ga1 = s_ga[wv_][lane_ * 5 + 1]; ga2 = s_ga[wv_][lane_ * 5 + 2];
    }
    pin_cam(c, true);
    const float ga[GRAD_FLOATS] = {ga0.x, ga0.y, ga0.z, ga0.w, ga1.x, ga1.y, ga1.z, ga1.w, ga2.x, ga2.y, 0.f, 0.f, 0.f, 0.f, 0.f, 0.f};
    const bool live = in && rad > 0;
    float o_m2[2] = {0.f, 0.f}, o_m3[3] = {0.f, 0.f, 0.f}, o_col[3] = {0.f, 0.f, 0.f}, o_sc[3] = {0.f, 0.f, 0.f};
    float o_rot[4] = {0.f, 0.f, 0.f, 0.f}, o_cov[6] = {0.f, 0.f, 0.f, 0.f, 0.f, 0.f}, o_opac = 0.f, o_siso = 0.f;
    if (in && !live && a.g.dL_dsh) for (int k = 0; k < a.M * 3; ++k) a.g.dL_dsh[(size_t)idx * a.M * 3 + k] = 0.f;
    if (live) {
        float pv[3];
#pragma unroll
        for (int k = 0; k < 3; ++k) pv[k] = dot3p(c.V[k], c.V[4 + k], c.V[8 + k], c.V[12 + k], x, y, z);
        if (!COV) cov3d_from_scale_rot(s, q, a.mod, cov, Mm);
        Proj p;
        project_cov(c, pv, cov, p);

        const float det_q = p.cxx * p.cyy - p.cxy * p.cxy;
        const float det_inv_q = 1.f / det_q;
        const float qa = p.cyy * det_inv_q, qb = -p.cxy * det_inv_q, qc = p.cxx * det_inv_q;
        const float gA = -0.5f * opq * ga[G_SXX], gBh = 0.5f * (-opq * ga[G_SXY]), gC = -0.5f * opq * ga[G_SYY];
        const float n00 = gA * qa + gBh * qb, n01 = gA * qb + gBh * qc;
        const float n10 = gBh * qa + gC * qb, n11 = gBh * qb + gC * qc;
        const float m00 = -(qa * n00 + qb * n10);
        const float m01 = -(qa * n01 + qb * n11);
        const float m11 = -(qb * n01 + qc * n11);

        float A0[3], A1[3];
#pragma unroll
        for (int j = 0; j < 3; ++j) {
            A0[j] = m00 * p.T0[j] + m01 * p.T1[j];
            A1[j] = m01 * p.T0[j] + m11 * p.T1[j];
        }
        float Gs[3][3];
#pragma unroll
        for (int i = 0; i < 3; ++i)
#pragma unroll
            for (int j = 0; j < 3; ++j) Gs[i][j] = p.T0[i] * A0[j] + p.T1[i] * A1[j];
        const float S[3][3] = {{cov[0], cov[1], cov[2]}, {cov[1], cov[3], cov[4]}, {cov[2], cov[4], cov[5]}};
        float dT0[3], dT1[3];
#pragma unroll
        for (int j = 0; j < 3; ++j) {
            dT0[j] = 2.f * ((A0[0] * S[0][j] + A0[1] * S[1][j]) + A0[2] * S[2][j]);
            dT1[j] = 2.f * ((A1[0] * S[0][j] + A1[1] * S[1][j]) + A1[2] * S[2][j]);
        }
        const float dJ00 = (dT0[0] * c.V[0] + dT0[1] * c.V[4]) + dT0[2] * c.V[8];
        const float dJ02 = (dT0[0] * c.V[2] + dT0[1] * c.V[6]) + dT0[2] * c.V[10];
        const float dJ11 = (dT1[0] * c.V[1] + dT1[1] * c.V[5]) + dT1[2] * c.V[9];
        const float dJ12 = (dT1[0] * c.V[2] + dT1[1] * c.V[6]) + dT1[2] * c.V[10];
        float dRv[3][3];
#pragma unroll
        for (int j = 0; j < 3; ++j) {
            dRv[0][j] = p.J00 * dT0[j];
            dRv[1][j] = p.J11 * dT1[j];
            dRv[2][j] = p.J02 * dT0[j] + p.J12 * dT1[j];
        }
        const float tz = p.tz, itz = 1.f / tz, itz2 = itz * itz, itz3 = itz2 * itz;
        float gpc[3];
        gpc[0] = p.clamp_x ? 0.f : -c.focal_x * itz2 * dJ02;
        gpc[1] = p.clamp_y ? 0.f : -c.focal_y * itz2 * dJ12;
        gpc[2] = -c.focal_x * itz2 * dJ00 - c.focal_y * itz2 * dJ11 + 2.f * c.focal_x * p.tx * itz3 * dJ02 +
                 2.f * c.focal_y * p.ty * itz3 * dJ12;

        const float gpx = -opq * (qa * ga[G_SX] + qb * ga[G_SY]);
        const float gpy = -opq * (qc * ga[G_SY] + qb * ga[G_SX]);
        const float gnx = gpx * 0.5f * (float)a.W, gny = gpy * 0.5f * (float)a.H;
        o_m2[0] = gnx; o_m2[1] = gny;
        float ph[4];
#pragma unroll
        for (int k = 0; k < 4; ++k) ph[k] = dot3p(c.PM[k], c.PM[4 + k], c.PM[8 + k], c.PM[12 + k], x, y, z);
        const float p_w = 1.0f / (ph[3] + 0.0000001f);
        const float dph[4] = {gnx * p_w, gny * p_w, 0.f, -(gnx * ph[0] + gny * ph[1]) * p_w * p_w};
#pragma unroll
        for (int j = 0; j < 3; ++j)
            gpc[j] += ((dph[0] * c.PR[4 * j] + dph[1] * c.PR[4 * j + 1]) + dph[2] * c.PR[4 * j + 2]) +
                      dph[3] * c.PR[4 * j + 3];
// ... 227 lines not shown
```

monogs_amd/rasterizer.py:

```python
from __future__ import annotations

import contextlib
import ctypes as C
import weakref
from typing import NamedTuple, Optional

import torch
import torch.nn as nn

from . import _lib


class GaussianRasterizationSettings(NamedTuple):
    image_height: int
    image_width: int
    tanfovx: float
    tanfovy: float
    bg: torch.Tensor
    scale_modifier: float
    viewmatrix: torch.Tensor
    projmatrix: torch.Tensor
    projmatrix_raw: torch.Tensor
    sh_degree: int
    campos: torch.Tensor
# ... 211 lines not shown
            hint = _State.capacity_hint.get(key)
            if capturing and hint is None:
                raise RuntimeError("graph capture needs a capacity hint: run one eager forward with the same "
                                   "(P, W, H) first")
            if _State.exact_failed and not capturing:
                bits, _State.exact_failed = _State.exact_failed, 0
                _raise_sort_failure(bits)
            if (capturing or _sync_free["enabled"]) and hint is not None and P > 0:
                R = max(int(hint * _sync_free["headroom"]) + 4096, 4096)
                binning = torch.empty(lib.mgs_binning_bytes(R, W, H), **u8)
                _lib.check(lib.mgs_forward_capacity(
                    C.byref(cam), P, _ptr(means3D), _ptr(sh_), _ptr(col_), _ptr(opac_), _ptr(sc_), _ptr(rot_), _ptr(cov_),
                    geom_p, radii.data_ptr(), bwd_p, R, binning.data_ptr(), img_p, color.data_ptr(), depth.data_ptr(),
                    opacity.data_ptr(), n_touched.data_ptr(), status.data_ptr(), tref, _stream()), "mgs_forward_capacity")
                (_State.graph if capturing else _State.pending).append((key, status))
                if len(_State.pending) > PENDING_MAX:
                    del _State.pending[:PENDING_MAX // 2]
                ctx.overflow = status
            else:
                num_rendered, prev_bits = C.c_uint64(0), C.c_uint32(0)
                prev = _State.exact_pending
                here = (torch._C._cuda_getDevice(), _stream())
                if prev is not None and (prev[2], prev[3]) != here:
                    _State.exact_other.append(prev)
                    if len(_State.exact_other) > PENDING_MAX:
                        _drain_exact_other(PENDING_MAX // 2)
                    prev = None
                _lib.check(lib.mgs_forward_preprocess(
                    C.byref(cam), P, _ptr(means3D), _ptr(sh_), _ptr(col_), _ptr(opac_), _ptr(sc_), _ptr(rot_),
                    _ptr(cov_), geom_p, radii.data_ptr(), bwd_p, C.byref(num_rendered),
                    prev[1].data_ptr() if prev is not None else None, C.byref(prev_bits) if prev is not None else None,
                    tref, _stream()), "mgs_forward_preprocess")
                _State.exact_pending = None
                if prev_bits.value & (STATUS_DEPTH_SORT_TIMEOUT | STATUS_TILE_SORT_TIMEOUT):
                    _raise_sort_failure(prev_bits.value)
                R = int(num_rendered.value)
                _remember_hint(key, R)
                binning = torch.empty(lib.mgs_binning_bytes(R, W, H), **u8)
                _lib.check(lib.mgs_forward_render(
                    C.byref(cam), P, R, geom_p, binning.data_ptr(), img_p, color.data_ptr(),
                    depth.data_ptr(), opacity.data_ptr(), n_touched.data_ptr(), _ptr(status), tref, _stream()),
                    "mgs_forward_render")
                if status is not None:
                    _State.exact_pending = (key, status, here[0], here[1])
                ctx.overflow = None
            if rs.debug:
                check_overflow()
            if timing is not None:
                d = timing.as_dict()
                d.update(kind="forward", num_rendered=R, P=P)
                _timing_sink.append(d)

        ctx.cam, ctx.keep = cam, keep
        ctx.geom_off, ctx.img_off = off0, off0 + n_geom
        ctx.raster_settings = rs
        ctx.num_rendered = R
        ctx.sh_coeffs = M
        ctx.scale_dim = scale_dim
        ctx.has = (sh_ is not None, col_ is not None, sc_ is not None, cov_ is not None,
                   theta is not None, rho is not None)
        dummy = torch.empty(0, device=dev)
        ctx.save_for_backward(means3D, sh_ if sh_ is not None else dummy, col_ if col_ is not None else dummy,
                              opac_, sc_ if sc_ is not None else dummy, rot_ if rot_ is not None else dummy,
                              cov_ if cov_ is not None else dummy, radii, arena, binning)
        ctx.out_version = out5._version
        ctx.mark_non_differentiable(radii, n_touched)
        ctx.set_materialize_grads(False)
        return color, radii, depth, opacity, n_touched

    @staticmethod
    def backward(ctx, grad_color, grad_radii, grad_depth, grad_opacity, grad_n_touched):
        lib = _lib.load()
        rs = ctx.raster_settings
        means3D, sh_, col_, opac_, sc_, rot_, cov_, radii, arena, binning = ctx.saved_tensors
        geom_p, img_p = arena.data_ptr() + ctx.geom_off, arena.data_ptr() + ctx.img_off
        has_sh, has_col, has_sr, has_cov, has_theta, has_rho = ctx.has
        P = means3D.shape[0]
        dev = means3D.device
        H, W = int(rs.image_height), int(rs.image_width)
        need = ctx.needs_input_grad

        with _device_guard(dev):
            cam = ctx.cam
            f32 = dict(dtype=torch.float32, device=dev)
            g_color = _f32(grad_color, "grad_color") if grad_color is not None else torch.zeros(3, H, W, **f32)
            g_depth = _f32(grad_depth, "grad_depth") if grad_depth is not None else torch.zeros(1, H, W, **f32)
            out = lambda cond, *shape: torch.empty(*shape, **f32) if cond else None
            d_means2D = out(need[1], P, 3)
            d_sh = out(need[2] and has_sh, P, max(ctx.sh_coeffs, 1), 3)
            d_cov = out(need[7] and has_cov, P, 6)
            widths = [3 if need[0] else 0, 3 if (need[3] and has_col) else 0, 1 if need[4] else 0,
                      ctx.scale_dim if (need[5] and has_sr) else 0, 4 if (need[6] and has_sr) else 0]
            flat = torch.empty(P * sum(widths), **f32) if sum(widths) else None
            views, o = [], 0
            for w in widths:
                views.append(flat[o:o + P * w].view(P, w) if w else None)
                o += P * w
            d_means3D, d_col, d_opac, d_scales, d_rot = views
            want_tau = (need[8] and has_theta) or (need[9] and has_rho)
            prepared = ctx.scratch is not None and not ctx.scratch_used
            ctx.scratch_used = True
            scratch = ctx.scratch if prepared else torch.empty(lib.mgs_backward_bytes(P), dtype=torch.uint8, device=dev)
            if want_tau and prepared:
                off = int(lib.mgs_backward_tau(scratch.data_ptr(), P)) - scratch.data_ptr()
                d_tau = scratch[off:off + 24].view(torch.float32)
            else:
                d_tau = torch.empty(6, **f32) if want_tau else None
            timing = _lib.MgsTiming() if _timing_sink is not None else None
            tref = C.byref(timing) if timing is not None else None
            out5 = ctx.out_ref() if ctx.out_ref is not None else None
            if out5 is not None and out5._version != ctx.out_version:
                out5 = None
            _lib.check(lib.mgs_backward(
                C.byref(cam), P, ctx.num_rendered,
                _ptr(means3D), _ptr(sh_) if has_sh else None, _ptr(col_) if has_col else None, _ptr(opac_),
                _ptr(sc_) if has_sr else None, _ptr(rot_) if has_sr else None, _ptr(cov_) if has_cov else None,
                radii.data_ptr(), geom_p, binning.data_ptr(), img_p,
                g_color.data_ptr(), g_depth.data_ptr(),
                out5.data_ptr() if out5 is not None else None,
                out5.data_ptr() + 12 * H * W if out5 is not None else None,
                _ptr(d_means2D), _ptr(d_col), _ptr(d_opac), _ptr(d_means3D), _ptr(d_cov), _ptr(d_sh),
                _ptr(d_scales), _ptr(d_rot), _ptr(d_tau), scratch.data_ptr(), 1 if prepared else 0, tref, _stream()),
                "mgs_backward")
            if timing is not None:
                d = timing.as_dict()
                d.update(kind="backward", num_rendered=ctx.num_rendered, P=P)
                _timing_sink.append(d)
        d_theta = d_tau[3:] if (d_tau is not None and need[8] and has_theta) else None
        d_rho = d_tau[:3] if (d_tau is not None and need[9] and has_rho) else None
        return (d_means3D, d_means2D, d_sh, d_col, d_opac, d_scales, d_rot, d_cov, d_theta, d_rho, None)


def debug_blend_stats(color: torch.Tensor) -> dict:
    fn = color.grad_fn
    if fn is None or not hasattr(fn, "raster_settings"):
        raise RuntimeError("debug_blend_stats needs the colour image of a differentiable rasteriser forward")
    lib = _lib.load()
    means3D, _, _, _, _, _, _, _, arena, binning = fn.saved_tensors
    cam = fn.cam
    out = torch.zeros(24, dtype=torch.int64, device=means3D.device)
    with _device_guard(means3D.device):
        _lib.check(lib.mgs_debug_blend_stats(C.byref(cam), means3D.shape[0], fn.num_rendered,
                                             arena.data_ptr() + fn.geom_off, binning.data_ptr(),
                                             arena.data_ptr() + fn.img_off, out.data_ptr(), _stream()),
                   "mgs_debug_blend_stats")
    v = out.tolist()
    groups = {}
    for d, name in enumerate(("halves_8x4", "halves_4x8", "blocks_4x4", "strips_8x2", "blocks_4x2")):
        groups[name] = dict(trips_paired_per_step=v[8 + 3 * d], rows=v[9 + 3 * d], trips_own_lists=v[10 + 3 * d])
    return dict(steps=v[0], survivors=v[1], active_survivors=v[2], active_pairs=v[3], inactive_by_depth_order=v[4],
                active_le2=v[5], active_le4=v[6], active_le8=v[7], group_streams=groups)


def rasterize_gaussians(means3D, means2D, sh, colors_precomp, opacities, scales, rotations, cov3Ds_precomp,
                        theta, rho, raster_settings):
    return _RasterizeGaussians.apply(means3D, means2D, sh, colors_precomp, opacities, scales, rotations,
                                     cov3Ds_precomp, theta, rho, raster_settings)


class GaussianRasterizer(nn.Module):
    def __init__(self, raster_settings: GaussianRasterizationSettings):
        super().__init__()
        self.raster_settings = raster_settings

    def markVisible(self, positions: torch.Tensor) -> torch.Tensor:
        lib = _lib.load()
        rs = self.raster_settings
        with torch.no_grad():
            pos = _f32(positions, "positions")
            P = pos.shape[0]
            vis = torch.zeros(P, dtype=torch.uint8, device=pos.device)
            with _device_guard(pos.device):
                vm = _f32(rs.viewmatrix, "viewmatrix")
                pm = _f32(rs.projmatrix, "projmatrix")
                _lib.check(lib.mgs_mark_visible(P, pos.data_ptr(), vm.data_ptr(), pm.data_ptr(), vis.data_ptr(),
                                                _stream()), "mgs_mark_visible")
        return vis.bool()

    def forward(self, means3D, means2D, opacities, shs=None, colors_precomp=None, scales=None, rotations=None,
                cov3D_precomp=None, theta=None, rho=None):
        rs = self.raster_settings
        if (shs is None and colors_precomp is None) or (shs is not None and colors_precomp is not None):
            raise Exception("Please provide excatly one of either SHs or precomputed colors!")
        if ((scales is None or rotations is None) and cov3D_precomp is None) or \
                ((scales is not None or rotations is not None) and cov3D_precomp is not None):
            raise Exception("Please provide exactly one of either scale/rotation pair or precomputed 3D covariance!")
        return rasterize_gaussians(means3D, means2D, shs, colors_precomp, opacities, scales, rotations,
                                   cov3D_precomp, theta, rho, rs)
```

Baseline: 2905 Mpix/s.

## Reuse forward per-wave hit masks in backward blend and move grad zeroing

```diff
diff --git a/include/monogs_raster.h b/include/monogs_raster.h
--- a/include/monogs_raster.h
+++ b/include/monogs_raster.h
@@ -8,7 +8,7 @@
 extern "C" {
 #endif
 
-#define MGS_ABI_VERSION 12
+#define MGS_ABI_VERSION 13
 #define MGS_TILE 16
 
 typedef struct mgs_camera {
@@ -125,6 +125,10 @@
 #define MGS_BLEND_STATS_WORDS 24
 int mgs_debug_blend_stats(const mgs_camera* cam, int32_t P, uint64_t num_rendered, const void* geometry,
                           const void* binning, const void* image, uint64_t* stats_dev, void* stream);
+
+#define MGS_BLEND_MASK_STATS_WORDS 4
+int mgs_debug_blend_mask_stats(const mgs_camera* cam, int32_t P, uint64_t num_rendered, const void* geometry,
+                               const void* binning, const void* image, uint64_t* stats_dev, void* stream);
 
 int mgs_mark_visible(int32_t P, const float* means3D, const float* viewmatrix, const float* projmatrix,
                      uint8_t* visible, void* stream);
diff --git a/monogs_amd/_lib.py b/monogs_amd/_lib.py
--- a/monogs_amd/_lib.py
+++ b/monogs_amd/_lib.py
@@ -5,7 +5,7 @@
 
 _HERE = os.path.dirname(os.path.abspath(__file__))
 LIB_PATH = os.environ.get("MGS_LIB_PATH") or os.path.join(_HERE, "lib", "libmonogs_raster.so")
-ABI_VERSION = 12
+ABI_VERSION = 13
 
 c_float_p = C.c_void_p
 
@@ -55,6 +55,7 @@
                      + [C.c_void_p, C.c_int32, C.POINTER(MgsTiming), C.c_void_p]),
     "mgs_backward_tau": (C.c_void_p, [C.c_void_p, C.c_int32]),
     "mgs_debug_blend_stats": (C.c_int, [C.POINTER(MgsCamera), C.c_int32, C.c_uint64] + [C.c_void_p] * 5),
+    "mgs_debug_blend_mask_stats": (C.c_int, [C.POINTER(MgsCamera), C.c_int32, C.c_uint64] + [C.c_void_p] * 5),
     "mgs_debug_valu_ceiling": (C.c_int, [C.c_void_p, C.c_int32, C.c_void_p]),
     "mgs_debug_set_blend_events": (C.c_int, [C.c_void_p] * 4),
     "mgs_debug_last_backward_split": (C.c_int, []),
diff --git a/monogs_amd/csrc/api.hip b/monogs_amd/csrc/api.hip
--- a/monogs_amd/csrc/api.hip
+++ b/monogs_amd/csrc/api.hip
@@ -39,6 +39,7 @@
     g.tile_hist = (uint32_t*)take(p, 4 * 256 * sizeof(uint32_t));
     g.sort_temp_bytes = radix_depth_temp_bytes((uint64_t)P);
     g.sort_temp = take(p, g.sort_temp_bytes);
+    g.prepare = (unsigned long long*)take(p, 2 * sizeof(unsigned long long));
     g.end = p;
     return g;
 }
@@ -61,9 +62,13 @@
     return s;
 }
 
+size_t BinningState::fwd_mask_rows(uint64_t R, int W, int H) {
+    return (size_t)(R / 64) + (size_t)tiles_x(W) * tiles_y(H) + 1;
+}
 size_t BinningState::bytes(uint64_t R, int W, int H) {
     const size_t r = (size_t)(R ? R : 1);
-    return align_up(r * 4, 256) * 4 + align_up(mgs::sort_temp_bytes(R, tile_bits(W, H)), 256) + 256 + 256;
+    return align_up(r * 4, 256) * 4 + align_up(mgs::sort_temp_bytes(R, tile_bits(W, H)), 256) + 256 +
+           align_up(fwd_mask_rows(R, W, H) * 4 * sizeof(unsigned long long), 256) + 256;
 }
 BinningState BinningState::carve(void* base, uint64_t R, int W, int H) {
     const size_t r = (size_t)(R ? R : 1);
@@ -79,6 +84,7 @@
     b.sort_temp_bytes = mgs::sort_temp_bytes(R, tile_bits(W, H));
     b.sort_temp = take(p, b.sort_temp_bytes);
     b.count = (uint32_t*)take(p, 2 * sizeof(uint32_t));
+    b.fwd_masks = (unsigned long long*)take(p, fwd_mask_rows(R, W, H) * 4 * sizeof(unsigned long long));
     return b;
 }
 
@@ -252,7 +258,7 @@
     tm.mark();
     if (g_dbg_fwd_events[0]) MGS_HIP(hipEventRecord(g_dbg_fwd_events[0], s));
     if (int rc = launch_blend_forward(*cam, g, b, img, out_color, out_depth, out_opacity, n_touched, sort_err, overflow,
-                                      fused ? &ts : nullptr, s)) return rc;
+                                      fused ? &ts : nullptr, P, s)) return rc;
     if (g_dbg_fwd_events[1]) MGS_HIP(hipEventRecord(g_dbg_fwd_events[1], s));
     tm.mark();
     if (timing) {
@@ -366,6 +372,20 @@
     return launch_blend_backward_stats(*cam, g, b, img, (unsigned long long*)stats_dev, s);
 }
 
+int mgs_debug_blend_mask_stats(const mgs_camera* cam, int32_t P, uint64_t R, const void* geometry, const void* binning,
+                               const void* image, uint64_t* stats_dev, void* stream) {
+    if (check_cam(cam)) return 1;
+    if (!geometry || !image || !stats_dev || (R > 0 && !binning)) { set_error("bad arguments"); return 1; }
+    hipStream_t s = (hipStream_t)stream;
+    MGS_HIP(zero_fill(stats_dev, MGS_BLEND_MASK_STATS_WORDS * sizeof(uint64_t), s));
+    if (P == 0 || R == 0) return 0;
+    const int W = cam->image_width, H = cam->image_height;
+    GeometryState g = GeometryState::carve(const_cast<void*>(geometry), P);
+    ImageState img = ImageState::carve(const_cast<void*>(image), W, H);
+    BinningState b = BinningState::carve(const_cast<void*>(binning), R, W, H);
+    return launch_blend_mask_stats(*cam, g, b, img, (unsigned long long*)stats_dev, s);
+}
+
 int mgs_debug_valu_ceiling(float* out, int32_t iters, void* stream) {
     if (!out || iters < 1) { set_error("mgs_debug_valu_ceiling: bad arguments"); return 1; }
     return launch_valu_ceiling(out, iters, (hipStream_t)stream);
diff --git a/monogs_amd/csrc/binning.hip b/monogs_amd/csrc/binning.hip
--- a/monogs_amd/csrc/binning.hip
+++ b/monogs_amd/csrc/binning.hip
@@ -163,8 +163,13 @@
                                                         uint32_t* __restrict__ count, uint32_t* __restrict__ overflow,
                                                         const uint32_t* __restrict__ depth_err, int offsets_global,
                                                         uint32_t* __restrict__ hist , int hist_passes,
-                                                        int n_threads , int slot_major) {
+                                                        int n_threads , int slot_major,
+                                                        unsigned long long* __restrict__ prepare ) {
     const int i = blockIdx.x * 256 + threadIdx.x;
+    if (i == 0 && prepare) {
+        prepare[1] = prepare[0];
+        prepare[0] = 0ull;
+    }
     const int lane = threadIdx.x & 63;
     grid_zero(zero_ptr, zero_words, (size_t)n_threads, 256);
     const bool depth_bad = depth_err && radix_failed(depth_err) != 0u;
@@ -369,7 +374,8 @@
                        (uint32_t)(r_cap > 0xFFFFFFFFull ? 0xFFFFFFFFull : r_cap), n_touched, img.ranges, ntiles, zero_ptr,
                        zero_words, count, overflow, depth_err,
                        (P > 0 && scan_is_small(P)) ? 1 : 0,
-                       count_digits ? g.tile_hist : nullptr, (sort_bits + 7) / 8, n_threads, slot_major ? 1 : 0);
+                       count_digits ? g.tile_hist : nullptr, (sort_bits + 7) / 8, n_threads, slot_major ? 1 : 0,
+                       P > 0 ? g.prepare : nullptr);
     MGS_HIP(hipGetLastError());
     return 0;
 }
diff --git a/monogs_amd/csrc/blend.hip b/monogs_amd/csrc/blend.hip
--- a/monogs_amd/csrc/blend.hip
+++ b/monogs_amd/csrc/blend.hip
@@ -29,8 +29,12 @@
     const uint32_t* __restrict__ point_list;
     const uint2* __restrict__ ranges;
     const float* __restrict__ bg;
+    unsigned long long* fwd_masks;
     int W, H, gx;
 };
+__device__ __forceinline__ size_t fwd_mask_word(uint32_t range_x, int tile, int wave) {
+    return ((size_t)(range_x / WAVE) + (size_t)tile) * 4 + (size_t)wave;
+}
 
 __device__ __forceinline__ bool quadrant_hit(const float4 c , const float4 n ,
                                              float qx0, float qy0, unsigned long long alive) {
@@ -136,8 +140,19 @@
                                                             int32_t* __restrict__ n_touched,
                                                             uint2* ranges_rw ,
                                                             const uint32_t* __restrict__ sort_err,
-                                                            uint32_t* __restrict__ status, TileSortArgs ts) {
+                                                            uint32_t* __restrict__ status, TileSortArgs ts,
+                                                            const unsigned long long* __restrict__ prepare ,
+                                                            int P, int lines_per_tile ) {
     MGS_TILE_WAVE(a.gx * ((a.H + TILE - 1) / TILE), tile, wave, ws)
+    if (prepare) {
+        float* const acc = reinterpret_cast<float*>((uintptr_t)MGS_CONST_U64(prepare)[1]);
+        if (acc) {
+            const int first = tile * lines_per_tile;
+            const int n4 = 4 * min(lines_per_tile, P - first);
+            float4* const base = reinterpret_cast<float4*>(acc + (size_t)first * GRAD_FLOATS);
+            for (int i = (int)threadIdx.x; i < n4; i += 256) base[i] = make_float4(0.f, 0.f, 0.f, 0.f);
+        }
+    }
     const int tx = tile % a.gx, ty = tile / a.gx;
     const int lane = threadIdx.x & 63;
     const bool first_of_tile = wave == 0 && lane == 0;
@@ -220,6 +235,8 @@
         }
         if (decltype(touch_tag)::value && touched_cnt != 0) atomicAdd(n_touched + gid_l, touched_cnt);
     };
+    unsigned long long* const mask_row = a.fwd_masks + fwd_mask_word((uint32_t)__builtin_amdgcn_readfirstlane((int)range.x), tile, wave);
+    uint32_t mask_off = 0;
     if (range.x < range.y) prefetch(range.x + lane);
     for (uint32_t base = range.x; base < range.y && live != 0ull; base += WAVE) {
         const uint32_t gid_l = gid_n;
@@ -229,6 +246,9 @@
         const unsigned long long mask = __builtin_amdgcn_ballot_w64(quadrant_hit(c, el, qx0, qy0, live));
         if ((live & __builtin_amdgcn_ballot_w64(T > 0.5f)) != 0ull) walk_step(std::true_type{}, base, gid_l, mask);
         else walk_step(std::false_type{}, base, gid_l, mask);
+        if (__builtin_amdgcn_inverse_ballot_w64(1ull))
+            asm volatile("global_store_dwordx2 %0, %1, %2" ::"v"(mask_off), "v"(mask), "s"(mask_row) : "memory");
+        mask_off += 4u * (uint32_t)sizeof(unsigned long long);
     }
 #ifdef BS_TRACE
     if (a.trace) {
@@ -263,6 +283,7 @@
     a.point_list = b.vals_sorted;
     a.ranges = img.ranges;
     a.bg = cam.bg;
+    a.fwd_masks = b.fwd_masks;
     a.W = cam.image_width;
     a.H = cam.image_height;
     a.gx = tiles_x(a.W);
@@ -272,7 +293,7 @@
 int launch_blend_forward(const mgs_camera& cam, const GeometryState& g, const BinningState& b,
                          const ImageState& img, float* out_color, float* out_depth, float* out_opacity,
                          int32_t* n_touched, const uint32_t* sort_err, uint32_t* status, const TileSortArgs* tile_sort,
-                         hipStream_t s) {
+                         int P, hipStream_t s) {
     BlendArgs a = make_args(cam, g, b, img);
 #ifdef BS_TRACE
     a.trace = g_trace_fwd;
@@ -281,12 +302,16 @@
     if (ntiles == 0) return 0;
     const dim3 grid(ntiles), block(256);
     const TileSortArgs ts = tile_sort ? *tile_sort : TileSortArgs{};
+    const unsigned long long* const prepare = P > 0 ? g.prepare : nullptr;
+    const int lines_per_tile = (P + ntiles - 1) / ntiles;
     if (tile_sort)
         hipLaunchKernelGGL(blend_forward_kernel<true>, grid, block, 0, s, a, out_color, out_depth,
-                           out_opacity, img.final_T, img.n_contrib, n_touched, img.ranges, sort_err, status, ts);
+                           out_opacity, img.final_T, img.n_contrib, n_touched, img.ranges, sort_err, status, ts, prepare, P,
+                           lines_per_tile);
     else
         hipLaunchKernelGGL(blend_forward_kernel<false>, grid, block, 0, s, a, out_color, out_depth,
-                           out_opacity, img.final_T, img.n_contrib, n_touched, img.ranges, sort_err, status, ts);
+                           out_opacity, img.final_T, img.n_contrib, n_touched, img.ranges, sort_err, status, ts, prepare, P,
+                           lines_per_tile);
     MGS_HIP(hipGetLastError());
     return 0;
 }
@@ -745,20 +770,12 @@
 #endif
 
     const int q = lane & 15;
-    const int fxi = qx0i + 4 * (q & 1), fyi = qy0i + (q >> 1);
-    if (lane < 16) {
-#pragma unroll
-        for (int i = 0; i < 4; ++i) {
-            const bool in_i = (fxi + i) < a.W && fyi < a.H;
-            const size_t px_i = (size_t)fyi * a.W + fxi + i;
-            if (!POSE_ONLY) {
-                s_pix_ws[(0 * 16 + q) * 4 + i] = in_i ? dL_dcolor[px_i] : 0.f;
-                s_pix_ws[(1 * 16 + q) * 4 + i] = in_i ? dL_dcolor[HW + px_i] : 0.f;
-                s_pix_ws[(2 * 16 + q) * 4 + i] = in_i ? dL_dcolor[2 * HW + px_i] : 0.f;
-            }
-            s_pix_ws[((POSE_ONLY ? 0 : 3) * 16 + q) * 4 + i] = in_i ? dL_ddepth[px_i] : 0.f;
-        }
-    }
+    if (!POSE_ONLY) {
+        s_pix_ws[0 * 64 + lane] = g0;
+        s_pix_ws[1 * 64 + lane] = g1;
+        s_pix_ws[2 * 64 + lane] = g2;
+    }
+    s_pix_ws[(POSE_ONLY ? 0 : 3) * 64 + lane] = gd;
     const int slot = POSE_ONLY ? bt_slot6(q) : bt_slot10(q);
     const uint32_t slot_bytes = slot < 0 ? 0u : (uint32_t)slot * 4u;
     const unsigned long long m_out = __builtin_amdgcn_ballot_w64(slot >= 0);
@@ -770,28 +787,29 @@
     float zero = 0.f;
     asm volatile("" : "+v"(zero));
 
+    const const_u64_p mask_row = MGS_CONST_U64(a.fwd_masks) + fwd_mask_word((uint32_t)__builtin_amdgcn_readfirstlane((int)range.x), tile, wave);
     uint32_t gid_n = 0;
-    float4 box_n = make_float4(0.f, 0.f, -1.f, -1.f), ell_n = make_float4(0.f, 0.f, 0.f, 0.f);
+    float2 ctr_n = make_float2(0.f, 0.f);
+    unsigned long long mask_n = 0ull;
     auto prefetch = [&](int b) {
+        mask_n = mask_row[(size_t)max(b, 0) * 4];
         gid_n = 0;
-        box_n = make_float4(0.f, 0.f, -1.f, -1.f);
         const uint32_t i = range.x + (uint32_t)b * WAVE + (uint32_t)(FRONT ? lane : 63 - lane);
         if (b >= (FRONT ? 0 : b_lo) && i < end) {
             gid_n = a.point_list[i];
-            box_n = a.rec[(size_t)gid_n * 4];
-            ell_n = a.rec[(size_t)gid_n * 4 + 3];
+            ctr_n = *reinterpret_cast<const float2*>(a.rec + (size_t)gid_n * 4);
         }
     };
     const int b_first = FRONT ? 0 : (int)((maxc - 1) / WAVE), b_step = FRONT ? 1 : -1;
     prefetch(b_first);
     for (int b = b_first; FRONT ? b < b_lo : b >= b_lo; b += b_step) {
-        const float4 c = box_n, el = ell_n;
-        v3f meta = {c.x, c.y, __uint_as_float(gid_n << 6)};
+        v3f meta = {ctr_n.x, ctr_n.y, __uint_as_float(gid_n << 6)};
+        unsigned long long mask = mask_n;
         prefetch(b + b_step);
-        const unsigned long long alive = __builtin_amdgcn_ballot_w64(last >= (uint32_t)b * WAVE + 1u);
-        int qxs = qx0i, qys = qy0i;
-        asm volatile("" : "+s"(qxs), "+s"(qys));
-        unsigned long long mask = __builtin_amdgcn_ballot_w64(quadrant_hit(c, el, (float)qxs, (float)qys, alive));
+        if (!FRONT) {
+            if (b == b_first) mask &= ~0ull >> (63u - ((maxc - 1u) & 63u));
+            mask = __builtin_bitreverse64(mask);
+        }
         const int thr = FRONT ? (int)last - (int)((uint32_t)b * WAVE + 1u) : 63 + (int)((uint32_t)b * WAVE + 1u) - (int)last;
 #define BS_POP(J, R0, R1)                                                                                                    \
         asm volatile("s_ff1_i32_b64 %0, %1\n\ts_bitset0_b64 %1, %0" : "=&s"(J), "+s"(mask));                                 \
@@ -1123,6 +1141,54 @@
     return 0;
 }
 
+__global__ void __launch_bounds__(256) blend_mask_stats_kernel(BlendArgs a, int ntiles, const uint32_t* __restrict__ n_contrib,
+                                                               unsigned long long* __restrict__ stats) {
+    const int wave = threadIdx.x >> 6, lane = threadIdx.x & 63;
+    const int tile = (int)blockIdx.x;
+    if (tile >= ntiles) return;
+    const int tx = tile % a.gx, ty = tile / a.gx;
+    const uint2 range = a.ranges[tile];
+    if (range.y <= range.x) return;
+    const int qx0i = tx * TILE + (wave & 1) * SUB, qy0i = ty * TILE + (wave >> 1) * SUB;
+    const int pxi = qx0i + (lane & 7), pyi = qy0i + (lane >> 3);
+    const bool inside = pxi < a.W && pyi < a.H;
+    const float qx0 = (float)qx0i, qy0 = (float)qy0i;
+    const uint32_t last = inside ? n_contrib[(size_t)pyi * a.W + pxi] : 0u;
+    const uint32_t maxc = wave_max_u32(last);
+    if (maxc == 0) return;
+    const uint32_t end = range.x + maxc;
+    const unsigned long long* const mask_row = a.fwd_masks + fwd_mask_word(range.x, tile, wave);
+    unsigned long long c0 = 0, c1 = 0, c2 = 0, c3 = 0;
+    const int b_first = (int)((maxc - 1) / WAVE);
+    for (int b = b_first; b >= 0; --b) {
+        const uint32_t i = range.x + (uint32_t)b * WAVE + lane;
+        float4 box = make_float4(0.f, 0.f, -1.f, -1.f), el = make_float4(0.f, 0.f, 0.f, 0.f);
+        if (i < end) {
+            const uint32_t gid_l = a.point_list[i];
+            box = a.rec[(size_t)gid_l * 4];
+            el = a.rec[(size_t)gid_l * 4 + 3];
+        }
+        const unsigned long long alive = __builtin_amdgcn_ballot_w64(last >= (uint32_t)b * WAVE + 1u);
+        const unsigned long long own = __builtin_amdgcn_ballot_w64(quadrant_hit(box, el, qx0, qy0, alive));
+        unsigned long long fwd = mask_row[(size_t)b * 4];
+        if (b == b_first) fwd &= ~0ull >> (63u - ((maxc - 1u) & 63u));
+        c0 += 1;
+        c1 += __popcll(own);
+        c2 += __popcll(fwd);
+        c3 += __popcll(own & ~fwd);
+    }
+    if (lane < 4) atomicAdd(stats + lane, lane == 0 ? c0 : lane == 1 ? c1 : lane == 2 ? c2 : c3);
+}
+int launch_blend_mask_stats(const mgs_camera& cam, const GeometryState& g, const BinningState& b,
+                            const ImageState& img, unsigned long long* stats, hipStream_t s) {
+    const BlendArgs a = make_args(cam, g, b, img);
+    const int ntiles = a.gx * tiles_y(a.H);
+    if (ntiles == 0) return 0;
+    hipLaunchKernelGGL(blend_mask_stats_kernel, dim3(ntiles), dim3(256), 0, s, a, ntiles, img.n_contrib, stats);
+    MGS_HIP(hipGetLastError());
+    return 0;
+}
+
 int g_opt_blend_bwd_split = -1;
 int g_opt_blend_bwd_split_min = BS_SPLIT_MIN, g_opt_blend_bwd_split_frac = BS_SPLIT_FRAC;
 int g_opt_blend_bwd_transposed = 2;
diff --git a/monogs_amd/csrc/common.h b/monogs_amd/csrc/common.h
--- a/monogs_amd/csrc/common.h
+++ b/monogs_amd/csrc/common.h
@@ -29,10 +29,14 @@
 
 #if defined(__HIP_DEVICE_COMPILE__)
 typedef const float __attribute__((address_space(4))) * const_float_p;
+typedef const unsigned long long __attribute__((address_space(4))) * const_u64_p;
 #define MGS_CONST(p) ((mgs::const_float_p)(p))
+#define MGS_CONST_U64(p) ((mgs::const_u64_p)(p))
 #else
 typedef const float* const_float_p;
+typedef const unsigned long long* const_u64_p;
 #define MGS_CONST(p) (p)
+#define MGS_CONST_U64(p) (p)
 #endif
 
 __device__ __forceinline__ uint32_t wave_incl_scan_dpp(uint32_t v) {
@@ -104,6 +108,7 @@
     uint32_t* tile_hist;
     void* sort_temp;
     size_t sort_temp_bytes;
+    unsigned long long* prepare;
     char* end;
     static size_t bytes(int P);
     static GeometryState carve(void* base, int P);
@@ -128,6 +133,8 @@
     void* sort_temp;
     size_t sort_temp_bytes;
     uint32_t* count;
+    unsigned long long* fwd_masks;
+    static size_t fwd_mask_rows(uint64_t R, int W, int H);
     static size_t bytes(uint64_t R, int W, int H);
     static BinningState carve(void* base, uint64_t R, int W, int H);
 };
@@ -221,12 +228,14 @@
 int launch_blend_forward(const mgs_camera& cam, const GeometryState& g, const BinningState& b,
                          const ImageState& img, float* out_color, float* out_depth, float* out_opacity,
                          int32_t* n_touched, const uint32_t* sort_err, uint32_t* status, const TileSortArgs* tile_sort,
-                         hipStream_t s);
+                         int P, hipStream_t s);
 int launch_blend_backward(const mgs_camera& cam, const GeometryState& g, const BinningState& b,
                           const ImageState& img, const float* dL_dcolor, const float* dL_ddepth, const float* out_color,
                           const float* out_depth, float* grad_acc, bool pose_only, uint64_t num_rendered, hipStream_t s);
 int launch_blend_backward_stats(const mgs_camera& cam, const GeometryState& g, const BinningState& b,
                                 const ImageState& img, unsigned long long* stats, hipStream_t s);
+int launch_blend_mask_stats(const mgs_camera& cam, const GeometryState& g, const BinningState& b,
+                            const ImageState& img, unsigned long long* stats, hipStream_t s);
 int launch_valu_ceiling(float* out, int iters, hipStream_t s);
 struct GeomBackwardArgs {
     const float *means3D, *shs, *colors_precomp, *opacities, *scales, *rotations, *cov3D_precomp;
diff --git a/monogs_amd/csrc/preprocess.hip b/monogs_amd/csrc/preprocess.hip
--- a/monogs_amd/csrc/preprocess.hip
+++ b/monogs_amd/csrc/preprocess.hip
@@ -158,6 +158,7 @@
     uint32_t* zero_ptr;
     size_t zero_words;
     float* grad_acc;
+    unsigned long long* prepare;
 };
 
 __device__ __forceinline__ void load4(const float* __restrict__ p, bool aligned16, float o[4]) {
@@ -262,6 +263,7 @@
         float4* t4 = reinterpret_cast<float4*>(a.grad_acc + (size_t)a.P * GRAD_FLOATS);
         for (int i = threadIdx.x; i < (TAU_SLOTS + 1) * 4; i += 256) t4[i] = make_float4(0.f, 0.f, 0.f, 0.f);
     }
+    if (idx == 0) a.prepare[0] = (unsigned long long)(uintptr_t)a.grad_acc;
     if (idx >= a.P) return;
     Cam c;
     load_cam(c, a.V, a.PM, nullptr, a.campos);
@@ -312,20 +314,6 @@
         } else if (vis) {
             float4* rec = reinterpret_cast<float4*>(a.rec + (size_t)idx * REC_FLOATS);
             rec[0] = o.r0; rec[1] = o.r1; rec[2] = o.r2; rec[3] = o.r3;
-        }
-    }
-    if (a.grad_acc) {
-        const float4 z4 = make_float4(0.f, 0.f, 0.f, 0.f);
-        const int lane = threadIdx.x & 63, wave_first = idx - lane;
-        if (wave_first + WAVE <= a.P) {
-            const unsigned long long vm = __builtin_amdgcn_ballot_w64(vis);
-            float4* base = reinterpret_cast<float4*>(a.grad_acc + (size_t)wave_first * GRAD_FLOATS);
-#pragma unroll
-            for (int k = 0; k < 4; ++k)
-                if ((vm >> ((lane >> 2) + 16 * k)) & 1ull) base[k * WAVE + lane] = z4;
-        } else if (vis) {
-            float4* ga = reinterpret_cast<float4*>(a.grad_acc + (size_t)idx * GRAD_FLOATS);
-            ga[0] = z4; ga[1] = z4; ga[2] = z4; ga[3] = z4;
         }
     }
 }
@@ -340,6 +328,7 @@
     a.V = cam.viewmatrix; a.PM = cam.projmatrix; a.campos = cam.campos;
     a.rec = g.rec; a.depth_key = g.depth_key;
     a.grad_acc = prepare_grad_acc;
+    a.prepare = g.prepare;
     a.rot_aligned16 = rotations && ((size_t)rotations % 16 == 0);
     a.clamped = g.clamped; a.rect = g.rect; a.radii = radii;
     a.tanfovx = cam.tanfovx; a.tanfovy = cam.tanfovy;
diff --git a/monogs_amd/rasterizer.py b/monogs_amd/rasterizer.py
--- a/monogs_amd/rasterizer.py
+++ b/monogs_amd/rasterizer.py
@@ -387,6 +387,22 @@
                 active_le2=v[5], active_le4=v[6], active_le8=v[7], group_streams=groups)
 
 
+def debug_blend_mask_stats(color: torch.Tensor) -> dict:
+    fn = color.grad_fn
+    if fn is None or not hasattr(fn, "raster_settings"):
+        raise RuntimeError("debug_blend_mask_stats needs the colour image of a differentiable rasteriser forward")
+    lib = _lib.load()
+    means3D, _, _, _, _, _, _, _, arena, binning = fn.saved_tensors
+    out = torch.zeros(4, dtype=torch.int64, device=means3D.device)
+    with _device_guard(means3D.device):
+        _lib.check(lib.mgs_debug_blend_mask_stats(C.byref(fn.cam), means3D.shape[0], fn.num_rendered,
+                                                  arena.data_ptr() + fn.geom_off, binning.data_ptr(),
+                                                  arena.data_ptr() + fn.img_off, out.data_ptr(), _stream()),
+                   "mgs_debug_blend_mask_stats")
+    v = out.tolist()
+    return dict(steps=v[0], own_cull=v[1], forward_masks=v[2], missing=v[3])
+
+
 def rasterize_gaussians(means3D, means2D, sh, colors_precomp, opacities, scales, rotations, cov3Ds_precomp,
                         theta, rho, raster_settings):
     return _RasterizeGaussians.apply(means3D, means2D, sh, colors_precomp, opacities, scales, rotations,
```

Measured after the change: 2973 Mpix/s, median of 6. 1.02x the previous value.
